# speechandlanguageprocessing/ICASSP2022-Depression

Measured on AMD Instinct MI355X. Metric: utterances/sec (train step) for GRU-256 on (B,T,F)=(512,300,256), higher is better.
Workload: dtype f32; 1 GPU; audio_gru_whole.AudioBiLSTM train step, B=512/GPU T=300 F=256 H=256 L=2 dropout=0.5 AdamW, CE-on-softmax; global_batch=512, parallelism=dp1, ranks=1, backend=none

## Files before the change

### icassp2022-depression_amd/_lib.py

```python
import ctypes as C
import os

import torch

HERE = os.path.dirname(os.path.abspath(__file__))
LIB_PATH = os.environ.get('DEP_LIB_PATH') or os.path.join(HERE, 'libdep_rnn.so')

CELL_GRU, CELL_LSTM = 0, 1
POOL_NONE, POOL_MEAN, POOL_SUM = 0, 1, 2
RUN_EVAL, RUN_TRAIN, RUN_DROPOUT_ONLY = 0, 1, 2
LOSS_CE_ON_SOFTMAX, LOSS_L1_RELU, LOSS_SMOOTHL1_RELU, LOSS_CE_LOGITS, LOSS_SMOOTHL1 = 0, 1, 2, 3, 4
LOSS_LABELS_I64 = 0x100
REG_L1, REG_SMOOTHL1, REG_HUBER, REG_MSE = 0, 1, 2, 3
SITE_FC0, SITE_FC1, SITE_FC2, SITE_FC3 = 1, 2, 3, 4


class DepError(RuntimeError):
    pass


class RnnDesc(C.Structure):
    _fields_ = [('cell', C.c_int32), ('B', C.c_int32), ('T', C.c_int32), ('F', C.c_int32), ('H', C.c_int32),
                ('L', C.c_int32), ('dirs', C.c_int32), ('training', C.c_int32), ('dropout_p', C.c_float),
                ('seed', C.c_uint64), ('pool', C.c_int32), ('impl', C.c_int32)]


_P = C.c_void_p


class GradSync(C.Structure):
    _fields_ = [('comm', _P), ('comm_stream', _P), ('range_ptr', _P * 8), ('range_count', C.c_long * 8)]


_BWD_ARGS = [C.POINTER(RnnDesc), _P, C.POINTER(_P), _P, _P, _P, C.POINTER(_P), _P, _P, C.c_size_t, _P, C.c_size_t, _P]
_BWD_VARLEN_ARGS = _BWD_ARGS[:2] + [_P] + _BWD_ARGS[2:]
_SIGS = {
    'dep_last_error': (C.c_char_p, []),
    'dep_version': (C.c_int, []),
    'dep_arch': (C.c_char_p, []),
    'dep_rnn_reserve_bytes': (C.c_size_t, [C.POINTER(RnnDesc)]),
    'dep_rnn_workspace_bytes': (C.c_size_t, [C.POINTER(RnnDesc)]),
    'dep_rnn_reserve_y_offset': (C.c_size_t, [C.POINTER(RnnDesc), C.c_int]),
    'dep_rnn_reserve_ydrop_offset': (C.c_size_t, [C.POINTER(RnnDesc), C.c_int]),
    'dep_rnn_status': (C.c_int, [C.POINTER(RnnDesc), _P, _P]),
    'dep_rnn_set_exclusive': (C.c_int, [C.c_int]),
    'dep_rnn_get_exclusive': (C.c_int, []),
    'dep_rnn_workspace_xbuf_offset': (C.c_size_t, [C.POINTER(RnnDesc)]),
    'dep_rnn_forward': (C.c_int, [C.POINTER(RnnDesc), _P, C.POINTER(_P), _P, _P, _P, _P, C.c_size_t, _P, C.c_size_t, _P]),
    'dep_rnn_backward': (C.c_int, _BWD_ARGS),
    'dep_rnn_backward_overlapped': (C.c_int, _BWD_ARGS + [C.POINTER(GradSync)]),
    'dep_rnn_forward_varlen': (C.c_int, [C.POINTER(RnnDesc), _P, _P, C.POINTER(_P), _P, _P, _P, _P, C.c_size_t, _P, C.c_size_t, _P]),
    'dep_rnn_backward_varlen': (C.c_int, _BWD_VARLEN_ARGS),
    'dep_rnn_backward_overlapped_varlen': (C.c_int, _BWD_VARLEN_ARGS + [C.POINTER(GradSync)]),
    'dep_comm_available': (C.c_int, []),
    'dep_comm_unique_id': (C.c_int, [_P, C.c_size_t]),
    'dep_comm_init': (C.c_int, [C.POINTER(_P), C.c_int, C.c_int, _P, C.c_size_t, C.c_int]),
    'dep_comm_world': (C.c_int, [_P]),
    'dep_comm_rank': (C.c_int, [_P]),
    'dep_comm_allreduce': (C.c_int, [_P, _P, C.c_long, _P]),
    'dep_comm_allreduce_ranges': (C.c_int, [_P, C.POINTER(_P), C.POINTER(C.c_long), C.c_int, _P]),
    'dep_comm_destroy': (C.c_int, [_P]),
    'dep_gemm_workspace_bytes': (C.c_size_t, [C.c_int] * 5),
    'dep_gemm_f32': (C.c_int, [C.c_int] * 5 + [_P, C.c_int, _P, C.c_int, _P, C.c_int, _P, C.c_float, C.c_int, C.c_int,
                               _P, C.c_size_t, _P]),
    'dep_gemm_bf16x3': (C.c_int, [C.c_int] * 5 + [_P, C.c_int, _P, C.c_int, _P, C.c_int, _P, C.c_float, C.c_int, C.c_int,
                                  _P, C.c_size_t, _P]),
    'dep_gemm': (C.c_int, [C.c_int] * 5 + [_P, C.c_int, _P, C.c_int, _P, C.c_int, _P, C.c_float, C.c_int, C.c_int,
                           _P, C.c_size_t, _P]),
    'dep_set_gemm_mode': (C.c_int, [C.c_int, C.c_long]),
    'dep_get_gemm_mode': (C.c_int, []),
    'dep_layernorm_fwd': (C.c_int, [_P, _P, _P, _P, _P, C.c_int, C.c_int, C.c_float, _P]),
    'dep_ln_fold_fwd': (C.c_int, [_P, _P, _P, _P, _P, _P, C.c_int, C.c_int, _P]),
    'dep_ln_fold_bwd': (C.c_int, [_P, _P, _P, _P, _P, _P, _P, _P, _P, C.c_int, C.c_int, _P]),
    'dep_layernorm_bwd_workspace_bytes': (C.c_size_t, [C.c_int, C.c_int]),
    'dep_layernorm_bwd': (C.c_int, [_P, _P, _P, _P, _P, _P, _P, C.c_int, C.c_int, _P, C.c_size_t, _P]),
    'dep_attn_fwd': (C.c_int, [_P, _P, C.c_int, _P, _P, _P, _P, _P, _P, C.c_int, C.c_int, C.c_int, _P]),
    'dep_attn_bwd_workspace_bytes': (C.c_size_t, [C.c_int, C.c_int, C.c_int]),
    'dep_attn_bwd': (C.c_int, [_P, _P, _P, _P, _P, _P, C.c_int, _P, _P, _P, _P, C.c_int, C.c_int, C.c_int, _P,
                               C.c_size_t, _P]),
    'dep_attn_fwd_varlen': (C.c_int, [_P, _P, _P, C.c_int, _P, _P, _P, _P, _P, _P, C.c_int, C.c_int, C.c_int, _P]),
    'dep_attn_bwd_varlen': (C.c_int, [_P, _P, _P, _P, _P, _P, _P, C.c_int, _P, _P, _P, _P, C.c_int, C.c_int, C.c_int, _P,
                                      C.c_size_t, _P]),
    'dep_dropout': (C.c_int, [_P, _P, C.c_long, C.c_float, C.c_uint64, C.c_uint32, _P]),
    'dep_dropout_mask': (C.c_int, [_P, C.c_long, C.c_float, C.c_uint64, C.c_uint32, _P]),
    'dep_relu_dropout_fwd': (C.c_int, [_P, _P, C.c_long, C.c_float, C.c_uint64, C.c_uint32, _P]),
    'dep_relu_dropout_bwd': (C.c_int, [_P, _P, _P, C.c_long, C.c_float, C.c_uint64, C.c_uint32, _P]),
    'dep_colsum': (C.c_int, [_P, C.c_int, C.c_int, C.c_int, _P, _P]),
    'dep_head_loss': (C.c_int, [C.c_int, _P, _P, _P, _P, _P, C.c_int, C.c_int, C.c_float, _P]),
    'dep_reduce_loss': (C.c_int, [_P, C.c_int, C.c_float, _P, C.c_int, _P]),
    'dep_head_loss_ce': (C.c_int, [C.c_int, _P, _P, _P, C.c_float, C.c_longlong, _P, _P, _P, C.c_int, C.c_int, C.c_float, _P, _P]),
    'dep_ce_weight_sum': (C.c_int, [_P, C.c_int, _P, C.c_longlong, C.c_int, C.c_int, _P, _P]),
    'dep_reduce_loss_by': (C.c_int, [_P, C.c_int, _P, _P, C.c_int, _P]),
    'dep_head_loss_reg': (C.c_int, [C.c_int, C.c_int, C.c_float, _P, _P, _P, _P, _P, _P, C.c_int, C.c_int, C.c_float, _P, _P]),
    'dep_row_weight_sum': (C.c_int, [_P, C.c_int, C.c_float, _P, _P]),
    'dep_gemm_set_xcds': (C.c_int, [C.c_int, C.c_int]),
    'dep_head_mlp_supported': (C.c_int, [C.c_int, C.c_int, C.c_int]),
    'dep_head_mlp_fwd': (C.c_int, [_P] * 9 + [C.c_int] * 4 + [C.c_float, C.c_uint64, C.c_uint32, C.c_uint32, C.c_int, _P]),
    'dep_head_mlp_bwd': (C.c_int, [_P] * 12 + [C.c_int] * 4 + [C.c_float, C.c_uint64, C.c_uint32, C.c_uint32, C.c_int, _P]),
    'dep_adam_step': (C.c_int, [_P, _P, _P, _P, C.c_long, C.c_float, C.c_float, C.c_float, C.c_float, C.c_float,
                                C.c_int, C.c_int, _P]),
    'dep_grad_norm_slots': (C.c_int, []),
    'dep_grad_norm_chunk': (C.c_int, []),
    'dep_grad_sqnorm': (C.c_int, [C.POINTER(_P), C.POINTER(C.c_long), C.c_int, _P, _P]),
    'dep_adam_step_clipped': (C.c_int, [_P, _P, _P, _P, C.c_long, C.c_float, C.c_float, C.c_float, C.c_float, C.c_float,
                                        C.c_int, C.c_int, _P, C.c_float, C.c_int, _P, _P, _P]),
    'dep_grad_clip_scale': (C.c_int, [C.POINTER(_P), C.POINTER(C.c_long), C.c_int, _P, C.c_float, _P, _P]),
    'dep_grad_accumulate': (C.c_int, [C.POINTER(_P), C.POINTER(_P), C.POINTER(C.c_long), C.c_int, C.c_float, C.c_int, _P, _P]),
    'dep_adam_step_ext': (C.c_int, [_P, _P, _P, _P, C.c_long, C.c_float, C.c_float, C.c_float, C.c_float, C.c_float,
                                    C.c_int, C.c_int, _P, _P, C.c_float, C.c_int, _P, _P, _P]),
    'dep_swap': (C.c_int, [_P, _P, C.c_long, _P]),
    'dep_frame_window': (C.c_int, [_P, C.c_long, C.c_int, C.c_int, C.c_int, _P, _P]),
    'dep_power_spectrum': (C.c_int, [_P, C.c_int, C.c_int, C.c_int, _P, _P]),
    'dep_log_floor': (C.c_int, [_P, _P, C.c_long, C.c_float, _P]),
    'dep_row_softmax': (C.c_int, [_P, _P, C.c_int, C.c_int, _P]),
    'dep_vlad_normalize': (C.c_int, [_P, _P, _P, _P, C.c_int, C.c_int, _P]),
    'dep_profile_enable': (C.c_int, [C.c_int]),
    'dep_profile_read': (C.c_int, [C.POINTER(C.c_double), C.POINTER(C.c_int), C.c_int]),
    'dep_instance_log_enable': (C.c_int, [C.c_int]),
    'dep_instance_log_read': (C.c_long, [C.c_char_p, C.c_long, C.c_int]),
    'dep_order_log_enable': (C.c_int, [C.c_int]),
    'dep_order_log_note': (C.c_int, [C.c_char_p]),
    'dep_order_log_read': (C.c_long, [C.c_char_p, C.c_long, C.c_int]),
    'dep_fill': (C.c_int, [_P, C.c_long, C.c_float, _P]),
    'dep_axpby': (C.c_int, [_P, _P, C.c_long, C.c_float, C.c_float, _P]),
    'dep_sigmoid_gate': (C.c_int, [_P, _P, _P, C.c_long, _P]),
    'dep_loss_accumulate': (C.c_int, [_P, _P, _P, _P, _P]),
    'dep_gather_rows': (C.c_int, [_P, _P, _P, C.c_long, C.c_long, _P]),
    'dep_copy2d': (C.c_int, [_P, C.c_long, _P, C.c_long, C.c_long, C.c_long, _P]),
    'dep_argmax_count': (C.c_int, [_P, _P, C.c_int, C.c_int, C.c_int, _P, _P, _P]),
}
EXPORTS = tuple(_SIGS)

_lib = None

# ... 362 lines not shown
    lib = load()
    dev = out.device
    dout = torch.empty_like(out)
    dh_n = torch.empty(K, B, H, dtype=torch.float32, device=dev)
    ws = torch.empty(lib.dep_attn_bwd_workspace_bytes(B, T, H) // 4 + 64, dtype=torch.float32, device=dev)
    if lengths is not None:
        check(lib.dep_attn_bwd_varlen(_ptr(dctx), _ptr(out), _ptr(check_lengths(lengths, B, dev)), _ptr(Wa), _ptr(alpha), _ptr(pre),
                                      _ptr(hsum), K, _ptr(dout), _ptr(dh_n), _ptr(dWa), _ptr(dba), B, T, H, _ptr(ws),
                                      ws.numel() * 4, stream()), 'dep_attn_bwd_varlen')
        return dout, dh_n
    check(lib.dep_attn_bwd(_ptr(dctx), _ptr(out), _ptr(Wa), _ptr(alpha), _ptr(pre), _ptr(hsum), K, _ptr(dout),
                           _ptr(dh_n), _ptr(dWa), _ptr(dba), B, T, H, _ptr(ws), ws.numel() * 4, stream()),
          'dep_attn_bwd')
    return dout, dh_n


_fallback_noted = [False]


def note_fallback():
    load().dep_rnn_set_exclusive(0)
    if not _fallback_noted[0]:
        _fallback_noted[0] = True
        import warnings
        warnings.warn('icassp2022_depression_amd: the GPU is shared with other kernels -- the fused GRU forward fell back to the '
                      'co-schedule-tolerant sweeps (results unaffected); using those directly from now on '
                      '(dep_rnn_set_exclusive(0); set DEP_EXCLUSIVE=0 to start that way)', RuntimeWarning, stacklevel=3)


class Rnn:

    def __init__(self, cell, B, T, F, H, L, dirs, training, dropout_p, pool, device, impl=0):
        self.lib = load()
        self.desc = RnnDesc(cell, B, T, F, H, L, dirs, int(training), float(dropout_p), 0, pool, impl)
        self.device = device
        rb = self.lib.dep_rnn_reserve_bytes(C.byref(self.desc))
        wb = self.lib.dep_rnn_workspace_bytes(C.byref(self.desc))
        if rb == 0 or wb == 0:
            why = self.lib.dep_last_error().decode() if cell == CELL_GRU and dirs == 2 else ''
            raise DepError(f'bad rnn descriptor: {cell=} {B=} {T=} {F=} {H=} {L=} {dirs=} {impl=}' + (f': {why}' if 'bidirectional GRU' in why else ''))
        self.reserve = torch.empty(rb // 4, dtype=torch.float32, device=device)
        self.workspace = torch.empty(wb // 4, dtype=torch.float32, device=device)
        self.n_w = 4 * L * dirs
        self._warr = (_P * self.n_w)()
        self._garr = (_P * self.n_w)()

    def check(self):
        check(self.lib.dep_rnn_status(C.byref(self.desc), _ptr(self.workspace), stream()), 'dep_rnn_status')
        w = self.fallback_word()
        if w is not None and self.lib.dep_rnn_get_exclusive() and int(w.item()) != 0:
            note_fallback()

    def fallback_word(self):
        off = self.lib.dep_rnn_workspace_xbuf_offset(C.byref(self.desc))
        if off == C.c_size_t(-1).value:
            return None
        return self.workspace.view(torch.int32)[off // 4 + 1]

    def status_word(self):
        off = self.lib.dep_rnn_workspace_xbuf_offset(C.byref(self.desc))
        if off == C.c_size_t(-1).value:
            return None
        return self.workspace.view(torch.int32)[off // 4]

    def layer_output(self, layer=None):
        d = self.desc
        layer = d.L - 1 if layer is None else layer
        off = self.lib.dep_rnn_reserve_y_offset(C.byref(d), layer)
        if off == C.c_size_t(-1).value:
            raise DepError(f'layer {layer} output is not kept in the reserve (run mode {d.training}; pass y= to forward)')
        off //= 4
        n = d.B * d.T * d.H * d.dirs
        return self.reserve[off:off + n].view(d.B, d.T, d.H * d.dirs)

    def layer_output_dropped(self, layer):
        d = self.desc
        off = self.lib.dep_rnn_reserve_ydrop_offset(C.byref(d), layer)
        if off == C.c_size_t(-1).value:
            return None
        off //= 4
        n = d.B * d.T * d.H * d.dirs
        return self.reserve[off:off + n].view(d.B, d.T, d.H * d.dirs)

    def forward(self, x, weights, seed=0, pooled=None, h_n=None, y=None, lengths=None):
        for i, w in enumerate(weights):
            self._warr[i] = w.data_ptr()
        self.desc.seed = seed
        if lengths is not None:
            check(self.lib.dep_rnn_forward_varlen(C.byref(self.desc), _ptr(x), _ptr(check_lengths(lengths, self.desc.B, self.device)),
                                                  self._warr, _ptr(y), _ptr(pooled), _ptr(h_n), _ptr(self.reserve),
                                                  self.reserve.numel() * 4, _ptr(self.workspace), self.workspace.numel() * 4,
                                                  stream()), 'dep_rnn_forward_varlen')
            return
        check(self.lib.dep_rnn_forward(C.byref(self.desc), _ptr(x), self._warr, _ptr(y), _ptr(pooled), _ptr(h_n),
                                       _ptr(self.reserve), self.reserve.numel() * 4, _ptr(self.workspace),
                                       self.workspace.numel() * 4, stream()), 'dep_rnn_forward')

    def backward(self, x, weights, dweights, dy=None, dpooled=None, dh_n=None, dx=None, grad_sync=None, lengths=None):
        for i, (w, g) in enumerate(zip(weights, dweights)):
            self._warr[i] = w.data_ptr()
            self._garr[i] = g.data_ptr()
        args = (C.byref(self.desc), _ptr(x), self._warr, _ptr(dy), _ptr(dpooled), _ptr(dh_n), self._garr, _ptr(dx),
                _ptr(self.reserve), self.reserve.numel() * 4, _ptr(self.workspace), self.workspace.numel() * 4, stream())
        if lengths is not None:
            args = args[:2] + (_ptr(check_lengths(lengths, self.desc.B, self.device)),) + args[2:]
            if grad_sync is None:
                check(self.lib.dep_rnn_backward_varlen(*args), 'dep_rnn_backward_varlen')
            else:
                check(self.lib.dep_rnn_backward_overlapped_varlen(*args, C.byref(grad_sync)), 'dep_rnn_backward_overlapped_varlen')
        elif grad_sync is None:
            check(self.lib.dep_rnn_backward(*args), 'dep_rnn_backward')
        else:
            check(self.lib.dep_rnn_backward_overlapped(*args, C.byref(grad_sync)), 'dep_rnn_backward_overlapped')


PROF_CATS = ('gru_fwd_sweep', 'gru_bwd_sweep', 'lstm_fwd_sweep', 'lstm_bwd_sweep', 'gemm_nt', 'gemm_nn', 'gemm_tn')


def instance_log_enable(on=True):
    load().dep_instance_log_enable(int(on))


def instance_log_read(reset=False):
    lib = load()
    n = lib.dep_instance_log_read(None, 0, 0)
    buf = C.create_string_buffer(n + 1)
    lib.dep_instance_log_read(buf, n + 1, int(reset))
    return set(l for l in buf.value.decode().split('\n') if l)


def profile_enable(on=True):
    load().dep_profile_enable(int(on))


def profile_read():
    n = len(PROF_CATS)
    ms = (C.c_double * n)(); cnt = (C.c_int * n)()
    load().dep_profile_read(ms, cnt, n)
    return {PROF_CATS[i]: (ms[i], cnt[i]) for i in range(n)}


_order_on = [False]


def order_log_enable(on=True):
    load().dep_order_log_enable(int(on)); _order_on[0] = bool(on)


def order_note(text):
    if _order_on[0]:
        load().dep_order_log_note(text.encode())


def order_log_read(reset=False):
    lib = load()
    n = lib.dep_order_log_read(None, 0, 0)
    buf = C.create_string_buffer(n + 1)
    lib.dep_order_log_read(buf, n + 1, int(reset))
    return [l for l in buf.value.decode().split('\n') if l]
```

### icassp2022-depression_amd/csrc/api.hip

```cpp
#include <stdarg.h>
#include <stdlib.h>
#include <string.h>
#include <atomic>
#include <mutex>
#include <set>
#include <string>
#include <utility>
#include <vector>
#include "dep_common.h"

static thread_local char g_err[512] = "";

void dep_set_error(const char* fmt, ...) {
    va_list ap;
    va_start(ap, fmt);
    vsnprintf(g_err, sizeof(g_err), fmt, ap);
    va_end(ap);
}

extern "C" const char* dep_last_error(void) { return g_err; }
extern "C" int dep_version(void) { return 100; }
extern "C" const char* dep_arch(void) { return "gfx950"; }

namespace {
// ... 197 lines not shown
    }
    {
        const size_t b3 = (size_t)D * G * H * maxin * sizeof(float);
        if (b3 > gb) gb = b3;
    }
    lo.gemm = w; lo.gemm_bytes = gb; w += al(gb / sizeof(float) + 64);
    const bool cok = d->cell == DEP_CELL_GRU ? d->dirs == 1 && dep_cluster_ok(d->cell, d->H, d->B, d->dirs) : dep_cluster_lstm_ok(d->H, d->B, d->dirs);
    if (d->impl == 3 && !cok) return false;
    lo.cluster = cok && (d->impl == 0 || d->impl == 3);
    lo.xbuf = w; lo.xbuf_bytes = !lo.cluster ? 0 : (d->cell == DEP_CELL_GRU ? dep_cluster_xbuf_bytes(d->cell, d->H, d->B, d->dirs)
                                                                : dep_cluster_lstm_xbuf_bytes(d->H, d->B, d->dirs));
    if (lo.cluster) lo.nwg = dep_cdiv(d->B, 16);
    lo.fused2 = lo.cluster && dep_fused2_ok(d->cell, d->H, d->L, d->dirs);
    if (lo.fused2) {
        size_t fb = dep_fused2_xbuf_bytes(d->B); if (fb > lo.xbuf_bytes) lo.xbuf_bytes = fb;
        if (lo.keep) { fb = dep_fused2_bwd_xbuf_bytes(d->B); if (fb > lo.xbuf_bytes) lo.xbuf_bytes = fb; }
    }
    w += al(lo.xbuf_bytes / sizeof(float) + 64);
    lo.wih_img = w; if (lo.fused2) w += al(G * H * H);
    lo.gi2 = lo.dghn2 = lo.dbpart2 = 0;
    if (lo.fused2 && lo.keep) {
        lo.gi2 = w; w += al(lo.BT * (G + 1) * H);
        lo.dghn2 = w; w += al(lo.BT * H);
        lo.dbpart2 = w; w += al((size_t)lo.nwg * 4 * H);
    }
    lo.ws_floats = w;
    return true;
}

}

extern "C" size_t dep_rnn_reserve_bytes(const dep_rnn_desc* d) {
    Layout lo;
    if (!make_layout(d, lo)) { (void)bigru_refusal(d, "dep_rnn_reserve_bytes"); return 0; }
    return lo.reserve_floats * sizeof(float);
}
extern "C" size_t dep_rnn_workspace_bytes(const dep_rnn_desc* d) {
    Layout lo;
    if (!make_layout(d, lo)) return 0;
    return lo.ws_floats * sizeof(float);
}
extern "C" size_t dep_rnn_reserve_y_offset(const dep_rnn_desc* d, int layer) {
    Layout lo;
    if (!make_layout(d, lo) || layer < 0 || layer >= d->L || lo.y[layer] == NOT_KEPT) return (size_t)-1;
    return lo.y[layer] * sizeof(float);
}
extern "C" size_t dep_rnn_reserve_ydrop_offset(const dep_rnn_desc* d, int layer) {
    Layout lo;
    if (!make_layout(d, lo) || layer < 0 || layer >= d->L - 1 || !lo.drop) return (size_t)-1;
    return lo.ydrop[layer] * sizeof(float);
}

extern "C" size_t dep_rnn_workspace_xbuf_offset(const dep_rnn_desc* d) {
    Layout lo;
    if (!make_layout(d, lo) || !lo.cluster) return (size_t)-1;
    return lo.xbuf * sizeof(float);
}

extern "C" int dep_rnn_status(const dep_rnn_desc* d, void* workspace, void* stream) {
    Layout lo;
    DEP_CHECK_ARG(make_layout(d, lo) && workspace);
    if (!lo.cluster) return DEP_OK;
    unsigned st = 0;
    if (hipMemcpyAsync(&st, (float*)workspace + lo.xbuf, sizeof(st), hipMemcpyDeviceToHost, (hipStream_t)stream) != hipSuccess ||
        hipStreamSynchronize((hipStream_t)stream) != hipSuccess) {
        dep_set_error("dep_rnn_status: HIP copy failed"); return DEP_ERR_HIP;
    }
    if (st != 0) { dep_set_error("cluster sweep gave up waiting for a member (status %u)", st); return DEP_ERR_HIP; }
    return DEP_OK;
}

const RnnSwitches& dep_rnn_switches() {
    static const RnnSwitches sw = [] {
        RnnSwitches w;
        const char* e = getenv("DEP_SV16"); w.sv16 = !(e && e[0] == '0');
        e = getenv("DEP_LSTM_SV16"); w.lstm_sv16 = e && e[0] == '1';
        e = getenv("DEP_FUSED2"); w.fused2 = !(e && e[0] == '0');
        e = getenv("DEP_FUSED2_BWD"); w.fused2_bwd = e ? e[0] == '1' : DEP_FUSED2_BWD_DEFAULT != 0;
        e = getenv("DEP_CLUSTER16"); w.cluster16 = !(e && e[0] == '0');
        e = getenv("DEP_CLUSTER_LSTM"); w.cluster_lstm = !(e && e[0] == '0');
        e = getenv("DEP_DGI_PK"); w.dgi_pk = !(e && e[0] == '0');
        e = getenv("DEP_COMM_OVERLAP"); w.comm_beside_sweeps = e && e[0] == 's';
        e = getenv("DEP_EXCLUSIVE"); w.exclusive = !(e && e[0] == '0');
        return w;
    }();
    return sw;
}

static std::atomic<int> g_exclusive{-1};
static bool dep_exclusive_on() { const int v = g_exclusive.load(std::memory_order_relaxed); return v >= 0 ? v == 1 : dep_rnn_switches().exclusive; }
extern "C" int dep_rnn_set_exclusive(int on) { g_exclusive.store(on ? 1 : 0); return DEP_OK; }
extern "C" int dep_rnn_get_exclusive(void) { return dep_exclusive_on() ? 1 : 0; }

namespace {

enum FwdKernel { FWD_FUSED2,
                 FWD_CLUSTER16,
                 FWD_CLUSTER_GRU,
                 FWD_CLUSTER_LSTM,
                 FWD_TILE };
enum BwdKernel { BWD_FUSED2, BWD_CLUSTER_GRU, BWD_CLUSTER_LSTM, BWD_TILE };
enum WhhImage { WHH_NONE, WHH_SPLIT16, WHH_SPLIT32, WHH_LSTM_PAIR , WHH_BWD_SPLIT, WHH_BWD_F32  };
enum ReserveTag { TAG_SPLIT = 1, TAG_SV16 = 4, TAG_BF16ST = 8, TAG_DONLY = 16 };

struct RnnPlan {
    bool excl;
    bool split;
    FwdKernel fwd; BwdKernel bwd;
    bool whh_f32;
    WhhImage whh_fwd, whh_bwd;
    bool sv16;
    bool sv16_fwd;
    bool dg4;
    bool bf16st;
    bool pk;
    int pk_fmt;
    bool dw_pair;
    int tag;
};

RnnPlan make_plan(const dep_rnn_desc* d, const Layout& lo, int mode, bool excl, bool ragged) {
    const RnnSwitches& sw = dep_rnn_switches();
    const bool gru = d->cell == DEP_CELL_GRU;
    RnnPlan p{};
    p.excl = excl; p.split = mode >= 1;
    const bool csplit = lo.cluster && p.split;
    const bool cluster16 = lo.cluster && dep_cluster16_ok(d->cell, d->H, d->B);
    p.fwd = (lo.fused2 && p.split && excl && !ragged) ? FWD_FUSED2 : (cluster16 && excl && !ragged) ? FWD_CLUSTER16
          : !lo.cluster ? FWD_TILE : gru ? FWD_CLUSTER_GRU : FWD_CLUSTER_LSTM;
    p.bwd = (lo.fused2 && sw.fused2_bwd && p.split && dep_fused2_bwd_fits(d->B, d->T) && !ragged) ? BWD_FUSED2
          : !lo.cluster ? BWD_TILE : gru ? BWD_CLUSTER_GRU : BWD_CLUSTER_LSTM;
    p.whh_f32 = lo.cluster ? !p.split : dep_sweep_use_mfma(d->H, d->impl);
    p.whh_fwd = !csplit ? WHH_NONE : !gru ? WHH_LSTM_PAIR : p.fwd == FWD_CLUSTER16 ? WHH_SPLIT16 : WHH_SPLIT32;
    p.whh_bwd = (!lo.cluster || !lo.keep || p.whh_fwd == WHH_LSTM_PAIR) ? WHH_NONE : p.split ? WHH_BWD_SPLIT : WHH_BWD_F32;
    p.sv16 = p.split && sw.sv16 && d->training != DEP_RUN_EVAL && lo.cluster && (gru ? (lo.fused2 || !cluster16) : dep_cluster_lstm_sv16_ok());
    p.sv16_fwd = p.sv16 && p.fwd != FWD_CLUSTER16;
    p.dg4 = lo.cluster && gru && d->dirs == 1;
    p.bf16st = mode == 3 && lo.keep && p.sv16 && lo.fused2 && p.dg4 && d->T % 2 == 0 && dep_cluster_bwd_pk_ok(d->H, d->T);
    p.pk = sw.dgi_pk && csplit && lo.BT % 2 == 0 &&
           (gru ? p.dg4 && d->T % 2 == 0 && (p.bwd == BWD_FUSED2 || dep_cluster_bwd_pk_ok(d->H, d->T)) : d->dirs == 2 && dep_cluster_lstm_bwd_pk_ok(d->T));
    p.pk_fmt = (p.bf16st || mode >= 2) ? FMT_PKH : FMT_PK;
    p.dw_pair = p.dg4 && mode == 1;
    p.tag = (p.split ? TAG_SPLIT : 0) | (p.sv16 ? TAG_SV16 : 0) | (p.bf16st ? TAG_BF16ST : 0) | (lo.donly ? TAG_DONLY : 0);
    return p;
}

struct LayerIn { const float* p; int K; };
LayerIn layer_input(const dep_rnn_desc* d, const Layout& lo, const float* x, const float* R, int l) {
    if (l == 0) return {x, d->F};
    return {R + (lo.drop ? lo.ydrop[l - 1] : lo.y[l - 1]), d->dirs * d->H};
}

struct TagRec { const void* p; int tag; };
TagRec g_tags[256];
int g_tag_next = 0;
std::mutex g_tag_mu;
void record_reserve_tag(const void* reserve, int tag) {
    std::lock_guard<std::mutex> lk(g_tag_mu);
    for (auto& r : g_tags) if (r.p == reserve) { r.tag = tag; return; }
    g_tags[g_tag_next] = {reserve, tag};
    g_tag_next = (g_tag_next + 1) % 256;
}
int reserve_tag_refusal(const void* reserve, int want, int bits) {
    int have = -1;
    {
        std::lock_guard<std::mutex> lk(g_tag_mu);
        for (auto& r : g_tags) if (r.p == reserve) { have = r.tag; break; }
    }
    if (have < 0) return DEP_OK;
    const int diff = (have ^ want) & bits;
    if (diff & TAG_DONLY)
        dep_set_error("dep_rnn_backward: the reserve was last written by a DEP_RUN_DROPOUT_ONLY forward, which keeps no saved gates; "
                      "run the forward with DEP_RUN_TRAIN before a backward");
    else if (diff & TAG_SPLIT)
        dep_set_error("dep_rnn_backward: the reserve was produced by a forward in %s mode, the current mode is %s "
                      "(dep_set_gemm_mode must not change between a forward and its backward)",
                      (have & TAG_SPLIT) ? "bf16x3" : "f32", (have & TAG_SPLIT) ? "f32" : "bf16x3");
    else if (diff & TAG_BF16ST)
        dep_set_error("dep_rnn_backward: the reserve was %swritten in bf16-storage mode (dep_set_gemm_mode(3)), this call runs in the other", (have & TAG_BF16ST) ? "" : "not ");
    else if (diff & TAG_SV16)
        dep_set_error("dep_rnn_backward: the reserve holds %s saved gates, this call expects the other format (DEP_SV16 / DEP_EXCLUSIVE changed?)",
                      (have & TAG_SV16) ? "16-bit" : "fp32");
    return diff ? DEP_ERR_ARG : DEP_OK;
}

int ragged_mode_refusal(const char* who, const int32_t* lengths, int mode) {
    if (!lengths || mode <= 1) return DEP_OK;
    dep_set_error("%s: a ragged call (lengths given) runs in GEMM modes 0 and 1 only; the current mode is %d (dep_set_gemm_mode)", who, mode);
    return DEP_ERR_ARG;
}

}

static int rnn_forward_impl(const dep_rnn_desc* d, const float* x, const int32_t* lengths, const float* const* weights, float* y,
                            float* pooled, float* h_n, void* reserve, size_t reserve_bytes, void* workspace,
                            size_t workspace_bytes, void* stream) {
    Layout lo;
    if (const int rf = bigru_refusal(d, "dep_rnn_forward")) return rf;
    DEP_CHECK_ARG(make_layout(d, lo));
    const int mode = dep_get_gemm_mode();
    if (const int rf = ragged_mode_refusal("dep_rnn_forward_varlen", lengths, mode)) return rf;
    const RnnPlan p = make_plan(d, lo, mode, dep_exclusive_on(), lengths != nullptr);
    DEP_CHECK_ARG(x && weights && reserve && workspace);
    DEP_CHECK_ARG(!(pooled && (d->cell != DEP_CELL_GRU || d->pool == DEP_POOL_NONE)));
    if (reserve_bytes < lo.reserve_floats * sizeof(float) || workspace_bytes < lo.ws_floats * sizeof(float)) {
        dep_set_error("dep_rnn_forward: reserve/workspace too small (%zu/%zu given, %zu/%zu needed)", reserve_bytes,
                      workspace_bytes, lo.reserve_floats * sizeof(float), lo.ws_floats * sizeof(float));
        return DEP_ERR_WORKSPACE;
    }
    hipStream_t s = (hipStream_t)stream;
    float* R = (float*)reserve; float* W = (float*)workspace;
    const int B = d->B, T = d->T, H = d->H, D = d->dirs, G = lo.G, L = d->L;
    const int BTr = (int)lo.BT;
    DepGemmOpts proj; proj.scratch = W + lo.gemm; proj.scratch_bytes = lo.gemm_bytes;
    float* const gi = W + lo.gi;
    int rc;
    if (lo.cluster) { rc = dep_cluster_reset_status(W + lo.xbuf, s); if (rc) return rc; }
    if (p.bf16st && (!p.excl || y)) {
        dep_set_error("dep_rnn_forward: bf16-storage mode (dep_set_gemm_mode(3)) runs the exclusive fused forward only (dep_rnn_set_exclusive(1)) "
                      "and has no fp32 copy of the output sequence (y must be NULL)");
        return DEP_ERR_ARG;
    }
    record_reserve_tag(reserve, p.tag);
    auto yout = [&](int l, bool null_ok) -> float* {
        if (lo.y[l] != NOT_KEPT) return R + lo.y[l];
        if (l == L - 1 && y) return y;
        return null_ok ? nullptr : W + lo.dx[0];
    };
    const bool ytop_kept = lo.y[L - 1] != NOT_KEPT;
    const float pool_scale = d->pool == DEP_POOL_MEAN ? 1.0f / (float)T : 1.0f;
    auto sweep_args = [&](int l, const unsigned* only_if) {
        dep_sweep_args a{};
        a.B = B; a.T = T; a.H = H; a.cell = d->cell; a.dirs = D; a.training = d->training; a.impl = d->impl;
        a.split = (lo.cluster && p.split) ? 1 : 0;
        for (int dd = 0; dd < D; ++dd) {
            const float* const* wl = weights + (size_t)(l * D + dd) * 4;
            a.w_hh[dd] = wl[1]; a.b_hh[dd] = wl[3]; a.wp[dd] = R + lo.wp[l][dd];
        }
        const bool dropl = lo.drop && l < L - 1;
        a.gi = gi; a.y = yout(l, p.fwd == FWD_CLUSTER_LSTM && dropl); a.ldy = D * H;
        a.ydrop = dropl ? R + lo.ydrop[l] : nullptr;
        a.drop_p = dropl ? d->dropout_p : 0.f; a.seed = d->seed; a.site = DEP_SITE_RNN0 + l;
        a.pooled = l == L - 1 ? pooled : nullptr;
        a.pool_scale = pool_scale;
        a.h_n = h_n ? h_n + (size_t)l * D * B * H : nullptr;
        if (lo.keep) { a.sv0 = R + lo.sv[l][0]; a.sv1 = R + lo.sv[l][1]; a.sv2 = R + lo.sv[l][2]; a.sv3 = R + lo.sv[l][3]; }
        a.only_if = only_if; a.stream = s; a.sv16 = p.sv16_fwd ? 1 : 0;
        a.lengths = lengths; a.pool_mean = d->pool == DEP_POOL_MEAN ? 1 : 0;
        a.hdr_slot = only_if ? 1 + l : (l < DEP_HDR_SLOTS ? l : 0); a.hdr_clean = only_if || l < DEP_HDR_SLOTS;
        return a;
    };
    if (p.fwd == FWD_FUSED2) {
        const float* const* w0 = weights; const float* const* w1 = weights + 4;
        for (int k = 0; k < 4; ++k) DEP_CHECK_ARG(w0[k] && w1[k]);
        {
            const float* srcs[5] = {w0[1], w1[1], w1[0], w0[1], w1[1]};
            float* dsts[5] = {R + lo.wp[0][0], R + lo.wp[1][0], W + lo.wih_img, R + lo.wpT[0][0], R + lo.wpT[1][0]};
            const int kinds[5] = {0, 0, 0, 1, 1};
            rc = dep_pack_cluster_split_multi(p.whh_bwd == WHH_BWD_SPLIT ? 5 : 3, srcs, dsts, kinds, H, s); if (rc) return rc;
        }
        rc = dep_gemm_internal(0, 1, BTr, G * H, d->F, x, d->F, w0[0], d->F, gi, G * H, w0[2], 0.f, 0, 0, nullptr, 0, proj, s);
        if (rc) return rc;
        dep_fused2_args f{};
        f.B = B; f.T = T; f.training = d->training;
        f.wp0 = R + lo.wp[0][0]; f.wp1 = R + lo.wp[1][0]; f.wpi = W + lo.wih_img;
        f.b_hh0 = w0[3]; f.b_ih1 = w1[2]; f.b_hh1 = w1[3];
        f.ostride = (lo.BT * H + 63) / 64 * 64;
        f.gi = gi; f.y0 = lo.donly ? nullptr : R + lo.y[0]; f.y0d = (lo.drop && !lo.donly) ? R + lo.ydrop[0] : nullptr; f.y1 = yout(1, true);
        f.drop_p = lo.drop ? d->dropout_p : 0.f; f.seed = d->seed; f.site = DEP_SITE_RNN0;
        f.pooled = pooled; f.pool_scale = pool_scale;
        f.hn0 = h_n; f.hn1 = h_n ? h_n + (size_t)B * H : nullptr;
        for (int l = 0; l < 2; ++l) for (int k = 0; k < 4; ++k) f.sv[l][k] = lo.keep ? R + lo.sv[l][k] : nullptr;
        f.stream = s;
        f.soft_fallback = p.bf16st ? 0 : 1;
        f.sv16 = p.sv16 ? 1 : 0; f.bf16st = p.bf16st ? 1 : 0;
        f.hdr_clean = 1;
        rc = dep_launch_fused2_fwd(f, W + lo.xbuf, lo.xbuf_bytes); if (rc) return rc;
        const unsigned* soft = reinterpret_cast<const unsigned*>(W + lo.xbuf) + 1;
        for (int l = 0; l < 2 && !p.bf16st; ++l) {
            if (l == 1) {
                const LayerIn in = layer_input(d, lo, x, R, 1);
                DepGemmOpts fallback = proj; fallback.only_if = soft;
                rc = dep_gemm_internal(0, 1, BTr, G * H, in.K, in.p, in.K, w1[0], in.K, gi, G * H, w1[2], 0.f, 0, 0, nullptr, 0, fallback, s);
                if (rc) return rc;
            }
            rc = dep_launch_cluster_fwd(sweep_args(l, soft), W + lo.xbuf, lo.xbuf_bytes); if (rc) return rc;
        }
        if (y && ytop_kept) { rc = dep_axpby(R + lo.y[1], y, (long)lo.BT * H, 1.f, 0.f, s); if (rc) return rc; }
        return DEP_OK;
    }
    if (D == 2) {
        const float* src[16]; const float* add[16]; float* dst[16]; long cnt[16]; int nj = 0;
        for (int l = 0; l < L; ++l) {
            const int Kl = layer_input(d, lo, x, R, l).K;
            for (int dd = 0; dd < D; ++dd) {
                const float* const* wl = weights + (size_t)(l * D + dd) * 4;
                DEP_CHECK_ARG(wl[0] && wl[1] && wl[2] && wl[3]);
                src[nj] = wl[0]; add[nj] = nullptr; dst[nj] = R + lo.wstack[l] + (size_t)dd * G * H * Kl; cnt[nj++] = (long)G * H * Kl;
                src[nj] = wl[2]; add[nj] = d->cell == DEP_CELL_LSTM ? wl[3] : nullptr; dst[nj] = R + lo.bstack[l] + (size_t)dd * G * H; cnt[nj++] = (long)G * H;
                if (nj == 16) { rc = dep_multi_copy(nj, src, add, dst, cnt, s); if (rc) return rc; nj = 0; }
            }
        }
        if (nj) { rc = dep_multi_copy(nj, src, add, dst, cnt, s); if (rc) return rc; }
    }
    for (int l = 0; l < L; ++l) {
        const LayerIn in = layer_input(d, lo, x, R, l);
        const int Kl = in.K;
        const bool stacked = D == 2;
        for (int dd = 0; dd < D; ++dd) {
            const float* const* wl = weights + (size_t)(l * D + dd) * 4;
            DEP_CHECK_ARG(wl[0] && wl[1] && wl[2] && wl[3]);
            float* const wp = R + lo.wp[l][dd]; float* const wpT = lo.wpT[l][dd] == NOT_KEPT ? nullptr : R + lo.wpT[l][dd];
            if (p.whh_f32) { rc = dep_pack_whh(wl[1], wp, wpT, G, H, s); if (rc) return rc; }
            rc = p.whh_fwd == WHH_LSTM_PAIR ? dep_pack_cluster_lstm_split(wl[1], wp, lo.keep ? wpT : nullptr, H, s)
               : p.whh_fwd == WHH_SPLIT16 ? dep_pack_cluster16_fwd_split(wl[1], wp, H, s)
               : p.whh_fwd == WHH_SPLIT32 ? dep_pack_cluster_fwd_split(wl[1], wp, H, s) : DEP_OK;
            if (rc) return rc;
            rc = p.whh_bwd == WHH_BWD_SPLIT ? dep_pack_cluster_bwd_split(wl[1], wpT, H, s)
               : p.whh_bwd == WHH_BWD_F32 ? dep_pack_cluster_bwd(wl[1], wpT, G, H, s) : DEP_OK;
            if (rc) return rc;
            const float* bias = wl[2];
            if (stacked) continue;
            if (d->cell == DEP_CELL_LSTM) {
                float* tb = W + lo.biastmp;
                rc = dep_axpby(wl[2], tb, (long)G * H, 1.f, 0.f, s); if (rc) return rc;
                rc = dep_axpby(wl[3], tb, (long)G * H, 1.f, 1.f, s); if (rc) return rc;
                bias = tb;
            }
            rc = dep_gemm_internal(0, 1, BTr, G * H, Kl, in.p, Kl, wl[0], Kl, gi + (size_t)dd * G * H, D * G * H, bias,
                                   0.f, 0, 0, nullptr, 0, proj, s);
            if (rc) return rc;
        }
        if (stacked) {
            rc = dep_gemm_internal(0, 1, BTr, D * G * H, Kl, in.p, Kl, R + lo.wstack[l], Kl, gi, D * G * H, R + lo.bstack[l],
                                   0.f, 0, 0, nullptr, 0, proj, s);
            if (rc) return rc;
        }
        const dep_sweep_args a = sweep_args(l, nullptr);
        rc = p.fwd == FWD_CLUSTER16 ? dep_launch_cluster16_fwd(a, W + lo.xbuf, lo.xbuf_bytes)
           : p.fwd == FWD_CLUSTER_LSTM ? dep_launch_cluster_lstm_fwd(a, W + lo.xbuf, lo.xbuf_bytes)
           : p.fwd == FWD_CLUSTER_GRU ? dep_launch_cluster_fwd(a, W + lo.xbuf, lo.xbuf_bytes) : dep_launch_sweep_fwd(a);
        if (rc) return rc;
    }
    if (y && ytop_kept) {
        rc = dep_axpby(R + lo.y[L - 1], y, (long)lo.BT * D * H, 1.f, 0.f, s);
        if (rc) return rc;
    }
    return DEP_OK;
}

extern "C" int dep_rnn_forward(const dep_rnn_desc* d, const float* x, const float* const* weights, float* y,
                               float* pooled, float* h_n, void* reserve, size_t reserve_bytes, void* workspace,
                               size_t workspace_bytes, void* stream) {
    return rnn_forward_impl(d, x, nullptr, weights, y, pooled, h_n, reserve, reserve_bytes, workspace, workspace_bytes, stream);
}

extern "C" int dep_rnn_forward_varlen(const dep_rnn_desc* d, const float* x, const int32_t* lengths, const float* const* weights,
                                      float* y, float* pooled, float* h_n, void* reserve, size_t reserve_bytes, void* workspace,
                                      size_t workspace_bytes, void* stream) {
    DEP_CHECK_ARG(lengths);
    return rnn_forward_impl(d, x, lengths, weights, y, pooled, h_n, reserve, reserve_bytes, workspace, workspace_bytes, stream);
}

static int rnn_backward_impl(const dep_rnn_desc* d, const float* x, const int32_t* lengths, const float* const* weights, const float* dy,
                             const float* dpooled, const float* dh_n, float* const* dweights, float* dx,
                             void* reserve, size_t reserve_bytes, void* workspace, size_t workspace_bytes,
                             void* stream, const dep_grad_sync* gs) {
    Layout lo;
    if (const int rf = bigru_refusal(d, "dep_rnn_backward")) return rf;
    DEP_CHECK_ARG(make_layout(d, lo));
    const int mode = dep_get_gemm_mode();
    if (const int rf = ragged_mode_refusal("dep_rnn_backward_varlen", lengths, mode)) return rf;
    const RnnPlan p = make_plan(d, lo, mode, dep_exclusive_on(), lengths != nullptr);
    if (d->training != DEP_RUN_TRAIN) {
        dep_set_error("dep_rnn_backward: the descriptor's run mode is %d; a backward needs a DEP_RUN_TRAIN (1) forward's reserve%s", d->training,
                      d->training == DEP_RUN_DROPOUT_ONLY ? " (DEP_RUN_DROPOUT_ONLY keeps no saved gates)" : "");
        return DEP_ERR_ARG;
    }
    int rc = reserve_tag_refusal(reserve, p.tag, TAG_DONLY); if (rc) return rc;
    DEP_CHECK_ARG(x && weights && dweights && reserve && workspace);
    DEP_CHECK_ARG(dy || dpooled || dh_n);
    DEP_CHECK_ARG(!(dpooled && (d->cell != DEP_CELL_GRU || d->pool == DEP_POOL_NONE)));
    if (reserve_bytes < lo.reserve_floats * sizeof(float) || workspace_bytes < lo.ws_floats * sizeof(float)) {
        dep_set_error("dep_rnn_backward: reserve/workspace too small");
        return DEP_ERR_WORKSPACE;
    }
    if (lo.cluster) { rc = reserve_tag_refusal(reserve, p.tag, TAG_SPLIT | TAG_BF16ST | TAG_SV16); if (rc) return rc; }
    hipStream_t s = (hipStream_t)stream;
    float* R = (float*)reserve; float* W = (float*)workspace;
    const int B = d->B, T = d->T, H = d->H, D = d->dirs, G = lo.G, L = d->L;
    const int BTr = (int)lo.BT;
    const bool gru = d->cell == DEP_CELL_GRU;
    void* gws = W + lo.gemm; const size_t gwsb = lo.gemm_bytes;
    const float pool_scale = d->pool == DEP_POOL_MEAN ? 1.0f / (float)T : 1.0f;
    const int ldg = p.dg4 ? 4 * H : D * G * H;
    const char* const no_pk = "dep_rnn_backward: bf16-storage mode needs the pre-split gate-gradient path (aligned operands, DEP_DGI_PK not 0, contractions above the split threshold)";
    const bool fused = p.bwd == BWD_FUSED2;
    auto al16 = [](const void* q) { return (reinterpret_cast<uintptr_t>(q) & 15) == 0; };
    auto pk_ok = [&](int l, const float* dxl) {
        const LayerIn in = layer_input(d, lo, x, R, l);
        const int M = D * G * H;
        bool ok = p.pk && (in.K % 4 == 0) && al16(in.p) &&
                  (gru ? al16(weights[(size_t)l * 4]) && al16(dweights[(size_t)l * 4]) : lo.wstack[l] != 0 && al16(W + lo.dwstack)) &&
                  dep_gemm_uses_bf16x3(M, in.K, BTr, 0) && dep_gemm_uses_bf16x3(G * H, H, BTr, T) &&
                  (!dxl || (dep_gemm_uses_bf16x3(BTr, in.K, M, 0) && al16(dxl)));
        for (int dd = 0; dd < D && ok; ++dd) ok = al16(dweights[(size_t)(l * D + dd) * 4 + 1]);
        return ok;
    };
    bool fused_pk = false;
    if (fused) {
        const float* const* w0 = weights; const float* const* w1 = weights + 4;
        float* const* g0 = dweights; float* const* g1 = dweights + 4;
        for (int k = 0; k < 4; ++k) DEP_CHECK_ARG(w0[k] && w1[k] && g0[k] && g1[k]);
        fused_pk = p.sv16 && pk_ok(1, nullptr) && pk_ok(0, dx);
        rc = dep_pack_cluster_bwd_split(w1[0], W + lo.wih_img, H, s); if (rc) return rc;
        dep_fused2_bwd_args f{};
        f.B = B; f.T = T;
        f.wh1 = R + lo.wpT[1][0]; f.wi1 = W + lo.wih_img; f.wh0 = R + lo.wpT[0][0];
        f.y1 = R + lo.y[1]; f.y0 = R + lo.y[0]; f.sv1 = R + lo.sv[1][0]; f.sv0 = R + lo.sv[0][0];
        f.svstride = (lo.BT * H + 63) / 64 * 64;
        f.dy = dy; f.dpooled = dpooled; f.pool_scale = pool_scale;
        f.dhn1 = dh_n ? dh_n + (size_t)B * H : nullptr; f.dhn0 = dh_n;
        f.drop_p = lo.drop ? d->dropout_p : 0.f; f.seed = d->seed; f.site = DEP_SITE_RNN0;
        f.dgi1 = W + lo.gi; f.dgi0 = W + lo.gi2;
        f.dghn1 = p.dg4 ? f.dgi1 + 3 * H : W + lo.dghn; f.dghn0 = p.dg4 ? f.dgi0 + 3 * H : W + lo.dghn2;
        f.lddg = ldg; f.lddghn = p.dg4 ? ldg : H;
        f.dbpart1 = W + lo.dbpart; f.dbpart0 = W + lo.dbpart2; f.dbpart_rows = lo.nwg; f.stream = s;
        if (p.bf16st && !fused_pk) { dep_set_error(no_pk); return DEP_ERR_ARG; }
        f.sv16 = p.sv16 ? 1 : 0; f.dg_pk = fused_pk ? 1 : 0; f.bf16st = p.bf16st ? 1 : 0;
        rc = dep_launch_fused2_bwd(f, W + lo.xbuf, lo.xbuf_bytes); if (rc) return rc;
    }
    auto sweep_args = [&](int l, bool pk) {
        const bool top = l == L - 1;
        const bool second = fused && l == 0;
        dep_sweep_bwd_args a{};
        a.B = B; a.T = T; a.H = H; a.cell = d->cell; a.dirs = D; a.impl = d->impl;
        a.split = (lo.cluster && p.split) ? 1 : 0;
        for (int dd = 0; dd < D; ++dd) {
            const float* const* wl = weights + (size_t)(l * D + dd) * 4;
            a.w_hh[dd] = wl[1]; a.wpT[dd] = R + lo.wpT[l][dd];
        }
        a.y = R + lo.y[l]; a.ldy = D * H;
        if (top) { a.dy = dy; a.drop_p = 0.f; }
        else { a.dy = W + lo.dx[(l + 1) & 1]; a.drop_p = lo.drop ? d->dropout_p : 0.f; }
        a.lddy = D * H; a.seed = d->seed; a.site = DEP_SITE_RNN0 + l;
        a.dpooled = top ? dpooled : nullptr;
        a.pool_scale = pool_scale;
        a.dh_n = dh_n ? dh_n + (size_t)l * D * B * H : nullptr;
        a.sv0 = R + lo.sv[l][0]; a.sv1 = R + lo.sv[l][1]; a.sv2 = R + lo.sv[l][2]; a.sv3 = R + lo.sv[l][3];
        a.dgi = W + (second ? lo.gi2 : lo.gi);
        a.dghn = p.dg4 ? a.dgi + 3 * H : W + (second ? lo.dghn2 : lo.dghn);
        a.lddg = p.dg4 ? ldg : 0; a.lddghn = p.dg4 ? ldg : 0;
        a.dbpart = W + (second ? lo.dbpart2 : lo.dbpart); a.dbpart_rows = D * lo.nwg; a.stream = s;
        a.hdr_slot = l < DEP_HDR_SLOTS ? l : 0; a.hdr_clean = l < DEP_HDR_SLOTS;
        a.dg_pk = pk ? 1 : 0; a.bf16st = p.bf16st ? 1 : 0; a.sv16 = p.sv16 ? 1 : 0;
        a.lengths = lengths; a.pool_mean = d->pool == DEP_POOL_MEAN ? 1 : 0;
        return a;
    };
    float* pending_ptr = nullptr; long pending_n = 0;
    if (lo.cluster && !fused) { rc = dep_cluster_reset_flags(W + lo.xbuf, s); if (rc) return rc; }
    for (int l = L - 1; l >= 0; --l) {
        const LayerIn lin = layer_input(d, lo, x, R, l);
        const float* const in = lin.p; const int Kl = lin.K;
        float* dxl = l == 0 ? dx : (fused ? nullptr : W + lo.dx[l & 1]);
        const bool pk = fused ? fused_pk : pk_ok(l, dxl);
        if (p.bf16st && !pk) { dep_set_error(no_pk); return DEP_ERR_ARG; }
        const dep_sweep_bwd_args a = sweep_args(l, pk);
        float* const dgi = a.dgi; float* const dghn = a.dghn;
        if (!fused) {
            rc = p.bwd == BWD_CLUSTER_LSTM ? dep_launch_cluster_lstm_bwd(a, W + lo.xbuf, lo.xbuf_bytes)
               : p.bwd == BWD_CLUSTER_GRU ? dep_launch_cluster_bwd(a, W + lo.xbuf, lo.xbuf_bytes) : dep_launch_sweep_bwd(a);
            if (rc) return rc;
        }
        if (pending_ptr) {
            rc = dep_comm_enqueue_after((dep_comm*)gs->comm, pending_ptr, pending_n, s, (hipStream_t)gs->comm_stream);
            if (rc) return rc;
            pending_ptr = nullptr;
        }
        float* dbi[2]; float* dbh[2];
        for (int dd = 0; dd < D; ++dd) {
            float* const* gl = dweights + (size_t)(l * D + dd) * 4;
            DEP_CHECK_ARG(gl[0] && gl[1] && gl[2] && gl[3]);
            dbi[dd] = gl[2]; dbh[dd] = gl[3];
        }
        rc = dep_finish_db(a, dbi, dbh);
        if (rc) return rc;
        DepGemmOpts go; go.scratch = gws; go.scratch_bytes = gwsb;
        if (pk) go.fmt_a = p.pk_fmt;
        const bool stacked = D == 2 && lo.wstack[l] != 0;
        if (dxl && stacked) {
            rc = dep_gemm_internal(0, 0, BTr, Kl, D * G * H, dgi, ldg, R + lo.wstack[l], Kl, dxl, Kl, nullptr, 0.f, 0, 0, nullptr, 0, go, s);
            if (rc) return rc;
        } else if (dxl) {
            for (int dd = 0; dd < D; ++dd) {
                const float* const* wl = weights + (size_t)(l * D + dd) * 4;
                rc = dep_gemm_internal(0, 0, BTr, Kl, G * H, dgi + (size_t)dd * G * H, ldg, wl[0], Kl, dxl, Kl, nullptr,
                                       dd == 0 ? 0.f : 1.f, 0, 0, nullptr, 0, go, s);
                if (rc) return rc;
            }
        }
        if (stacked) {
            float* dws = W + lo.dwstack;
            rc = dep_gemm_internal(1, 0, D * G * H, Kl, BTr, dgi, ldg, in, Kl, dws, Kl, nullptr, 0.f, 0, 0, gws, gwsb, go, s);
            if (rc) return rc;
            const float* src[2]; float* dst[2]; long cnt[2];
            for (int dd = 0; dd < D; ++dd) {
                src[dd] = dws + (size_t)dd * G * H * Kl; dst[dd] = (dweights + (size_t)(l * D + dd) * 4)[0]; cnt[dd] = (long)G * H * Kl;
            }
            rc = dep_multi_copy(D, src, nullptr, dst, cnt, s); if (rc) return rc;
        }
        bool paired = false;
        const bool pair_layer = p.dw_pair && Kl == H;
        const bool pair_shape = pair_layer && pk && !p.bf16st;
        DepGemmOpts dwo = go; dwo.split_target = pair_layer ? 512 : 0;
        if (pair_shape) {
            float* const* gl = dweights + (size_t)l * 4;
            DepGemmOpts po = dwo; po.skip_at = 2 * H; po.skip_by = H;
            const int pr = dep_gemm_tn_pair(G * H, H, BTr, dgi, dgi, ldg, in, Kl, 0, 0, R + lo.y[l], H, T, -1, gl[0], Kl, gl[1], H, po, gws, gwsb, s);
            if (pr < 0) return pr;
            paired = pr == 1;
        }
        bool paired_hh = false;
        if (pk && !gru) {
            float* const* gf = dweights + (size_t)(l * D) * 4; float* const* gb = dweights + (size_t)(l * D + 1) * 4;
            const int pr = dep_gemm_tn_pair(G * H, H, BTr, dgi, dgi + (size_t)G * H, ldg, R + lo.y[l], D * H, T, -1, R + lo.y[l] + H, D * H, T, 1,
                                            gf[1], H, gb[1], H, dwo, gws, gwsb, s);
            if (pr < 0) return pr;
            paired_hh = pr == 1;
        }
        for (int dd = 0; dd < D && !paired && !paired_hh; ++dd) {
            float* const* gl = dweights + (size_t)(l * D + dd) * 4;
            const float* dg = dgi + (size_t)dd * G * H;
            if (!stacked) {
                DepGemmOpts io = dwo; io.fmt_b = (p.bf16st && l > 0) ? FMT_BF16 : FMT_F32;
                rc = dep_gemm_internal(1, 0, G * H, Kl, BTr, dg, ldg, in, Kl, gl[0], Kl, nullptr, 0.f, 0, 0, gws, gwsb, io, s);
                if (rc) return rc;
            }
            DepGemmOpts ho = dwo; ho.fmt_b = p.bf16st ? FMT_BF16 : FMT_F32;
            const float* yl = R + lo.y[l] + (size_t)dd * H;
            const int shift = dd == 0 ? -1 : 1;
            if (p.dg4 && dep_gemm_uses_bf16x3(3 * H, H, BTr, T)) {
                DepGemmOpts so = ho; so.skip_at = 2 * H; so.skip_by = H;
                rc = dep_gemm_internal(1, 0, 3 * H, H, BTr, dg, ldg, yl, D * H, gl[1], H, nullptr, 0.f, T, shift, gws, gwsb, so, s);
                if (rc) return rc;
            } else if (gru) {
                rc = dep_gemm_internal(1, 0, 2 * H, H, BTr, dg, ldg, yl, D * H, gl[1], H, nullptr, 0.f, T, shift, gws, gwsb, ho, s);
                if (rc) return rc;
                rc = dep_gemm_internal(1, 0, H, H, BTr, dghn + (size_t)dd * H, p.dg4 ? ldg : D * H, yl, D * H, gl[1] + (size_t)2 * H * H, H, nullptr,
                                       0.f, T, shift, gws, gwsb, ho, s);
                if (rc) return rc;
            } else {
                rc = dep_gemm_internal(1, 0, 4 * H, H, BTr, dg, ldg, yl, D * H, gl[1], H, nullptr, 0.f, T, shift, gws, gwsb, ho, s);
                if (rc) return rc;
            }
        }
        if (gs && gs->comm && gs->range_ptr[l] && gs->range_count[l] > 0) {
            if (l > 0 && !dep_rnn_switches().comm_beside_sweeps && !fused) { pending_ptr = gs->range_ptr[l]; pending_n = gs->range_count[l]; }
            else {
                rc = dep_comm_enqueue_after((dep_comm*)gs->comm, gs->range_ptr[l], gs->range_count[l], s, (hipStream_t)gs->comm_stream);
                if (rc) return rc;
            }
        }
    }
    return DEP_OK;
}

extern "C" int dep_rnn_backward(const dep_rnn_desc* d, const float* x, const float* const* weights, const float* dy,
                                const float* dpooled, const float* dh_n, float* const* dweights, float* dx,
                                void* reserve, size_t reserve_bytes, void* workspace, size_t workspace_bytes,
// ... 32 lines not shown
```

### icassp2022-depression_amd/csrc/dep_common.h

```cpp
#pragma once
#include <hip/hip_runtime.h>
#include <stdint.h>
#include <stdio.h>
#include "../../include/dep_rnn.h"

typedef float f32x4 __attribute__((ext_vector_type(4)));
typedef float f32x16 __attribute__((ext_vector_type(16)));

void dep_set_error(const char* fmt, ...);

#define DEP_CHECK_ARG(cond)                                                          \
    do {                                                                             \
        if (!(cond)) {                                                               \
            dep_set_error("%s:%d: bad argument: %s", __FILE__, __LINE__, #cond);     \
            return DEP_ERR_ARG;                                                      \
        }                                                                            \
    } while (0)

#define DEP_CHECK_LAUNCH()                                                           \
    do {                                                                             \
        hipError_t e__ = hipGetLastError();                                          \
        if (e__ != hipSuccess) {                                                     \
            dep_set_error("%s:%d: HIP: %s", __FILE__, __LINE__, hipGetErrorString(e__)); \
            return DEP_ERR_HIP;                                                      \
        }                                                                            \
    } while (0)

static inline size_t dep_align(size_t x, size_t a = 256) { return (x + a - 1) / a * a; }
static inline int dep_cdiv(long a, long b) { return (int)((a + b - 1) / b); }

__device__ __forceinline__ float dep_sigmoid(float x) { return 1.0f / (1.0f + expf(-x)); }

__device__ __forceinline__ void dep_philox4(uint64_t seed, uint32_t site, uint64_t g4, uint32_t (&r)[4]) {
    uint32_t k0 = (uint32_t)seed, k1 = (uint32_t)(seed >> 32);
    uint32_t c0 = (uint32_t)g4, c1 = (uint32_t)(g4 >> 32), c2 = site, c3 = 0x2545F491u;
#pragma unroll
    for (int i = 0; i < 10; ++i) {
        const uint32_t hi0 = __umulhi(0xD2511F53u, c0), lo0 = 0xD2511F53u * c0;
        const uint32_t hi1 = __umulhi(0xCD9E8D57u, c2), lo1 = 0xCD9E8D57u * c2;
        const uint32_t n0 = hi1 ^ c1 ^ k0, n1 = lo1, n2 = hi0 ^ c3 ^ k1, n3 = lo0;
        c0 = n0; c1 = n1; c2 = n2; c3 = n3;
        k0 += 0x9E3779B9u; k1 += 0xBB67AE85u;
    }
    r[0] = c0; r[1] = c1; r[2] = c2; r[3] = c3;
}
__device__ __forceinline__ f32x4 dep_dropmask4(uint64_t seed, uint32_t site, uint64_t g4, float p, float scale) {
    uint32_t r[4];
    dep_philox4(seed, site, g4, r);
    f32x4 m;
#pragma unroll
    for (int i = 0; i < 4; ++i) {
        const float u = (float)(r[i] >> 8) * (1.0f / 16777216.0f);
        m[i] = (u >= p) ? scale : 0.0f;
    }
    return m;
}
__device__ __forceinline__ float dep_dropmask1(uint64_t seed, uint32_t site, uint64_t idx, float p, float scale) {
    const f32x4 m = dep_dropmask4(seed, site, idx >> 2, p, scale);
    return m[idx & 3];
}

__device__ __forceinline__ int dep_row_len(const int* lengths, int b, int T) { const int n = lengths[b]; return n < 0 ? 0 : (n > T ? T : n); }
__device__ __forceinline__ float dep_ragged_pool_scale(int pool_mean, int len, int T, float dense_scale) {
    return !pool_mean ? 1.0f : len == T ? dense_scale : len > 0 ? 1.0f / (float)len : 0.f;
}
__device__ __forceinline__ float2 dep_sel2(bool c, float2 a, float2 b) { return make_float2(c ? a.x : b.x, c ? a.y : b.y); }
__device__ __forceinline__ f32x4 dep_sel4(bool c, f32x4 a, f32x4 b) { f32x4 r = {c ? a[0] : b[0], c ? a[1] : b[1], c ? a[2] : b[2], c ? a[3] : b[3]}; return r; }


enum { DEP_SITE_RNN0 = 16 , DEP_SITE_USER = 0 };

__device__ __forceinline__ void dep_xcd_tile(int gx, int gy, int gz, int& bx, int& by, int& bz) {
    const int n = gx * gy * gz, orig = blockIdx.x;
    const int q = n / 8, r = n % 8, xcd = orig % 8;
    const int id = (xcd < r ? xcd * (q + 1) : r * (q + 1) + (xcd - r) * q) + orig / 8;
    bx = id % gx; by = (id / gx) % gy; bz = id / (gx * gy);
}

bool dep_ilog_on();
void dep_ilog_note(const char* kern, const char* where);
void dep_olog_add(char kind, const char* text, long n);
#define DEP_LAUNCH(kern, grid, blk, lds, stream, ...)                                          \
    do {                                                                                       \
        if (dep_ilog_on()) dep_ilog_note(#kern, __PRETTY_FUNCTION__);                          \
        hipLaunchKernelGGL(kern, grid, blk, lds, stream, __VA_ARGS__);                         \
    } while (0)

enum { DEP_PROF_GRU_FWD = 0, DEP_PROF_GRU_BWD = 1, DEP_PROF_LSTM_FWD = 2, DEP_PROF_LSTM_BWD = 3,
       DEP_PROF_GEMM_NT = 4, DEP_PROF_GEMM_NN = 5, DEP_PROF_GEMM_TN = 6, DEP_PROF_NCAT = 7 };
enum { FMT_F32 = 0, FMT_PK = 1, FMT_PKH = 2, FMT_BF16 = 3 };
enum { DEP_PREC_MODE = 0, DEP_PREC_EXACT = 1, DEP_PREC_X3 = 2 };
struct DepGemmOpts {
    int prec = DEP_PREC_MODE;
    int fmt_a = FMT_F32, fmt_b = FMT_F32;
    int skip_at = 0, skip_by = 0;
    long split_target = 0;
    const unsigned* only_if = nullptr;
    void* scratch = nullptr; size_t scratch_bytes = 0;
};
struct DepGemmSwitches {
    int mode;
    bool naive, pair, tn_dma, nt_dma, bm256, nt256;
    long split_target;
    int ablate, persist;
};
const DepGemmSwitches& dep_gemm_switches();
bool dep_gemm_bf16x3_pair_ok();
bool dep_gemm_uses_bf16x3(int M, int N, int K, int seq_T);
int dep_gemm_tn_pair(int M, int N, int K, const float* A0, const float* A1, int lda,
                     const float* B0, int ldb0, int seq_T0, int shift0, const float* B1, int ldb1, int seq_T1, int shift1,
                     float* C0, int ldc0, float* C1, int ldc1, const DepGemmOpts& o, void* ws, size_t ws_bytes, hipStream_t s);
int dep_gemm_bf16x3_tn_pair_launch(int M, int N, int K, const float* A0, const float* A1, int lda,
                                   const float* B0, int ldb0, int seq_T0, int shift0, const float* B1, int ldb1, int seq_T1, int shift1,
                                   float* C0, int ldc0, float* C1, int ldc1, const DepGemmOpts& o, int splits, int kchunk, float* part0, float* part1,
                                   hipStream_t s);
struct RnnSwitches {
    bool sv16, lstm_sv16;
    bool fused2, fused2_bwd;
    bool cluster16, cluster_lstm;
    bool dgi_pk;
    bool comm_beside_sweeps;
    bool exclusive;
};
const RnnSwitches& dep_rnn_switches();
bool dep_prof_on();
void dep_prof_begin(int cat, hipStream_t s);
void dep_prof_end(hipStream_t s);
struct DepProfScope {
    hipStream_t s; bool on;
    DepProfScope(int cat, hipStream_t st, bool enable = true) : s(st), on(enable && dep_prof_on()) { if (on) dep_prof_begin(cat, s); }
    ~DepProfScope() { if (on) dep_prof_end(s); }
};

struct dep_sweep_args {
    int B, T, H;
    int cell, dirs;
    int training;
    int impl;
    const float* w_hh[2];
    const float* b_hh[2];
    const float* wp[2];
    int split;
    const float* gi;
    float* y;  int ldy;
    float* ydrop;
    float drop_p; uint64_t seed; uint32_t site;
    float* pooled; float pool_scale;
    float* h_n;
    float* sv0; float* sv1; float* sv2; float* sv3;
    const unsigned* only_if;
    int sv16;
    int hdr_slot, hdr_clean;
    const int* lengths;
    int pool_mean;
    hipStream_t stream;
};
int dep_launch_sweep_fwd(const dep_sweep_args& a);

struct dep_sweep_bwd_args {
    int B, T, H;
    int cell, dirs;
    int impl;
    const float* w_hh[2];
    const float* wpT[2];
    int split;
    const float* y; int ldy;
    const float* dy; int lddy;
    float drop_p; uint64_t seed; uint32_t site;
    const float* dpooled; float pool_scale;
    const float* dh_n;
    const float* sv0; const float* sv1; const float* sv2; const float* sv3;
    float* dgi;
    float* dghn;
    int lddg, lddghn;
    float* dbpart;
    int dbpart_rows;
    int hdr_slot, hdr_clean;
    int sv16;
    int dg_pk;
    int bf16st;
    const int* lengths;
    int pool_mean;
    hipStream_t stream;
};
bool dep_cluster_bwd_pk_ok(int H, int T);
#define DEP_FUSED2_BWD_DEFAULT 1
bool dep_cluster_lstm_bwd_pk_ok(int T);
bool dep_cluster_lstm_sv16_ok();
int dep_launch_sweep_bwd(const dep_sweep_bwd_args& a);
int dep_sweep_num_wg(int B, int H, int impl);
bool dep_sweep_use_mfma(int H, int impl);

size_t dep_pack_floats(int G, int H);
int dep_pack_whh(const float* w_hh, float* wp, float* wpT, int G, int H, hipStream_t s);
int dep_finish_db(const dep_sweep_bwd_args& a, float* const* db_ih, float* const* db_hh);

bool dep_cluster_ok(int cell, int H, int B, int dirs);
size_t dep_cluster_xbuf_bytes(int cell, int H, int B, int dirs);
int dep_pack_cluster_bwd(const float* w_hh, float* out, int G, int H, hipStream_t s);
int dep_launch_cluster_fwd(const dep_sweep_args& a, void* xbuf, size_t xbuf_bytes);
int dep_launch_cluster_bwd(const dep_sweep_bwd_args& a, void* xbuf, size_t xbuf_bytes);
bool dep_cluster16_ok(int cell, int H, int B);
bool dep_cluster_lstm_ok(int H, int B, int dirs);
size_t dep_cluster_lstm_xbuf_bytes(int H, int B, int dirs);
int dep_launch_cluster_lstm_fwd(const dep_sweep_args& a, void* xbuf, size_t xbuf_bytes);
int dep_launch_cluster_lstm_bwd(const dep_sweep_bwd_args& a, void* xbuf, size_t xbuf_bytes);
int dep_cluster_chunk(int members, int per_cu, int max_wgs);
struct dep_fused2_args {
    int B, T, training;
    const float* wp0; const float* wp1; const float* wpi;
    const float* b_hh0; const float* b_ih1; const float* b_hh1;
    const float* gi;
    float* y0; float* y0d; float* y1;
    size_t ostride;
    float drop_p; uint64_t seed; uint32_t site;
    float* pooled; float pool_scale; float* hn0; float* hn1;
    float* sv[2][4];
    int sv16;
    int bf16st;
    int soft_fallback;
    int hdr_clean;
    hipStream_t stream;
};
bool dep_fused2_ok(int cell, int H, int L, int dirs);
size_t dep_fused2_xbuf_bytes(int B);
int dep_launch_fused2_fwd(const dep_fused2_args& a, void* xbuf, size_t xbuf_bytes);
struct dep_fused2_bwd_args {
    int B, T;
    const float* wh1; const float* wi1; const float* wh0;
    const float* y1; const float* y0; const float* sv1; const float* sv0; size_t svstride;
    const float* dy; const float* dpooled; float pool_scale; const float* dhn1; const float* dhn0;
    float drop_p; uint64_t seed; uint32_t site;
    float* dgi1; float* dghn1; float* dgi0; float* dghn0; float* dbpart1; float* dbpart0; int dbpart_rows;
    int lddg, lddghn;
    int sv16;
    int bf16st;
    int dg_pk;
    hipStream_t stream;
};
size_t dep_fused2_bwd_xbuf_bytes(int B);
bool dep_fused2_bwd_fits(int B, int T);
int dep_launch_fused2_bwd(const dep_fused2_bwd_args& a, void* xbuf, size_t xbuf_bytes);
int dep_comm_enqueue_after(dep_comm* c, float* buf, long n, hipStream_t compute, hipStream_t comm_stream);
constexpr int DEP_HDR_SLOTS = 4;
int dep_cluster_reset_status(void* xbuf, hipStream_t s);
int dep_cluster_reset_flags(void* xbuf, hipStream_t s);
int dep_pack_cluster16_fwd_split(const float* w_hh, float* out, int H, hipStream_t s);
int dep_pack_cluster_bwd_split(const float* w_hh, float* out, int H, hipStream_t s);
int dep_pack_cluster_split_multi(int n, const float* const* src, float* const* dst, const int* bwd, int H, hipStream_t s);
int dep_multi_copy(int count, const float* const* src, const float* const* add, float* const* dst, const long* n, hipStream_t s);
int dep_attn2_fwd(const float* out, const float* pre, float* ctx, float* alpha, int B, int T, int H, const int* lengths, hipStream_t s);
int dep_attn2_bwd(const float* dctx, const float* out, const float* alpha, const float* pre, float* dout, float* dpre, int B,
                  int T, int H, const int* lengths, hipStream_t s);
int dep_pack_cluster_fwd_split(const float* w_hh, float* out, int H, hipStream_t s);
int dep_pack_cluster_lstm_split(const float* w_hh, float* wp, float* wpT, int H, hipStream_t s);
int dep_launch_cluster16_fwd(const dep_sweep_args& a, void* xbuf, size_t xbuf_bytes);

int dep_gemm_internal(int transA, int transB, int M, int N, int K, const float* A, int lda,
                      const float* B, int ldb, float* C, int ldc, const float* bias, float beta,
                      int seq_T, int shiftB, void* ws, size_t ws_bytes, const DepGemmOpts& o, hipStream_t s);
```

### icassp2022-depression_amd/csrc/elementwise.hip

```cpp
#include "dep_common.h"

namespace {

__device__ __forceinline__ float wave_sum(float v) {
#pragma unroll
    for (int m = 32; m >= 1; m >>= 1) v += __shfl_xor(v, m, 64);
    return v;
}
__device__ __forceinline__ float wave_max(float v) {
#pragma unroll
    for (int m = 32; m >= 1; m >>= 1) v = fmaxf(v, __shfl_xor(v, m, 64));
    return v;
}
__device__ __forceinline__ float block_sum(float v, float* red) {
    const int lane = threadIdx.x & 63, w = threadIdx.x >> 6, nw = blockDim.x >> 6;
    v = wave_sum(v);
    __syncthreads();
    if (lane == 0) red[w] = v;
    __syncthreads();
    float s = 0.f;
    for (int i = 0; i < nw; ++i) s += red[i];
    return s;
}
__device__ __forceinline__ float block_max(float v, float* red) {
    const int lane = threadIdx.x & 63, w = threadIdx.x >> 6, nw = blockDim.x >> 6;
    v = wave_max(v);
    __syncthreads();
    if (lane == 0) red[w] = v;
    __syncthreads();
    float s = red[0];
    for (int i = 1; i < nw; ++i) s = fmaxf(s, red[i]);
    return s;
}

__global__ __launch_bounds__(256) void ln_fwd_kernel(const float* __restrict__ x, const float* __restrict__ gamma,
                                                     const float* __restrict__ beta, float* __restrict__ y,
                                                     float* __restrict__ mr, int rows, int F, float eps) {
    const int lane = threadIdx.x & 63;
    const long row = (long)blockIdx.x * 4 + (threadIdx.x >> 6);
    if (row >= rows) return;
    const float* xr = x + row * F;
    float s = 0.f;
    for (int i = lane; i < F; i += 64) s += xr[i];
    const float mean = wave_sum(s) / (float)F;
    float v = 0.f;
    for (int i = lane; i < F; i += 64) { const float d = xr[i] - mean; v = fmaf(d, d, v); }
    const float rstd = 1.0f / sqrtf(wave_sum(v) / (float)F + eps);
    float* yr = y + row * F;
    if (gamma) { for (int i = lane; i < F; i += 64) yr[i] = (xr[i] - mean) * rstd * gamma[i] + beta[i]; }
    else       { for (int i = lane; i < F; i += 64) yr[i] = (xr[i] - mean) * rstd; }
    if (mr && lane == 0) { mr[row * 2] = mean; mr[row * 2 + 1] = rstd; }
}

template <int NV>
__global__ __launch_bounds__(256) void ln_fwd_vec_kernel(const float* __restrict__ x, const float* __restrict__ gamma,
                                                         const float* __restrict__ beta, float* __restrict__ y,
                                                         float* __restrict__ mr, int rows, float eps) {
    constexpr int F = 256 * NV;
    const int lane = threadIdx.x & 63;
    const long row = (long)blockIdx.x * 4 + (threadIdx.x >> 6);
    if (row >= rows) return;
    const f32x4* xr = reinterpret_cast<const f32x4*>(x + row * F);
    f32x4 v[NV];
    float s = 0.f;
#pragma unroll
    for (int i = 0; i < NV; ++i) { v[i] = xr[i * 64 + lane]; s += (v[i][0] + v[i][1]) + (v[i][2] + v[i][3]); }
    const float mean = wave_sum(s) / (float)F;
    float q = 0.f;
#pragma unroll
    for (int i = 0; i < NV; ++i)
#pragma unroll
        for (int e = 0; e < 4; ++e) { const float d = v[i][e] - mean; q = fmaf(d, d, q); }
    const float rstd = 1.0f / sqrtf(wave_sum(q) / (float)F + eps);
    f32x4* yr = reinterpret_cast<f32x4*>(y + row * F);
#pragma unroll
    for (int i = 0; i < NV; ++i) {
        f32x4 o = (v[i] - mean) * rstd;
        if (gamma) {
            o = o * reinterpret_cast<const f32x4*>(gamma)[i * 64 + lane] + reinterpret_cast<const f32x4*>(beta)[i * 64 + lane];
        }
        yr[i * 64 + lane] = o;
    }
    if (mr && lane == 0) { mr[row * 2] = mean; mr[row * 2 + 1] = rstd; }
}

__global__ __launch_bounds__(256) void ln_fold_fwd_kernel(const float* __restrict__ W, const float* __restrict__ b,
                                                          const float* __restrict__ gamma, const float* __restrict__ beta,
                                                          float* __restrict__ Wf, float* __restrict__ bf, int J, int F) {
    const int lane = threadIdx.x & 63;
    const int j = blockIdx.x * 4 + (threadIdx.x >> 6);
    if (j >= J) return;
    float s = 0.f;
    for (int f = lane; f < F; f += 64) {
        const float w = W[(size_t)j * F + f];
        Wf[(size_t)j * F + f] = w * gamma[f];
        s = fmaf(w, beta[f], s);
    }
    s = wave_sum(s);
    if (lane == 0) bf[j] = b[j] + s;
}
constexpr int LFC = 16, LFR = 64;
__global__ __launch_bounds__(1024) void ln_fold_bwd_kernel(const float* __restrict__ W, const float* __restrict__ P,
                                                           const float* __restrict__ q, const float* __restrict__ gamma,
                                                           const float* __restrict__ beta, float* __restrict__ dW,
                                                           float* __restrict__ db, float* __restrict__ dgamma,
                                                           float* __restrict__ dbeta, int J, int F) {
    __shared__ float red[2][LFR][LFC];
    const int c = threadIdx.x % LFC, rg = threadIdx.x / LFC;
    const int f = blockIdx.x * LFC + c;
    float dg = 0.f, dbt = 0.f;
    if (f < F) {
        const float g = gamma[f], bt = beta[f];
#pragma unroll 4
        for (int j = rg; j < J; j += LFR) {
            const float w = W[(size_t)j * F + f], pj = P[(size_t)j * F + f], qj = q[j];
            dW[(size_t)j * F + f] = fmaf(pj, g, qj * bt);
            dg = fmaf(pj, w, dg);
            dbt = fmaf(w, qj, dbt);
        }
    }
    red[0][rg][c] = dg; red[1][rg][c] = dbt;
    __syncthreads();
    if (rg < 2 && f < F) {
        float a = 0.f;
#pragma unroll 8
        for (int r = 0; r < LFR; ++r) a += red[rg][r][c];
        (rg == 0 ? dgamma : dbeta)[f] = a;
    }
    if (blockIdx.x == 0) for (int j = threadIdx.x; j < J; j += 1024) db[j] = q[j];
}

__global__ __launch_bounds__(256) void ln_bwd_param_kernel(const float* __restrict__ dy, const float* __restrict__ x,
                                                           const float* __restrict__ mr, float* __restrict__ partial,
                                                           int rows, int F, int rows_per_blk) {
    const long r0 = (long)blockIdx.x * rows_per_blk;
    const long r1 = min((long)rows, r0 + rows_per_blk);
    for (int c = threadIdx.x; c < F; c += blockDim.x) {
        float dg = 0.f, db = 0.f;
        for (long r = r0; r < r1; ++r) {
            const float mean = mr[r * 2], rstd = mr[r * 2 + 1];
            const float g = dy[r * F + c];
            dg = fmaf(g, (x[r * F + c] - mean) * rstd, dg);
            db += g;
        }
        partial[((size_t)blockIdx.x * 2) * F + c] = dg;
        partial[((size_t)blockIdx.x * 2 + 1) * F + c] = db;
    }
}
__global__ __launch_bounds__(256) void ln_bwd_dx_kernel(const float* __restrict__ dy, const float* __restrict__ x,
                                                        const float* __restrict__ gamma, const float* __restrict__ mr,
                                                        float* __restrict__ dx, int rows, int F) {
    const int lane = threadIdx.x & 63;
    const long row = (long)blockIdx.x * 4 + (threadIdx.x >> 6);
    if (row >= rows) return;
    const float mean = mr[row * 2], rstd = mr[row * 2 + 1];
    const float* xr = x + row * F; const float* gr = dy + row * F;
    float s1 = 0.f, s2 = 0.f;
    for (int i = lane; i < F; i += 64) {
        const float g = gr[i] * gamma[i];
        s1 += g; s2 = fmaf(g, (xr[i] - mean) * rstd, s2);
    }
    s1 = wave_sum(s1) / (float)F; s2 = wave_sum(s2) / (float)F;
    for (int i = lane; i < F; i += 64) {
        const float g = gr[i] * gamma[i], xh = (xr[i] - mean) * rstd;
        dx[row * F + i] = rstd * (g - s1 - xh * s2);
    }
}

__global__ void dropout_kernel(const float* x, float* y, long n, float p, float scale, uint64_t seed, uint32_t site) {
    const long i = (long)blockIdx.x * blockDim.x + threadIdx.x;
    if (i >= n) return;
    y[i] = x[i] * dep_dropmask1(seed, site, (uint64_t)i, p, scale);
}
__global__ void dropout_mask_kernel(float* m, long n, float p, float scale, uint64_t seed, uint32_t site) {
    const long i = (long)blockIdx.x * blockDim.x + threadIdx.x;
    if (i >= n) return;
    m[i] = dep_dropmask1(seed, site, (uint64_t)i, p, scale);
}
__global__ void relu_dropout_fwd_kernel(const float* z, float* a, long n, float p, float scale, uint64_t seed, uint32_t site) {
    const long i = (long)blockIdx.x * blockDim.x + threadIdx.x;
    if (i >= n) return;
    float v = fmaxf(z[i], 0.f);
// ... 734 lines not shown
```

### icassp2022-depression_amd/csrc/head.hip

```cpp
#include "dep_common.h"

namespace {

constexpr int HR = 4;
constexpr int HT = 512;
constexpr int HMAX = 256;
constexpr int HC = 16;
constexpr int JR = 4;
constexpr int BCH = 1024;

struct HeadF {
    const float *x, *W1, *b1, *W2, *b2;
    float *a0, *z1, *a1, *z2;
    int B, Hin, H1, C;
    float p, scale;
    uint64_t seed;
    uint32_t site0, site1;
    int first;
};

__device__ __forceinline__ float wsum(float v) {
#pragma unroll
    for (int m = 32; m >= 1; m >>= 1) v += __shfl_xor(v, m, 64);
    return v;
// ... 9 lines not shown
    const int j = tid & (HMAX - 1), half = tid >> 8;
    const bool mine = j < q.H1;
    f32x4 w[NV];
    {
        const float* wr = q.W1 + (size_t)(mine ? j : 0) * Hin + half * KH;
#pragma unroll
        for (int m = 0; m < NV; ++m) w[m] = *reinterpret_cast<const f32x4*>(wr + 4 * m);
    }
    const bool drop0 = q.first && q.p > 0.f;
    constexpr int NX = (HR * Hin + HT - 1) / HT;
    float xv[NX];
#pragma unroll
    for (int k = 0; k < NX; ++k) {
        const int e = tid + k * HT, r = e / Hin, row = row0 + r;
        const bool ok = e < HR * Hin && row < q.B;
        xv[k] = q.x[ok ? (size_t)row * Hin + (e - r * Hin) : 0];
    }
#pragma unroll
    for (int k = 0; k < NX; ++k) {
        const int e = tid + k * HT, r = e / Hin, i = e - r * Hin, row = row0 + r;
        if (e >= HR * Hin) continue;
        float v = 0.f;
        if (row < q.B) {
            const size_t at = (size_t)row * Hin + i;
            v = xv[k];
            if (drop0) { v *= dep_dropmask1(q.seed, q.site0, (uint64_t)at, q.p, q.scale); q.a0[at] = v; }
        }
        xs[r][i] = v;
    }
    __syncthreads();
    float acc[HR] = {0.f, 0.f, 0.f, 0.f};
#pragma unroll
    for (int m = 0; m < NV; ++m) {
#pragma unroll
        for (int r = 0; r < HR; ++r) {
            const f32x4 xv = *reinterpret_cast<const f32x4*>(&xs[r][half * KH + 4 * m]);
            acc[r] = fmaf(xv[0], w[m][0], acc[r]); acc[r] = fmaf(xv[1], w[m][1], acc[r]);
            acc[r] = fmaf(xv[2], w[m][2], acc[r]); acc[r] = fmaf(xv[3], w[m][3], acc[r]);
        }
    }
    if (half == 1) {
#pragma unroll
        for (int r = 0; r < HR; ++r) part[r][j] = acc[r];
    }
    __syncthreads();
    if (half == 0 && mine) {
        const float bj = q.b1[j];
#pragma unroll
        for (int r = 0; r < HR; ++r) {
            const int row = row0 + r;
            float a = 0.f;
            if (row < q.B) {
                const size_t at = (size_t)row * q.H1 + j;
                const float z = (acc[r] + part[r][j]) + bj;
                a = fmaxf(z, 0.f);
                if (q.p > 0.f) a *= dep_dropmask1(q.seed, q.site1, (uint64_t)at, q.p, q.scale);
                q.z1[at] = z; q.a1[at] = a;
            }
            as1[r][j] = a;
        }
    }
    if (q.C <= 0) return;
    __syncthreads();
    const int wv = tid >> 6, lane = tid & 63, row = row0 + wv;
    if (wv >= HR || row >= q.B) return;
    for (int c = 0; c < q.C; ++c) {
        float s = 0.f;
        for (int k = lane; k < q.H1; k += 64) s = fmaf(as1[wv][k], q.W2[(size_t)c * q.H1 + k], s);
        s = wsum(s);
        if (lane == 0) q.z2[(size_t)row * q.C + c] = s + q.b2[c];
    }
}

struct HeadB {
    const float *dz2, *a0, *z1, *a1, *W1, *W2;
    float *dW1, *db1, *dW2, *db2, *dx, *dz1;
    int B, Hin, H1, C;
    float p, scale;
    uint64_t seed;
    uint32_t site0, site1;
    int first;
};

template <int NJ>
__global__ __launch_bounds__(HT) void head_mlp_bwd_rows_kernel(HeadB q) {
    __shared__ __attribute__((aligned(16))) float dzs[HR][HMAX];
    __shared__ __attribute__((aligned(16))) float ps[HT / 64][HR][HMAX];
    constexpr int H1 = NJ * 8;
    const int tid = threadIdx.x, row0 = blockIdx.x * HR, wv = tid >> 6, lane = tid & 63, i4 = lane * 4;
    const bool want_dx = q.dx != nullptr, col = i4 < q.Hin;
    f32x4 w[NJ];
    if (want_dx) {
        const float* wr = q.W1 + (size_t)(wv * NJ) * q.Hin + (col ? i4 : 0);
#pragma unroll
        for (int m = 0; m < NJ; ++m) w[m] = *reinterpret_cast<const f32x4*>(wr + (size_t)m * q.Hin);
    }
    constexpr int NX = (HR * H1 + HT - 1) / HT;
    float zv[NX];
#pragma unroll
    for (int k = 0; k < NX; ++k) {
        const int e = tid + k * HT, r = e / H1, row = row0 + r;
        const bool ok = e < HR * H1 && row < q.B;
        zv[k] = q.z1[ok ? (size_t)row * H1 + (e - r * H1) : 0];
    }
#pragma unroll
    for (int k = 0; k < NX; ++k) {
        const int e = tid + k * HT, r = e / H1, j = e - r * H1, row = row0 + r;
        if (e >= HR * H1) continue;
        float v = 0.f;
        if (row < q.B) {
            const size_t at = (size_t)row * H1 + j;
            float da = 0.f;
            for (int c = 0; c < q.C; ++c) da = fmaf(q.dz2[(size_t)row * q.C + c], q.W2[(size_t)c * H1 + j], da);
            v = zv[k] > 0.f ? da : 0.f;
            if (q.p > 0.f) v *= dep_dropmask1(q.seed, q.site1, (uint64_t)at, q.p, q.scale);
            q.dz1[at] = v;
        }
        dzs[r][j] = v;
    }
    if (!want_dx) return;
    __syncthreads();
    f32x4 acc[HR];
#pragma unroll
    for (int r = 0; r < HR; ++r) acc[r] = f32x4{0.f, 0.f, 0.f, 0.f};
#pragma unroll
    for (int m = 0; m < NJ; ++m) {
#pragma unroll
        for (int r = 0; r < HR; ++r) {
            const float d = dzs[r][wv * NJ + m];
#pragma unroll
            for (int e = 0; e < 4; ++e) acc[r][e] = fmaf(d, w[m][e], acc[r][e]);
        }
    }
#pragma unroll
    for (int r = 0; r < HR; ++r) *reinterpret_cast<f32x4*>(&ps[wv][r][i4]) = acc[r];
    __syncthreads();
    const bool drop0 = q.first && q.p > 0.f;
    for (int e = tid; e < HR * q.Hin; e += HT) {
        const int r = e / q.Hin, i = e - r * q.Hin, row = row0 + r;
        if (row >= q.B) continue;
        float v = 0.f;
#pragma unroll
        for (int u = 0; u < HT / 64; ++u) v += ps[u][r][i];
        const size_t at = (size_t)row * q.Hin + i;
        if (drop0) v *= dep_dropmask1(q.seed, q.site0, (uint64_t)at, q.p, q.scale);
        q.dx[at] = v;
    }
}

__device__ __forceinline__ void weight_rows(const float* __restrict__ D, int ldD, int nrows, int row0, const float* __restrict__ A,
                                            int ldA, int ncols, int B, float* out, float* bias) {
    __shared__ __attribute__((aligned(16))) float ds[BCH][JR];
    __shared__ __attribute__((aligned(16))) float ps[HT / 64][JR][HMAX];
    __shared__ float pb[HT / 64][JR];
    static_assert(JR == 4, "one 16-byte broadcast per batch row");
    const int tid = threadIdx.x, wv = tid >> 6, lane = tid & 63, i4 = lane * 4;
    const bool col = i4 < ncols;
    const float* Ac = A + (col ? i4 : 0);
    f32x4 acc[JR];
    float sb[JR];
#pragma unroll
    for (int u = 0; u < JR; ++u) { acc[u] = f32x4{0.f, 0.f, 0.f, 0.f}; sb[u] = 0.f; }
    for (int b0 = 0; b0 < B; b0 += BCH) {
        const int nb = (B - b0 < BCH) ? B - b0 : BCH;
        __syncthreads();
        for (int e0 = 0; e0 < nb * JR; e0 += HT * 4) {
            float dv[4];
#pragma unroll
            for (int k = 0; k < 4; ++k) {
                int e = e0 + tid + k * HT; e = e < nb * JR ? e : nb * JR - 1;
                const int bb = e / JR, u = e - bb * JR;
                dv[k] = D[(size_t)(b0 + bb) * ldD + (row0 + u < nrows ? row0 + u : nrows - 1)];
            }
#pragma unroll
            for (int k = 0; k < 4; ++k) {
                const int e = e0 + tid + k * HT;
                if (e < nb * JR) { const int bb = e / JR, u = e - bb * JR; ds[bb][u] = (row0 + u < nrows) ? dv[k] : 0.f; }
            }
        }
        __syncthreads();
        const int per = (nb + HT / 64 - 1) / (HT / 64);
        const int lo = wv * per, hi = (lo + per < nb) ? lo + per : nb;
        constexpr int NB = 16;
        for (int bb = lo; bb < hi; bb += NB) {
            f32x4 av[NB];
#pragma unroll
            for (int k = 0; k < NB; ++k) {
                const int b = bb + k < hi ? bb + k : hi - 1;
                av[k] = *reinterpret_cast<const f32x4*>(Ac + (size_t)(b0 + b) * ldA);
            }
#pragma unroll
            for (int k = 0; k < NB; ++k) {
                f32x4 d = *reinterpret_cast<const f32x4*>(&ds[bb + k < hi ? bb + k : hi - 1][0]);
                if (bb + k >= hi) d = f32x4{0.f, 0.f, 0.f, 0.f};
#pragma unroll
                for (int u = 0; u < JR; ++u) {
#pragma unroll
                    for (int e = 0; e < 4; ++e) acc[u][e] = fmaf(d[u], av[k][e], acc[u][e]);
                    sb[u] += d[u];
                }
            }
        }
    }
#pragma unroll
    for (int u = 0; u < JR; ++u) {
        *reinterpret_cast<f32x4*>(&ps[wv][u][i4]) = acc[u];
        if (lane == 0) pb[wv][u] = sb[u];
    }
    __syncthreads();
    for (int e = tid; e < JR * HMAX; e += HT) {
        const int u = e / HMAX, i = e - u * HMAX;
        if (i >= ncols || row0 + u >= nrows) continue;
        float v = 0.f;
#pragma unroll
        for (int k = 0; k < HT / 64; ++k) v += ps[k][u][i];
        out[(size_t)(row0 + u) * ncols + i] = v;
    }
    if (tid < JR && row0 + tid < nrows) {
        float v = 0.f;
#pragma unroll
        for (int k = 0; k < HT / 64; ++k) v += pb[k][tid];
        bias[row0 + tid] = v;
    }
}

__global__ __launch_bounds__(HT) void head_mlp_bwd_w_kernel(HeadB q) {
    const int n1 = (q.H1 + JR - 1) / JR;
    if ((int)blockIdx.x < n1) weight_rows(q.dz1, q.H1, q.H1, blockIdx.x * JR, q.a0, q.Hin, q.Hin, q.B, q.dW1, q.db1);
    else weight_rows(q.dz2, q.C, q.C, ((int)blockIdx.x - n1) * JR, q.a1, q.H1, q.H1, q.B, q.dW2, q.db2);
}

bool al16(const void* p) { return ((uintptr_t)p & 15) == 0; }
bool width_ok(int h) { return h >= 8 && h <= HMAX && (h & (h - 1)) == 0; }

}

#define S_ ((hipStream_t)stream)

extern "C" int dep_head_mlp_supported(int Hin, int H1, int C) { return width_ok(Hin) && width_ok(H1) && C >= 0 && C <= HC; }

extern "C" int dep_head_mlp_fwd(const float* x, const float* W1, const float* b1, const float* W2, const float* b2, float* a0,
                                float* z1, float* a1, float* z2, int B, int Hin, int H1, int C, float p, uint64_t seed,
                                uint32_t site0, uint32_t site1, int first_dropout, void* stream) {
    DEP_CHECK_ARG(x && W1 && b1 && z1 && a1 && B > 0 && p >= 0.f && p < 1.f);
    DEP_CHECK_ARG(C == 0 || (W2 && b2 && z2));
    DEP_CHECK_ARG(!(first_dropout && p > 0.f) || a0);
    if (!dep_head_mlp_supported(Hin, H1, C) || !al16(W1)) { dep_set_error("dep_head_mlp_fwd: shape not covered (see dep_head_mlp_supported)"); return DEP_ERR_ARG; }
    HeadF q{x, W1, b1, W2, b2, a0, z1, a1, z2, B, Hin, H1, C, p, 1.0f / (1.0f - p), seed, site0, site1, first_dropout};
    const dim3 g(dep_cdiv(B, HR)), b(HT);
    switch (Hin / 8) {
        case 1: DEP_LAUNCH(head_mlp_fwd_kernel<1>, g, b, 0, S_, q); break;
        case 2: DEP_LAUNCH(head_mlp_fwd_kernel<2>, g, b, 0, S_, q); break;
        case 4: DEP_LAUNCH(head_mlp_fwd_kernel<4>, g, b, 0, S_, q); break;
        case 8: DEP_LAUNCH(head_mlp_fwd_kernel<8>, g, b, 0, S_, q); break;
        case 16: DEP_LAUNCH(head_mlp_fwd_kernel<16>, g, b, 0, S_, q); break;
        default: DEP_LAUNCH(head_mlp_fwd_kernel<32>, g, b, 0, S_, q); break;
    }
    DEP_CHECK_LAUNCH();
    return DEP_OK;
}

extern "C" int dep_head_mlp_bwd(const float* dz2, const float* a0, const float* z1, const float* a1, const float* W1,
                                const float* W2, float* dW1, float* db1, float* dW2, float* db2, float* dx, float* dz1, int B,
                                int Hin, int H1, int C, float p, uint64_t seed, uint32_t site0, uint32_t site1,
                                int first_dropout, void* stream) {
    DEP_CHECK_ARG(dz2 && a0 && z1 && a1 && W1 && W2 && dW1 && db1 && dW2 && db2 && dz1 && B > 0 && C > 0 && p >= 0.f && p < 1.f);
    if (!dep_head_mlp_supported(Hin, H1, C) || !al16(W1) || !al16(a0) || !al16(a1)) {
        dep_set_error("dep_head_mlp_bwd: shape not covered (see dep_head_mlp_supported)"); return DEP_ERR_ARG;
    }
    HeadB q{dz2, a0, z1, a1, W1, W2, dW1, db1, dW2, db2, dx, dz1, B, Hin, H1, C, p, 1.0f / (1.0f - p), seed, site0, site1, first_dropout};
    const dim3 g(dep_cdiv(B, HR)), b(HT);
    switch (H1 / 8) {
        case 1: DEP_LAUNCH(head_mlp_bwd_rows_kernel<1>, g, b, 0, S_, q); break;
        case 2: DEP_LAUNCH(head_mlp_bwd_rows_kernel<2>, g, b, 0, S_, q); break;
        case 4: DEP_LAUNCH(head_mlp_bwd_rows_kernel<4>, g, b, 0, S_, q); break;
        case 8: DEP_LAUNCH(head_mlp_bwd_rows_kernel<8>, g, b, 0, S_, q); break;
        case 16: DEP_LAUNCH(head_mlp_bwd_rows_kernel<16>, g, b, 0, S_, q); break;
        default: DEP_LAUNCH(head_mlp_bwd_rows_kernel<32>, g, b, 0, S_, q); break;
    }
    DEP_LAUNCH(head_mlp_bwd_w_kernel, dim3(dep_cdiv(H1, JR) + dep_cdiv(C, JR)), b, 0, S_, q);
    DEP_CHECK_LAUNCH();
    return DEP_OK;
}
```

### icassp2022-depression_amd/csrc/rnn_cluster.hip

```cpp
#include <algorithm>
#include "rnn_cluster_launch.h"

using namespace depc;

namespace {

__global__ void pack_cluster_bwd_kernel(const float* __restrict__ W, float* __restrict__ out, int G, int H) {
    const long n = (long)G * H * H;
    const long idx = (long)blockIdx.x * blockDim.x + threadIdx.x;
    if (idx >= n) return;
    const int e = idx & 3, l = (idx >> 2) & 63;
    const long blk = idx >> 8;
    const int KCB = G * 2;
    const int kc = blk % KCB; const long r = blk / KCB;
    const int jt = r % (H / 16); const int c = r / (H / 16);
    const int k = kc * 16 + (l >> 4) * 4 + e;
    const int g = k / 32, u = k % 32;
    out[idx] = W[(size_t)(g * H + 32 * c + u) * H + jt * 16 + (l & 15)];
}

}

const ClusterSwitches& depc::cluster_switches() {
    static const ClusterSwitches sw = [] {
        ClusterSwitches w;
        const char* e = getenv("DEP_CLUSTER_NOFAST"); w.nofast = (e && e[0] == '1') ? 1 : 0;
        e = getenv("DEP_TRACE"); w.trace = e && e[0] == '1';
        e = getenv("DEP_NUM_CUS");
        int dev = 0, v = 0;
        if (e && atoi(e) > 0) w.num_cus = atoi(e);
        else if (hipGetDevice(&dev) == hipSuccess && hipDeviceGetAttribute(&v, hipDeviceAttributeMultiprocessorCount, dev) == hipSuccess && v > 0) w.num_cus = v;
        else w.num_cus = 256;
        e = getenv("DEP_FORCE_SOFT_FALLBACK"); w.force_soft = (e && e[0] >= '1' && e[0] <= '3') ? e[0] - '0' : 0;
        return w;
    }();
    return sw;
}

int dep_cluster_chunk(int members, int per_cu, int max_wgs) {
    long wgs = (long)cluster_switches().num_cus * per_cu;
    if (wgs > max_wgs) wgs = max_wgs;
    long tiles = wgs / members;
    if (tiles >= 8) tiles = tiles / 8 * 8;
    if (tiles < 1) tiles = 1;
    return (int)tiles * BT;
}

bool dep_cluster_ok(int cell, int H, int, int) {
    return cell == DEP_CELL_GRU && (H == 64 || H == 128 || H == 256 || H == 512);
}

size_t dep_cluster_xbuf_bytes(int cell, int H, int B, int dirs) {
    if (!dep_cluster_ok(cell, H, B, dirs)) return 0;
    const ChunkGeometry g32 = gru32_geometry(H, B), g16 = gru16_geometry(H, B);
    const size_t fwd = std::max(gru_fwd_payload_bytes(g32, H), gru_fwd_payload_bytes(g16, H));
    return PAYLOAD_OFF + std::max(fwd, 8192 + 2 * gru_bwd_payload_bytes(g32, H));
}

int dep_cluster_reset_status(void* xbuf, hipStream_t s) {
    if (hipMemsetAsync(xbuf, 0, PAYLOAD_OFF, s) != hipSuccess) { dep_set_error("hipMemsetAsync failed"); return DEP_ERR_HIP; }
    return DEP_OK;
}
int dep_cluster_reset_flags(void* xbuf, hipStream_t s) {
    if (hipMemsetAsync((char*)xbuf + FLAG_OFF, 0, PAYLOAD_OFF - FLAG_OFF, s) != hipSuccess) { dep_set_error("hipMemsetAsync failed"); return DEP_ERR_HIP; }
    return DEP_OK;
}

int dep_pack_cluster_bwd(const float* w_hh, float* out, int G, int H, hipStream_t s) {
    const long n = (long)G * H * H;
    DEP_LAUNCH(pack_cluster_bwd_kernel, dim3(dep_cdiv(n, 256)), dim3(256), 0, s, w_hh, out, G, H);
    DEP_CHECK_LAUNCH();
    return DEP_OK;
}
```

### icassp2022-depression_amd/csrc/rnn_cluster_bwd.hip

```cpp
#include "rnn_cluster_launch.h"

namespace {
using namespace depc;

constexpr size_t EXCLUSIVE_LDS = 84 * 1024;
#define DEP_STAMP(slot) do { if (tr && t >= 100 && t < 104) tr[(t - 100) * 8 + (slot)] = (long long)__builtin_readcyclecounter(); } while (0)

struct P2 {
    int B, T, H, nbtp, b0;
    const f32x4* wp;
    const float* y; int ldy;
    const float* dy; int lddy;
    float drop_p, drop_scale; uint64_t seed; uint32_t site;
    const float* dpooled; float pool_scale;
    const float* dh_n;
    const float* sv0; const float* sv1; const float* sv2; const float* sv3;
    float* dgi; int lddg;
    float* dghn; int lddghn;
    float* dbpart;
    unsigned* status; unsigned* flags; unsigned* hello; float* payload; unsigned payload_bytes;
    int nofast;
    long long* trace;
    int trall_off;
    int dgpk;
// ... 678 lines not shown
        float2 hy = h;
        if constexpr (RAG) {
            const bool live = t < len;
            h = dep_sel2(live, h, hprev);
            hy = dep_sel2(live, h, f2(0.f, 0.f));
        }
        hprev = h; pool.x += hy.x; pool.y += hy.y;
        const unsigned epoch = (unsigned)t + 1u;
        const size_t pbase = (size_t)(t & 1) * pstride + tile_base;
        const bool more = t + 1 < T;
        DEP_STAMP(3);
        if (more) {
            const u64 bits = SPLIT ? ((u64)split_word(h.x) | ((u64)split_word(h.y) << 32))
                                   : ((u64)__float_as_uint(h.x) | ((u64)__float_as_uint(h.y) << 32));
            if (fast) __hip_atomic_store((gu64*)(p.payload + pbase + (size_t)j * H + col), bits, __ATOMIC_RELAXED, __HIP_MEMORY_SCOPE_WORKGROUP);
            else __hip_atomic_store((gu64*)(p.payload + pbase + (size_t)j * H + col), bits, __ATOMIC_RELAXED, __HIP_MEMORY_SCOPE_AGENT);
            asm volatile("s_waitcnt vmcnt(0)" ::: "memory");
            DEP_STAMP(4);
            __builtin_amdgcn_s_barrier();
            if (tid == 0) { if (fast) st_local(myflag, epoch); else st_agent(myflag, epoch); }
        }
        if (valid) {
            const size_t o = row * p.ldy + col;
            st2(p.y + o, hy);
            if (p.ydrop) {
                const f32x4 m = dep_dropmask4(p.seed, p.site, o >> 2, p.drop_p, p.drop_scale);
                st2(p.ydrop + o, f2(hy.x * (kh ? m[2] : m[0]), hy.y * (kh ? m[3] : m[1])));
            }
            if (p.sv0) {
                const size_t so = row * H + col;
                if (p.sv16) {
                    *reinterpret_cast<unsigned*>(reinterpret_cast<unsigned short*>(p.sv0) + so) = pack_unorm2(r.x, r.y);
                    *reinterpret_cast<unsigned*>(reinterpret_cast<unsigned short*>(p.sv1) + so) = pack_unorm2(z.x, z.y);
                    *reinterpret_cast<unsigned*>(reinterpret_cast<unsigned short*>(p.sv2) + so) = pack_snorm2(n.x, n.y);
                } else { st2(p.sv0 + so, r); st2(p.sv1 + so, z); st2(p.sv2 + so, n); }
                st2(p.sv3 + so, hn);
            }
        }
        if (more) {
            if (!wait_flags(tflags, NC, epoch, p.status, 4)) return;
            DEP_STAMP(5);
            DEP_STAMP(6);
            constexpr int PER = KCH / 2;
#pragma unroll
            for (int k = 0; k < PER; ++k) {
                const int i4 = (tid + CT * k) * 4;
                const u32x4 v = __builtin_amdgcn_raw_buffer_load_b128(rsrc, (unsigned)((pbase + i4) * 4), 0, 16 );
                if constexpr (SPLIT) {
                    const int o = (i4 >> hshift) * LDHB + (i4 & (H - 1));
                    uint2 hi2, lo2;
                    hi2.x = (v.x >> 16) | (v.y & 0xffff0000u); hi2.y = (v.z >> 16) | (v.w & 0xffff0000u);
                    lo2.x = (v.x & 0xffffu) | (v.y << 16);      lo2.y = (v.z & 0xffffu) | (v.w << 16);
                    *reinterpret_cast<uint2*>(hs_hi + o) = hi2; *reinterpret_cast<uint2*>(hs_lo + o) = lo2;
                } else {
                    f32x4 f;
                    f[0] = __uint_as_float(v.x); f[1] = __uint_as_float(v.y); f[2] = __uint_as_float(v.z); f[3] = __uint_as_float(v.w);
                    *reinterpret_cast<f32x4*>(hs + (i4 >> hshift) * LDH + (i4 & (H - 1))) = f;
                }
            }
            bar_lds();
            DEP_STAMP(7);
        }
    }
    if (valid) {
        const float ps = RAG ? dep_ragged_pool_scale(p.pool_mean, len, T, p.pool_scale) : p.pool_scale;
        if (p.pooled) st2(p.pooled + (size_t)b * H + col, f2(pool.x * ps, pool.y * ps));
        if (p.h_n) st2(p.h_n + (size_t)b * H + col, hprev);
    }
}

__global__ void pack_cluster_bwd_split_kernel(const float* __restrict__ W, u32x4* __restrict__ out, int H) {
    const long n = pack_bwd_split_pieces(3, H);
    const long idx = (long)blockIdx.x * blockDim.x + threadIdx.x;
    if (idx >= n) return;
    pack_bwd_split_piece<3>(W, out, H, idx);
}
__global__ void pack_cluster_fwd_split_kernel(const float* __restrict__ W, u32x4* __restrict__ out, int H) {
    const long n = pack_fwd_split_pieces(3, H);
    const long idx = (long)blockIdx.x * blockDim.x + threadIdx.x;
    if (idx >= n) return;
    pack_fwd_split_piece<3>(W, out, H, idx);
}

struct PackJobs { const float* src[8]; u32x4* dst[8]; int bwd[8]; int n; };
__global__ void pack_cluster_split_multi_kernel(PackJobs j, int H) {
    const int k = blockIdx.y;
    if (k >= j.n) return;
    const long idx = (long)blockIdx.x * blockDim.x + threadIdx.x;
    const float* W = j.src[k]; u32x4* out = j.dst[k];
    if (j.bwd[k]) {
        if (idx >= pack_bwd_split_pieces(3, H)) return;
        pack_bwd_split_piece<3>(W, out, H, idx);
    } else {
        if (idx >= pack_fwd_split_pieces(3, H)) return;
        pack_fwd_split_piece<3>(W, out, H, idx);
    }
}

Instance<F2>& fwd_instance(int H, bool split, bool rag) {
    static Instance<F2> rows[4][2] = {
        { DEP_INSTANCE((gru_fwd_cluster_r1<2, false>), EXCLUSIVE_LDS), DEP_INSTANCE((gru_fwd_cluster_r1<2, true>), EXCLUSIVE_LDS) },
        { DEP_INSTANCE((gru_fwd_cluster_r1<4, false>), EXCLUSIVE_LDS), DEP_INSTANCE((gru_fwd_cluster_r1<4, true>), EXCLUSIVE_LDS) },
        { DEP_INSTANCE((gru_fwd_cluster_r1<8, false>), EXCLUSIVE_LDS), DEP_INSTANCE((gru_fwd_cluster_r1<8, true>), EXCLUSIVE_LDS) },
        { DEP_INSTANCE((gru_fwd_cluster_r1<16, false>), EXCLUSIVE_LDS), DEP_INSTANCE((gru_fwd_cluster_r1<16, true>), EXCLUSIVE_LDS) } };
    static Instance<F2> ragged[4][2] = {
        { DEP_INSTANCE((gru_fwd_cluster_r1<2, false, true>), EXCLUSIVE_LDS), DEP_INSTANCE((gru_fwd_cluster_r1<2, true, true>), EXCLUSIVE_LDS) },
        { DEP_INSTANCE((gru_fwd_cluster_r1<4, false, true>), EXCLUSIVE_LDS), DEP_INSTANCE((gru_fwd_cluster_r1<4, true, true>), EXCLUSIVE_LDS) },
        { DEP_INSTANCE((gru_fwd_cluster_r1<8, false, true>), EXCLUSIVE_LDS), DEP_INSTANCE((gru_fwd_cluster_r1<8, true, true>), EXCLUSIVE_LDS) },
        { DEP_INSTANCE((gru_fwd_cluster_r1<16, false, true>), EXCLUSIVE_LDS), DEP_INSTANCE((gru_fwd_cluster_r1<16, true, true>), EXCLUSIVE_LDS) } };
    return (rag ? ragged : rows)[H == 64 ? 0 : H == 128 ? 1 : H == 256 ? 2 : 3][split];
}

constexpr int bwd_burst(int H) { return H >= 512 ? 0 : 4; }
Instance<P2>& bwd_instance(int H, bool split, bool sv16, bool bf16st, bool rag) {
    constexpr size_t R1 = EXCLUSIVE_LDS + 2048, AG = burst_lds_bytes_ag(4) + 2048;
    constexpr size_t BURST = (burst_lds_bytes(4) > EXCLUSIVE_LDS ? burst_lds_bytes(4) : EXCLUSIVE_LDS) + 2048;
    static Instance<P2> h64[3] = { DEP_INSTANCE((gru_bwd_cluster_r1<1, false, 4, false>), BURST), DEP_INSTANCE((gru_bwd_cluster_r1<1, true, 4, true>), BURST),
                                   DEP_INSTANCE((gru_bwd_cluster_r1<1, true, 4, false>), BURST) };
    static Instance<P2> h128[3] = { DEP_INSTANCE((gru_bwd_cluster_r1<2, false, 4, false>), BURST), DEP_INSTANCE((gru_bwd_cluster_r1<2, true, 4, true>), BURST),
                                    DEP_INSTANCE((gru_bwd_cluster_r1<2, true, 4, false>), BURST) };
    static Instance<P2> h256_exact DEP_INSTANCE((gru_bwd_cluster_r1<4, false, 4, false>), BURST);
    static Instance<P2> h512[3] = { DEP_INSTANCE((gru_bwd_cluster_r1<8, false, 0>), R1), DEP_INSTANCE((gru_bwd_cluster_r1<8, true, 0, true>), R1),
                                    DEP_INSTANCE((gru_bwd_cluster_r1<8, true, 0>), R1) };
    static Instance<P2> h256_ag[3] = { DEP_INSTANCE((gru_bwd_cluster_r1<4, true, 4, false, false, true>), AG), DEP_INSTANCE((gru_bwd_cluster_r1<4, true, 4, true, false, true>), AG),
                                       DEP_INSTANCE((gru_bwd_cluster_r1<4, true, 4, true, true, true>), AG) };
    const int form = !split ? 0 : sv16 ? 1 : 2;
    if (rag) {
        static Instance<P2> r64[3] = { DEP_INSTANCE((gru_bwd_cluster_r1<1, false, 4, false, false, false, true>), BURST), DEP_INSTANCE((gru_bwd_cluster_r1<1, true, 4, true, false, false, true>), BURST),
                                       DEP_INSTANCE((gru_bwd_cluster_r1<1, true, 4, false, false, false, true>), BURST) };
        static Instance<P2> r128[3] = { DEP_INSTANCE((gru_bwd_cluster_r1<2, false, 4, false, false, false, true>), BURST), DEP_INSTANCE((gru_bwd_cluster_r1<2, true, 4, true, false, false, true>), BURST),
                                        DEP_INSTANCE((gru_bwd_cluster_r1<2, true, 4, false, false, false, true>), BURST) };
        static Instance<P2> r256[3] = { DEP_INSTANCE((gru_bwd_cluster_r1<4, false, 4, false, false, false, true>), BURST), DEP_INSTANCE((gru_bwd_cluster_r1<4, true, 4, true, false, true, true>), AG),
                                        DEP_INSTANCE((gru_bwd_cluster_r1<4, true, 4, false, false, true, true>), AG) };
        static Instance<P2> r512[3] = { DEP_INSTANCE((gru_bwd_cluster_r1<8, false, 0, false, false, false, true>), R1), DEP_INSTANCE((gru_bwd_cluster_r1<8, true, 0, true, false, false, true>), R1),
                                        DEP_INSTANCE((gru_bwd_cluster_r1<8, true, 0, false, false, false, true>), R1) };
        return (H == 64 ? r64 : H == 128 ? r128 : H == 256 ? r256 : r512)[form];
    }
    switch (H) {
        case 64: return h64[form];
        case 128: return h128[form];
        case 256: return !split ? h256_exact : h256_ag[bf16st ? 2 : sv16 ? 1 : 0];
        default: return h512[form];
    }
}
}

int dep_pack_cluster_split_multi(int n, const float* const* src, float* const* dst, const int* bwd, int H, hipStream_t s) {
    DEP_CHECK_ARG(n > 0 && n <= 8 && src && dst && bwd);
    PackJobs j{};
    j.n = n;
    for (int k = 0; k < n; ++k) { DEP_CHECK_ARG(src[k] && dst[k]); j.src[k] = src[k]; j.dst[k] = (u32x4*)dst[k]; j.bwd[k] = bwd[k]; }
    const long nf = pack_fwd_split_pieces(3, H), nb = pack_bwd_split_pieces(3, H);
    DEP_LAUNCH(pack_cluster_split_multi_kernel, dim3(dep_cdiv(nf > nb ? nf : nb, 256), n), dim3(256), 0, s, j, H);
    DEP_CHECK_LAUNCH();
    return DEP_OK;
}

int dep_pack_cluster_fwd_split(const float* w_hh, float* out, int H, hipStream_t s) {
    DEP_LAUNCH(pack_cluster_fwd_split_kernel, dim3(dep_cdiv(pack_fwd_split_pieces(3, H), 256)), dim3(256), 0, s, w_hh, (u32x4*)out, H);
    DEP_CHECK_LAUNCH();
    return DEP_OK;
}

int dep_pack_cluster_bwd_split(const float* w_hh, float* out, int H, hipStream_t s) {
    DEP_LAUNCH(pack_cluster_bwd_split_kernel, dim3(dep_cdiv(pack_bwd_split_pieces(3, H), 256)), dim3(256), 0, s, w_hh, (u32x4*)out, H);
    DEP_CHECK_LAUNCH();
    return DEP_OK;
}

int dep_launch_cluster_fwd(const dep_sweep_args& a, void* xbuf, size_t xbuf_bytes) {
    DEP_CHECK_ARG(dep_cluster_ok(a.cell, a.H, a.B, a.dirs) && xbuf && xbuf_bytes >= dep_cluster_xbuf_bytes(a.cell, a.H, a.B, a.dirs));
    const ChunkGeometry g = gru32_geometry(a.H, a.B);
    F2 p{};
    p.B = a.B; p.T = a.T; p.H = a.H;
    p.wp = (const f32x4*)a.wp[0]; p.b_hh = a.b_hh[0];
    p.gi = a.gi; p.ldgi = 3 * a.H; p.y = a.y; p.ldy = a.ldy;
    p.ydrop = (a.drop_p > 0.f) ? a.ydrop : nullptr;
    p.drop_p = a.drop_p; p.drop_scale = a.drop_p > 0.f ? 1.0f / (1.0f - a.drop_p) : 1.0f; p.seed = a.seed; p.site = a.site;
    p.pooled = a.pooled; p.pool_scale = a.pool_scale; p.h_n = a.h_n;
    p.sv0 = a.training ? a.sv0 : nullptr; p.sv1 = a.sv1; p.sv2 = a.sv2; p.sv3 = a.sv3;
    const size_t pay = gru_fwd_payload_bytes(g, a.H);
    DEP_CHECK_ARG(PAYLOAD_OFF + pay <= xbuf_bytes && g.resident());
    p.flags = bind_exchange(p, xbuf, a.hdr_slot, pay);
    p.only_if = a.only_if; p.sv16 = a.training ? a.sv16 : 0;
    p.lengths = a.lengths; p.pool_mean = a.pool_mean;
    DepProfScope prof(DEP_PROF_GRU_FWD, a.stream, a.only_if == nullptr);
    return launch_chunks(fwd_instance(a.H, a.split, a.lengths != nullptr), g, dim3(CT), p, a.stream, __PRETTY_FUNCTION__,
                         [&](int b0) { return hdr_prepare(xbuf, a.hdr_slot, a.hdr_clean && b0 == 0, a.stream); });
}

bool dep_cluster_bwd_pk_ok(int H, int T) { return H <= 256 && T % 2 == 0; }

int dep_launch_cluster_bwd(const dep_sweep_bwd_args& a, void* xbuf, size_t xbuf_bytes) {
    DEP_CHECK_ARG(dep_cluster_ok(a.cell, a.H, a.B, a.dirs) && xbuf && xbuf_bytes >= dep_cluster_xbuf_bytes(a.cell, a.H, a.B, a.dirs));
    const ChunkGeometry g = gru32_geometry(a.H, a.B);
    const int nbt = dep_cdiv(a.B, BT);
    P2 p{};
    p.B = a.B; p.T = a.T; p.H = a.H;
    p.wp = (const f32x4*)a.wpT[0];
    p.y = a.y; p.ldy = a.ldy; p.dy = a.dy; p.lddy = a.lddy;
    p.drop_p = a.dy ? a.drop_p : 0.f; p.drop_scale = a.drop_p > 0.f ? 1.0f / (1.0f - a.drop_p) : 1.0f;
    p.seed = a.seed; p.site = a.site;
    p.dpooled = a.dpooled; p.pool_scale = a.pool_scale; p.dh_n = a.dh_n;
    p.sv0 = a.sv0; p.sv1 = a.sv1; p.sv2 = a.sv2; p.sv3 = a.sv3;
    p.dgi = a.dgi; p.lddg = a.lddg ? a.lddg : 3 * a.H; p.dghn = a.dghn; p.lddghn = a.lddghn ? a.lddghn : a.H; p.dbpart = a.dbpart;
    p.dgpk = a.dg_pk;
    p.lengths = a.lengths; p.pool_mean = a.pool_mean;
    DEP_CHECK_ARG(!(a.lengths && a.bf16st));
    DEP_CHECK_ARG(!a.sv16 || a.split);
    DEP_CHECK_ARG(!a.bf16st || (a.H == 256 && a.split && a.sv16 && a.dg_pk));
    DEP_CHECK_ARG(a.dbpart_rows >= nbt);
    const size_t pay = gru_bwd_payload_bytes(g, a.H);
    DEP_CHECK_ARG(PAYLOAD_OFF + pay <= xbuf_bytes && g.resident());
    p.flags = bind_exchange(p, xbuf, a.hdr_slot, pay);
    DepProfScope prof(DEP_PROF_GRU_BWD, a.stream);
    { const int mxl = p.lddg > p.lddy ? p.lddg : p.lddy; DEP_CHECK_ARG((size_t)(BT * a.T + 1) * (mxl > p.ldy ? mxl : p.ldy) * 4 < 0xffffffffull); }
    const int kb = bwd_burst(a.H);
    Instance<P2>& k = bwd_instance(a.H, a.split, a.sv16, a.bf16st, a.lengths != nullptr);
    p.trall_off = (int)((k.lds - 2048) / 4);
    if (p.dgpk) {
        DEP_CHECK_ARG(kb == 4 && a.split && a.T % 2 == 0 && a.lddg == 4 * a.H && a.lddghn == 4 * a.H && a.dghn == a.dgi + 3 * a.H);
    }
    return launch_chunks(k, g, dim3(kb ? CT + SVC_THREADS : CT), p, a.stream, __PRETTY_FUNCTION__,
                         [&](int b0) { return hdr_prepare(xbuf, a.hdr_slot, a.hdr_clean && b0 == 0, a.stream); });
}
```

### icassp2022-depression_amd/csrc/rnn_fused2_bwd.hip

```cpp
#include "rnn_cluster_launch.h"

namespace {
using namespace depc;

constexpr int BH = 256, BNC = 8, BTHREADS = 768;
constexpr int N_IBUF = 11, N_OBUF = 8;
constexpr unsigned L1_MEMBER = 8 * 1024, L0_MEMBER = 6 * 1024;
constexpr int N_RED = 3 * 4 * 2 * 256;
constexpr int IARR = BT * 32;
constexpr int gate_arr(bool sv16) { return sv16 ? IARR / 2 : IARR; }
constexpr int hid_arr(bool bf) { return bf ? IARR / 2 : IARR; }
constexpr int ipar_floats(bool sv16, bool hasdy, bool bf = false) { return 2 * (3 * gate_arr(sv16) + 2 * hid_arr(bf)) + (hasdy ? IARR : 0); }
constexpr int iarr_off(int a, bool sv16, bool hasdy, bool bf = false) {
    const int n1 = hasdy ? 6 : 5, l1sz = 3 * gate_arr(sv16) + 2 * hid_arr(bf) + (hasdy ? IARR : 0);
    const int k = a < n1 ? a : a - n1;
    return (a < n1 ? 0 : l1sz) + (k < 3 ? k * gate_arr(sv16) : 3 * gate_arr(sv16) + (k - 3 < 2 ? (k - 3) * hid_arr(bf) : 2 * hid_arr(bf)));
}
constexpr int pf_dist(bool sv16, bool hasdy) { return (sv16 && !hasdy) ? 2 : 1; }
constexpr size_t fb_lds_bytes(bool sv16, bool hasdy, bool pk, bool bf = false) {
    return (size_t)(2 * N_RED + (pf_dist(sv16, hasdy) + 1) * ipar_floats(sv16, hasdy, bf) + ((pk ? 3 : 2) * N_OBUF + 8 + 2) * IARR + 64 + 192) * sizeof(float);
}

struct FB {
    int B, T, nbtp, b0;
// ... 349 lines not shown
        else { flush(tid, T); flush(tid, T + 1); }
    }
    if (grp != 1) {
        float2 a[4];
        {
            const int lt0 = tid & 255, lp0 = (lt0 >> 1) & 63, j0 = lp0 & 15, ul0 = (lt0 >> 7) * 16 + (lp0 >> 4) * 4 + 2 * (lt0 & 1);
            const float* da = dbl + (grp == 0 ? 0 : 4) * IARR + j0 * 32 + (((ul0 >> 2) ^ (j0 & 7)) << 2) + (ul0 & 3);
            const bool rowok = b0t + j0 < p.B;
#pragma unroll
            for (int k = 0; k < 4; ++k) a[k] = rowok ? ld2(da + k * IARR) : f2(0.f, 0.f);
        }
#pragma unroll
        for (int k = 0; k < 4; ++k)
#pragma unroll
            for (int m = 2; m <= 16; m <<= 1) { a[k].x += __shfl_xor(a[k].x, m, 64); a[k].y += __shfl_xor(a[k].y, m, 64); }
        const int lt = tid & 255, lp = (lt >> 1) & 63, half = lt & 1;
        const int col = c * 32 + (lt >> 7) * 16 + (lp >> 4) * 4 + 2 * half;
        if ((lp & 15) == 0) {
            float* o = (grp == 0 ? p.dbpart1 : p.dbpart0) + (size_t)(p.b0 / BT + bt) * 4 * BH;
            st2(o + col, a[0]); st2(o + BH + col, a[1]); st2(o + 2 * BH + col, a[2]); st2(o + 3 * BH + col, a[3]);
        }
    }
}

#define FB_ROW(D, Y, S, P) DEP_INSTANCE((gru2_bwd_fused<D, Y, S, P>), fb_lds_bytes(S, Y, P))
#define FB_ROWS(S, P) { { FB_ROW(true, true, S, P), FB_ROW(true, false, S, P) }, { FB_ROW(false, true, S, P), FB_ROW(false, false, S, P) } }
#define FB_ROW_BF(D, Y) DEP_INSTANCE((gru2_bwd_fused<D, Y, true, true, false, true>), fb_lds_bytes(true, Y, true, true))
Instance<FB>& bwd_instance(bool drop, bool hasdy, bool sv16, bool pk, bool bf, bool trace) {
    static Instance<FB> rows[3][2][2] = { FB_ROWS(false, false), FB_ROWS(true, false), FB_ROWS(true, true) };
    static Instance<FB> bf16st[2][2] = { { FB_ROW_BF(true, true), FB_ROW_BF(true, false) }, { FB_ROW_BF(false, true), FB_ROW_BF(false, false) } };
    static Instance<FB> stamped[2] = { DEP_INSTANCE((gru2_bwd_fused<true, false, true, true, true>), fb_lds_bytes(true, false, true)),
                                       DEP_INSTANCE((gru2_bwd_fused<false, false, true, true, true>), fb_lds_bytes(true, false, true)) };
    if (bf) return bf16st[!drop][!hasdy];
    if (trace && pk && !hasdy) return stamped[!drop];
    return rows[pk ? 2 : sv16 ? 1 : 0][!drop][!hasdy];
}
#undef FB_ROW_BF
#undef FB_ROWS
#undef FB_ROW

ChunkGeometry fused2_bwd_geometry(int B) { return chunk_geometry(BNC, 1, 256, B); }
size_t fused2_bwd_payload_bytes(int nbtp) { return (size_t)nbtp * BNC * (3 * L1_MEMBER + 2 * L0_MEMBER); }

}

bool dep_fused2_bwd_fits(int B, int T) { return (size_t)B * T * BH * sizeof(float) * 8 < 0xfffffff0ull; }

size_t dep_fused2_bwd_xbuf_bytes(int B) { return PAYLOAD_OFF + fused2_bwd_payload_bytes(fused2_bwd_geometry(B).nbtp_max) + 4096; }

int dep_launch_fused2_bwd(const dep_fused2_bwd_args& a, void* xbuf, size_t xbuf_bytes) {
    const ChunkGeometry g = fused2_bwd_geometry(a.B);
    const int nbt = dep_cdiv(a.B, BT);
    FB p{};
    p.B = a.B; p.T = a.T;
    p.wh1 = (const u32x4*)a.wh1; p.wi1 = (const u32x4*)a.wi1; p.wh0 = (const u32x4*)a.wh0;
    p.y1 = a.y1; p.y0 = a.y0; p.sv1 = a.sv1; p.sv0 = a.sv0; p.svstride = (unsigned)a.svstride;
    p.dy = a.dy; p.dpooled = a.dpooled; p.pool_scale = a.pool_scale; p.dhn1 = a.dhn1; p.dhn0 = a.dhn0;
    const bool drop = a.drop_p > 0.f;
    p.drop_p = a.drop_p; p.drop_scale = drop ? 1.0f / (1.0f - a.drop_p) : 1.0f; p.seed = a.seed; p.site = a.site;
    p.dgi1 = a.dgi1; p.dghn1 = a.dghn1; p.dgi0 = a.dgi0; p.dghn0 = a.dghn0; p.dbpart1 = a.dbpart1; p.dbpart0 = a.dbpart0;
    p.lddg = a.lddg ? a.lddg : 3 * BH; p.lddghn = a.lddghn ? a.lddghn : BH;
    DEP_CHECK_ARG(!a.dg_pk || (p.lddg == 4 * BH && a.dghn1 == a.dgi1 + 3 * BH && a.dghn0 == a.dgi0 + 3 * BH));
    DEP_CHECK_ARG(a.dbpart_rows >= nbt && a.wh1 && a.wi1 && a.wh0 && a.dgi1 && a.dgi0 && a.dghn1 && a.dghn0);
    static_assert(DEP_HDR_SLOTS >= 2, "the fused backward keeps layer 0's flags in header slot 1");
    p.flags1 = bind_exchange(p, xbuf, 0, 0);
    p.flags0 = hdr_words(xbuf, 1, FLAG_OFF);
    {
        const size_t arr = (size_t)a.B * a.T * BH * sizeof(float);
        auto span = [&](const float* y, const float* sv, const char*& base, unsigned& bytes, unsigned& oy, unsigned& osv) {
            const char* cy = (const char*)y; const char* cs = (const char*)sv;
            base = cy < cs ? cy : cs;
            const char* e1 = cy + arr; const char* e2 = cs + (size_t)3 * a.svstride * sizeof(float) + arr;
            const size_t n = (size_t)((e1 > e2 ? e1 : e2) - base);
            oy = (unsigned)(cy - base); osv = (unsigned)(cs - base); bytes = (unsigned)n;
            return n < 0xfffffff0ull;
        };
        DEP_CHECK_ARG(span(a.y1, a.sv1, p.sb1, p.sbytes1, p.o_y1, p.o_sv1) && span(a.y0, a.sv0, p.sb0, p.sbytes0, p.o_y0, p.o_sv0));
        DEP_CHECK_ARG(arr < 0xfffffff0ull);
    }
    const bool sv16 = a.sv16 != 0, pk = a.dg_pk != 0, bf = a.bf16st != 0;
    DEP_CHECK_ARG(!bf || (sv16 && pk));
    DEP_CHECK_ARG(!pk || (sv16 && a.T % 2 == 0 && (size_t)a.B * a.T * 4 * BH * 4 < 0xfffffff0ull));
    DepProfScope prof(DEP_PROF_GRU_BWD, a.stream);
    return launch_chunks(bwd_instance(drop, a.dy != nullptr, sv16, pk, bf, p.trace != nullptr), g, dim3(BTHREADS), p, a.stream, __PRETTY_FUNCTION__, [&](int) -> int {
        const size_t pay = fused2_bwd_payload_bytes(p.nbtp);
        DEP_CHECK_ARG(xbuf && PAYLOAD_OFF + pay <= xbuf_bytes && g.resident() && pay < (1ull << 32));
        p.payload_bytes = (unsigned)pay; p.l0_off = (unsigned)((size_t)3 * p.nbtp * BNC * L1_MEMBER);
        if (const int rc = hdr_prepare(xbuf, 0, false, a.stream)) return rc;
        return hdr_prepare(xbuf, 1, false, a.stream);
    });
}
```

### icassp2022-depression_amd/csrc/rnn_sweep.hip

```cpp
#include "dep_common.h"

namespace {

constexpr int BT = 16;
constexpr int LPAD = 4;

struct DirP {
    const f32x4* wp;
    const float* w;
    const float* b_hh;
};

struct FwdP {
    int B, T, H, dirs;
    DirP d[2];
    const float* gi; int ldgi;
    float* y; int ldy;
    float* ydrop; float drop_p, drop_scale; uint64_t seed; uint32_t site;
    float* pooled; float pool_scale;
    float* h_n;
    float* sv0; float* sv1; float* sv2; float* sv3;
    const int* lengths; int pool_mean;
};

// ... 555 lines not shown
    if (p.h_n) for (int i = threadIdx.x; i < H; i += GEN_T) p.h_n[((size_t)dir * p.B + b) * H + i] = hs[i];
}

template <bool RAG = false>
__global__ __launch_bounds__(GEN_T) void lstm_bwd_generic(BwdP p) {
    extern __shared__ __attribute__((aligned(16))) float smem[];
    const int H = p.H, T = p.T, b = blockIdx.x, dir = blockIdx.y, G4 = 4 * H;
    const int len = RAG ? dep_row_len(p.lengths, b, T) : T;
    float* dg = smem; float* dh = smem + G4; float* dc = smem + G4 + H;
    const float* W = p.d[dir].w;
    const int ldsg = p.dirs * 4 * H, ldsc = p.dirs * H;
    float* dbp = p.dbpart + ((size_t)dir * p.nwg + b) * 4 * H;
    for (int i = threadIdx.x; i < H; i += GEN_T) {
        dh[i] = p.dh_n ? p.dh_n[((size_t)dir * p.B + b) * H + i] : 0.f;
        dc[i] = 0.f;
    }
    for (int i = threadIdx.x; i < 4 * H; i += GEN_T) dbp[i] = 0.f;
    __syncthreads();
    for (int s = T - 1; s >= 0; --s) {
        const int t = dir ? (T - 1 - s) : s;
        const size_t row = (size_t)b * T + t;
        for (int i = threadIdx.x; i < H; i += GEN_T) {
            const float* gs = p.sv0 + row * ldsg + dir * 4 * H;
            const float ig = gs[i], fg = gs[H + i], gg = gs[2 * H + i], og = gs[3 * H + i];
            const float ct = p.sv1[row * ldsc + dir * H + i];
            float cp = 0.f;
            if (s > 0) { const size_t rowp = dir ? row + 1 : row - 1; cp = p.sv1[rowp * ldsc + dir * H + i]; }
            float d = dh[i];
            if (p.dy) {
                const size_t o = row * p.lddy + dir * H + i;
                float dyv = p.dy[o];
                if (p.drop_p > 0.f) dyv *= dep_dropmask1(p.seed, p.site, o, p.drop_p, p.drop_scale);
                d += dyv;
            }
            const float tc = tanhf(ct);
            if constexpr (RAG) {
                if (t >= len) {
                    dg[i] = 0.f; dg[H + i] = 0.f; dg[2 * H + i] = 0.f; dg[3 * H + i] = 0.f;
                    float* g0 = p.dgi + row * p.lddg + dir * 4 * H;
                    g0[i] = 0.f; g0[H + i] = 0.f; g0[2 * H + i] = 0.f; g0[3 * H + i] = 0.f;
                    continue;
                }
            }
            const float dog = d * tc * og * (1.0f - og);
            const float dct = d * og * (1.0f - tc * tc) + dc[i];
            const float dig = dct * gg * ig * (1.0f - ig);
            const float dfg = dct * cp * fg * (1.0f - fg);
            const float dgg = dct * ig * (1.0f - gg * gg);
            dc[i] = dct * fg;
            dg[i] = dig; dg[H + i] = dfg; dg[2 * H + i] = dgg; dg[3 * H + i] = dog;
            float* g = p.dgi + row * p.lddg + dir * 4 * H;
            g[i] = dig; g[H + i] = dfg; g[2 * H + i] = dgg; g[3 * H + i] = dog;
            dbp[i] += dig; dbp[H + i] += dfg; dbp[2 * H + i] += dgg; dbp[3 * H + i] += dog;
        }
        __syncthreads();
        for (int i = threadIdx.x; i < H; i += GEN_T) {
            float sum = 0.f;
            for (int k = 0; k < G4; ++k) sum = fmaf(dg[k], W[(size_t)k * H + i], sum);
            if (!RAG || t < len) dh[i] = sum;
        }
        __syncthreads();
    }
}

__global__ void pack_whh_kernel(const float* __restrict__ W, float* __restrict__ wp, float* __restrict__ wpT, int G, int H) {
    const long n = (long)G * H * H;
    const long idx = (long)blockIdx.x * blockDim.x + threadIdx.x;
    if (idx >= n) return;
    const int e = idx & 3, l = (idx >> 2) & 63;
    const long blk = idx >> 8;
    {
        const int KC = H / 16;
        const int kc = blk % KC; const long tg = blk / KC;
        const int g = tg % G; const int jt = tg / G;
        wp[idx] = W[(size_t)(g * H + jt * 16 + (l & 15)) * H + kc * 16 + (l >> 4) * 4 + e];
    }
    if (wpT) {
        const int KC2 = G * H / 16;
        const int kc = blk % KC2; const int jt = blk / KC2;
        wpT[idx] = W[(size_t)(kc * 16 + (l >> 4) * 4 + e) * H + jt * 16 + (l & 15)];
    }
}

__global__ void finish_db_kernel(const float* __restrict__ part, int nrows, int H, int G, int cell,
                                 float* db_ih, float* db_hh) {
    const int i = blockIdx.x * blockDim.x + threadIdx.x;
    if (i >= 4 * H) return;
    float s = 0.f;
    int r = 0;
    for (; r + 8 <= nrows; r += 8) {
        float v[8];
#pragma unroll
        for (int k = 0; k < 8; ++k) v[k] = part[(size_t)(r + k) * 4 * H + i];
#pragma unroll
        for (int k = 0; k < 8; ++k) s += v[k];
    }
    for (; r < nrows; ++r) s += part[(size_t)r * 4 * H + i];
    const int g = i / H, c = i % H;
    if (cell == DEP_CELL_GRU) {
        if (g < 2) { db_ih[g * H + c] = s; db_hh[g * H + c] = s; }
        else if (g == 2) db_ih[2 * H + c] = s;
        else db_hh[2 * H + c] = s;
    } else {
        db_ih[i] = s; db_hh[i] = s;
    }
}

int pick_jpw(int H, int* nw) {
    if (H % 16) return 0;
    const int tiles = H / 16;
    for (int w = 8; w >= 1; w >>= 1) {
        if (tiles % w == 0 && tiles / w <= 4) { *nw = w; return tiles / w; }
    }
    return 0;
}

}

bool dep_sweep_use_mfma(int H, int impl) {
    if (impl == 1) return false;
    int nw; const int jpw = pick_jpw(H, &nw);
    if (!jpw) return false;
    return (size_t)2 * BT * (4 * H + LPAD) * sizeof(float) <= 160 * 1024;
}

int dep_sweep_num_wg(int B, int H, int impl) { return dep_sweep_use_mfma(H, impl) ? dep_cdiv(B, BT) : B; }

size_t dep_pack_floats(int G, int H) { return (size_t)G * H * H; }

int dep_pack_whh(const float* w_hh, float* wp, float* wpT, int G, int H, hipStream_t s) {
    const long n = (long)G * H * H;
    DEP_LAUNCH(pack_whh_kernel, dim3(dep_cdiv(n, 256)), dim3(256), 0, s, w_hh, wp, wpT, G, H);
    DEP_CHECK_LAUNCH();
    return DEP_OK;
}

#define LAUNCH_JPW(kern, grid, nthr, lds, s, P)                                                    \
    do {                                                                                           \
        if (P.lengths) {                                                                           \
            switch (jpw) {                                                                         \
                case 1: (void)hipFuncSetAttribute((const void*)kern<1, true>, hipFuncAttributeMaxDynamicSharedMemorySize, (int)(lds)); \
                        DEP_LAUNCH((kern<1, true>), grid, dim3(nthr), lds, s, P); break;           \
                case 2: (void)hipFuncSetAttribute((const void*)kern<2, true>, hipFuncAttributeMaxDynamicSharedMemorySize, (int)(lds)); \
                        DEP_LAUNCH((kern<2, true>), grid, dim3(nthr), lds, s, P); break;           \
                case 3: (void)hipFuncSetAttribute((const void*)kern<3, true>, hipFuncAttributeMaxDynamicSharedMemorySize, (int)(lds)); \
                        DEP_LAUNCH((kern<3, true>), grid, dim3(nthr), lds, s, P); break;           \
                default: (void)hipFuncSetAttribute((const void*)kern<4, true>, hipFuncAttributeMaxDynamicSharedMemorySize, (int)(lds)); \
                        DEP_LAUNCH((kern<4, true>), grid, dim3(nthr), lds, s, P); break;           \
            }                                                                                      \
        } else                                                                                     \
        switch (jpw) {                                                                             \
            case 1: (void)hipFuncSetAttribute((const void*)kern<1>, hipFuncAttributeMaxDynamicSharedMemorySize, (int)(lds)); \
                    DEP_LAUNCH(kern<1>, grid, dim3(nthr), lds, s, P); break;               \
            case 2: (void)hipFuncSetAttribute((const void*)kern<2>, hipFuncAttributeMaxDynamicSharedMemorySize, (int)(lds)); \
                    DEP_LAUNCH(kern<2>, grid, dim3(nthr), lds, s, P); break;               \
            case 3: (void)hipFuncSetAttribute((const void*)kern<3>, hipFuncAttributeMaxDynamicSharedMemorySize, (int)(lds)); \
                    DEP_LAUNCH(kern<3>, grid, dim3(nthr), lds, s, P); break;               \
            default: (void)hipFuncSetAttribute((const void*)kern<4>, hipFuncAttributeMaxDynamicSharedMemorySize, (int)(lds)); \
                    DEP_LAUNCH(kern<4>, grid, dim3(nthr), lds, s, P); break;               \
        }                                                                                          \
    } while (0)

#define LAUNCH_JPW_BI_CASE(kern, J, RAG, grid, nthr, lds, s, P)                                    \
    (void)hipFuncSetAttribute((const void*)kern<J, RAG, true>, hipFuncAttributeMaxDynamicSharedMemorySize, (int)(lds)); \
    DEP_LAUNCH((kern<J, RAG, true>), grid, dim3(nthr), lds, s, P); break
#define LAUNCH_JPW_BI(kern, grid, nthr, lds, s, P)                                                 \
    do {                                                                                           \
        if (P.lengths) {                                                                           \
            switch (jpw) {                                                                         \
                case 1: LAUNCH_JPW_BI_CASE(kern, 1, true, grid, nthr, lds, s, P);                  \
                case 2: LAUNCH_JPW_BI_CASE(kern, 2, true, grid, nthr, lds, s, P);                  \
                case 3: LAUNCH_JPW_BI_CASE(kern, 3, true, grid, nthr, lds, s, P);                  \
                default: LAUNCH_JPW_BI_CASE(kern, 4, true, grid, nthr, lds, s, P);                 \
            }                                                                                      \
        } else                                                                                     \
        switch (jpw) {                                                                             \
            case 1: LAUNCH_JPW_BI_CASE(kern, 1, false, grid, nthr, lds, s, P);                     \
            case 2: LAUNCH_JPW_BI_CASE(kern, 2, false, grid, nthr, lds, s, P);                     \
            case 3: LAUNCH_JPW_BI_CASE(kern, 3, false, grid, nthr, lds, s, P);                     \
            default: LAUNCH_JPW_BI_CASE(kern, 4, false, grid, nthr, lds, s, P);                    \
        }                                                                                          \
    } while (0)

int dep_launch_sweep_fwd(const dep_sweep_args& a) {
    const int G = a.cell == DEP_CELL_GRU ? 3 : 4;
    FwdP p{};
    p.B = a.B; p.T = a.T; p.H = a.H; p.dirs = a.dirs;
    for (int d = 0; d < a.dirs; ++d) { p.d[d].wp = (const f32x4*)a.wp[d]; p.d[d].w = a.w_hh[d]; p.d[d].b_hh = a.b_hh[d]; }
    p.gi = a.gi; p.ldgi = a.dirs * G * a.H; p.y = a.y; p.ldy = a.ldy;
    p.ydrop = (a.drop_p > 0.f) ? a.ydrop : nullptr;
    p.drop_p = a.drop_p; p.drop_scale = a.drop_p > 0.f ? 1.0f / (1.0f - a.drop_p) : 1.0f; p.seed = a.seed; p.site = a.site;
    p.pooled = a.pooled; p.pool_scale = a.pool_scale; p.h_n = a.h_n;
    p.sv0 = a.training ? a.sv0 : nullptr; p.sv1 = a.sv1; p.sv2 = a.sv2; p.sv3 = a.sv3;
    p.lengths = a.lengths; p.pool_mean = a.pool_mean;
    DEP_CHECK_ARG(a.y && a.gi);
    const bool bigru = a.cell == DEP_CELL_GRU && a.dirs == 2;
    DEP_CHECK_ARG(!bigru || dep_sweep_use_mfma(a.H, a.impl));
    DepProfScope prof(a.cell == DEP_CELL_GRU ? DEP_PROF_GRU_FWD : DEP_PROF_LSTM_FWD, a.stream);
    if (dep_sweep_use_mfma(a.H, a.impl)) {
        int nw = 0; const int jpw = pick_jpw(a.H, &nw);
        const size_t lds = (size_t)2 * BT * (a.H + LPAD) * sizeof(float);
        dim3 grid(dep_cdiv(a.B, BT), a.dirs);
        if (bigru) LAUNCH_JPW_BI(gru_fwd_mfma, grid, nw * 64, lds, a.stream, p);
        else if (a.cell == DEP_CELL_GRU) LAUNCH_JPW(gru_fwd_mfma, grid, nw * 64, lds, a.stream, p);
        else LAUNCH_JPW(lstm_fwd_mfma, grid, nw * 64, lds, a.stream, p);
    } else {
        dim3 grid(a.B, a.dirs);
        const size_t lds = (size_t)3 * a.H * sizeof(float);
        if (a.lengths) {
            if (a.cell == DEP_CELL_GRU) DEP_LAUNCH(gru_fwd_generic<true>, grid, dim3(GEN_T), lds, a.stream, p);
            else DEP_LAUNCH(lstm_fwd_generic<true>, grid, dim3(GEN_T), lds, a.stream, p);
        } else if (a.cell == DEP_CELL_GRU) DEP_LAUNCH(gru_fwd_generic<>, grid, dim3(GEN_T), lds, a.stream, p);
        else DEP_LAUNCH(lstm_fwd_generic<>, grid, dim3(GEN_T), lds, a.stream, p);
    }
    DEP_CHECK_LAUNCH();
    return DEP_OK;
}

int dep_launch_sweep_bwd(const dep_sweep_bwd_args& a) {
    const int G = a.cell == DEP_CELL_GRU ? 3 : 4;
    BwdP p{};
    p.B = a.B; p.T = a.T; p.H = a.H; p.dirs = a.dirs;
    for (int d = 0; d < a.dirs; ++d) { p.d[d].wp = (const f32x4*)a.wpT[d]; p.d[d].w = a.w_hh[d]; p.d[d].b_hh = nullptr; }
    p.y = a.y; p.ldy = a.ldy; p.dy = a.dy; p.lddy = a.lddy;
    p.drop_p = a.dy ? a.drop_p : 0.f; p.drop_scale = a.drop_p > 0.f ? 1.0f / (1.0f - a.drop_p) : 1.0f;
    p.seed = a.seed; p.site = a.site;
    p.dpooled = a.dpooled; p.pool_scale = a.pool_scale; p.dh_n = a.dh_n;
    p.sv0 = a.sv0; p.sv1 = a.sv1; p.sv2 = a.sv2; p.sv3 = a.sv3;
    p.dgi = a.dgi; p.lddg = a.dirs * G * a.H; p.dghn = a.dghn; p.dbpart = a.dbpart;
    p.nwg = dep_sweep_num_wg(a.B, a.H, a.impl);
    p.lengths = a.lengths; p.pool_mean = a.pool_mean;
    DEP_CHECK_ARG(a.dbpart_rows >= p.nwg * a.dirs);
    DEP_CHECK_ARG(a.sv0 && a.dgi && a.dbpart);
    const bool bigru = a.cell == DEP_CELL_GRU && a.dirs == 2;
    DEP_CHECK_ARG(!bigru || dep_sweep_use_mfma(a.H, a.impl));
    DepProfScope prof(a.cell == DEP_CELL_GRU ? DEP_PROF_GRU_BWD : DEP_PROF_LSTM_BWD, a.stream);
    if (dep_sweep_use_mfma(a.H, a.impl)) {
        int nw = 0; const int jpw = pick_jpw(a.H, &nw);
        const size_t lds = (size_t)2 * BT * (G * a.H + LPAD) * sizeof(float);
        dim3 grid(dep_cdiv(a.B, BT), a.dirs);
        if (bigru) LAUNCH_JPW_BI(gru_bwd_mfma, grid, nw * 64, lds, a.stream, p);
        else if (a.cell == DEP_CELL_GRU) LAUNCH_JPW(gru_bwd_mfma, grid, nw * 64, lds, a.stream, p);
        else LAUNCH_JPW(lstm_bwd_mfma, grid, nw * 64, lds, a.stream, p);
    } else {
        dim3 grid(a.B, a.dirs);
        const size_t lds = (size_t)(G * a.H + 2 * a.H) * sizeof(float);
        if (a.lengths) {
            if (a.cell == DEP_CELL_GRU) DEP_LAUNCH(gru_bwd_generic<true>, grid, dim3(GEN_T), lds, a.stream, p);
            else DEP_LAUNCH(lstm_bwd_generic<true>, grid, dim3(GEN_T), lds, a.stream, p);
        } else if (a.cell == DEP_CELL_GRU) DEP_LAUNCH(gru_bwd_generic<>, grid, dim3(GEN_T), lds, a.stream, p);
        else DEP_LAUNCH(lstm_bwd_generic<>, grid, dim3(GEN_T), lds, a.stream, p);
    }
    DEP_CHECK_LAUNCH();
    return DEP_OK;
}

int dep_finish_db(const dep_sweep_bwd_args& a, float* const* db_ih, float* const* db_hh) {
    const int G = a.cell == DEP_CELL_GRU ? 3 : 4;
    DEP_CHECK_ARG(a.dirs >= 1 && a.dbpart_rows >= a.dirs && a.dbpart_rows % a.dirs == 0);
    const int nwg = a.dbpart_rows / a.dirs;
    for (int d = 0; d < a.dirs; ++d) {
        DEP_LAUNCH(finish_db_kernel, dim3(dep_cdiv(4 * a.H, 128)), dim3(128), 0, a.stream,
                           a.dbpart + (size_t)d * nwg * 4 * a.H, nwg, a.H, G, a.cell, db_ih[d], db_hh[d]);
        DEP_CHECK_LAUNCH();
    }
    return DEP_OK;
}
```

### icassp2022-depression_amd/models.py

```python
from __future__ import annotations

import numpy as np
import torch

from . import _lib as L
from . import nn
from . import parallel


def _rnn_names(prefix, F, H, Lyr, dirs, G):
    out = []
    for l in range(Lyr):
        for d in range(dirs):
            s = f'l{l}' + ('_reverse' if d else '')
            inp = F if l == 0 else H * dirs
            out += [(f'{prefix}.weight_ih_{s}', (G * H, inp)), (f'{prefix}.weight_hh_{s}', (G * H, H)),
                    (f'{prefix}.bias_ih_{s}', (G * H,)), (f'{prefix}.bias_hh_{s}', (G * H,))]
    return out


class _RnnCache:

    def __init__(self, cell, F, H, Lyr, dirs, p, pool, device):
        self.args = (cell, F, H, Lyr, dirs, p, pool, device)
# ... 100 lines not shown
        L.gemm(1, 0, H, Hin, B, dz1, H, a0, Hin, W1._grad, Hin)
        L.colsum(dz1, P[self.n1 + '.bias']._grad)
        dx = torch.empty_like(a0)
        L.gemm(0, 0, B, Hin, H, dz1, H, W1.data, Hin, dx, Hin)
        if self.first and p > 0:
            L.dropout(dx, dx, p, seed, self.sites[0])
        return dx


class AudioGRU(nn.Module):
    def __init__(self, config, variant='clf', seed=None):
        super().__init__()
        self.variant = variant
        self.num_classes = config['num_classes']; self.learning_rate = config['learning_rate']
        self.dropout = float(config['dropout']); self.hidden_dims = H = config['hidden_dims']
        self.rnn_layers = Lyr = config['rnn_layers']; self.embedding_size = F = config['embedding_size']
        self.bidirectional = config.get('bidirectional', False)
        if self.bidirectional:
            raise L.DepError('AudioBiLSTM: the reference runs a unidirectional GRU (bidirectional=False)')
        gen = nn.make_generator(seed)
        init = {}
        self._add('attention_layer.0.weight', (H, H), live=False); self._add('attention_layer.0.bias', (H,), live=False)
        init.update(nn.default_linear_init('attention_layer.0.weight', 'attention_layer.0.bias', H, H, gen))
        rn = _rnn_names('lstm_net_audio', F, H, Lyr, 1, 3)
        for n, s in rn:
            self._add(n, s)
        init.update(nn.default_rnn_init(rn, H, gen))
        self._buffers = {}
        if variant == 'clf':
            self._add('ln.weight', (F,)); self._add('ln.bias', (F,))
            init['ln.weight'] = np.ones(F, np.float32); init['ln.bias'] = np.zeros(F, np.float32)
        else:
            self._add('bn.weight', (3,), live=False); self._add('bn.bias', (3,), live=False)
            init['bn.weight'] = np.ones(3, np.float32); init['bn.bias'] = np.zeros(3, np.float32)
            self._buffers = {'bn.running_mean': torch.zeros(3), 'bn.running_var': torch.ones(3),
                             'bn.num_batches_tracked': torch.zeros((), dtype=torch.long)}
        self._add('fc_audio.1.weight', (H, H)); self._add('fc_audio.1.bias', (H,))
        self._add('fc_audio.4.weight', (self.num_classes, H)); self._add('fc_audio.4.bias', (self.num_classes,))
        init.update(nn.default_linear_init('fc_audio.1.weight', 'fc_audio.1.bias', H, H, gen))
        init.update(nn.default_linear_init('fc_audio.4.weight', 'fc_audio.4.bias', self.num_classes, H, gen))
        self._finalize(init)
        self._rnn_w = [self._params[n].data for n, _ in rn]
        self._rnn_g = [self._params[n]._grad for n, _ in rn]
        if variant == 'clf':
            mk = lambda *shape: torch.empty(*shape, dtype=torch.float32, device=self.device)
            self._fold = (mk(3 * H, F), mk(3 * H), mk(3 * H, F), mk(3 * H))
            self._rnn_w_fold = [self._fold[0], self._rnn_w[1], self._fold[1]] + self._rnn_w[3:]
            self._rnn_g_fold = [self._fold[2], self._rnn_g[1], self._fold[3]] + self._rnn_g[3:]
        pool = L.POOL_MEAN if variant == 'clf' else L.POOL_SUM
        self._rnns = _RnnCache(L.CELL_GRU, F, H, Lyr, 1, self.dropout, pool, self.device)
        self._head = _MLPHead(self, 'fc_audio.1', 'fc_audio.4', self.dropout, True, (L.SITE_FC0, L.SITE_FC1))

    def state_dict(self):
        sd = super().state_dict()
        if self._buffers:
            out = type(sd)()
            for k, v in sd.items():
                out[k] = v
                if k == 'bn.bias':
                    out.update(self._buffers)
            return out
        return sd

    def load_state_dict(self, sd, strict=True):
        sd = {k: v for k, v in sd.items() if k not in self._buffers}
        return super().load_state_dict(sd, strict)

    def check_health(self):
        self._rnns.check()

    def status_words(self):
        w = self._rnns.status_word()
        return [] if w is None else [w]

    def fallback_words(self):
        w = self._rnns.fallback_word()
        return [] if w is None else [w]

    def encode(self, x, training, seed, lengths=None):
        B, T, F = x.shape
        P = self._params
        if self.variant == 'clf':
            xn, _ = L.layernorm_fwd(x.view(B * T, F), None, None, save=False)
            L.ln_fold_fwd(self._rnn_w[0], self._rnn_w[2], P['ln.weight'].data, P['ln.bias'].data, *self._fold[:2])
            weights = self._rnn_w_fold
        else:
            xn, weights = x.view(B * T, F), self._rnn_w
        rnn = self._rnns.get(B, T, training)
        pooled = torch.empty(B, self.hidden_dims, dtype=torch.float32, device=self.device)
        rnn.forward(xn, weights, seed=seed, pooled=pooled, lengths=lengths)
        return pooled, (x, xn, rnn, lengths)

    def forward(self, x, lengths=None):
        x = self._to_dev(x)
        lengths = _RnnCache.lengths_on(lengths, x.shape[0], self.device)
        training = self.training
        seed = nn.next_dropout_seed() if training else 0
        pooled, enc = self.encode(x, training, seed, lengths)
        z = self._head.forward(pooled, seed, training)
        out = torch.empty_like(z)
        kind = L.LOSS_CE_ON_SOFTMAX if self.variant == 'clf' else L.LOSS_L1_RELU
        L.head_loss(kind, z, None, out, None, None, 1.0)
        self._saved = enc
        return nn.Output(out, self, z)

    def sync_plan(self):
        Lyr, px = self.rnn_layers, 'lstm_net_audio'
        in_call, post = {}, []
        for l in range(Lyr):
            first, last = f'{px}.weight_ih_l{l}', ('fc_audio.4.bias' if l == Lyr - 1 else f'{px}.bias_hh_l{l}')
            if l == 0 and self.variant == 'clf':
                post.append(self._span('ln.weight', last))
            else:
                in_call[l] = self._span(first, last)
        return in_call, post

    def backward(self, dz):
        x, xn, rnn, lengths = self._saved
        dpool = self._head.backward(dz)
        P = self._params
        in_call, post = self.sync_plan()
        gs = parallel.make_grad_sync(self, in_call)
        if self.variant == 'clf':
            rnn.backward(xn, self._rnn_w_fold, self._rnn_g_fold, dpooled=dpool, dx=None, grad_sync=gs, lengths=lengths)
            L.ln_fold_bwd(self._rnn_w[0], self._fold[2], self._fold[3], P['ln.weight'].data, P['ln.bias'].data,
                          self._rnn_g[0], self._rnn_g[2], P['ln.weight']._grad, P['ln.bias']._grad)
        else:
            rnn.backward(xn, self._rnn_w, self._rnn_g, dpooled=dpool, dx=None, grad_sync=gs, lengths=lengths)
        self._grad_ready = True
        parallel.finish_grad_sync(self, in_call, post)


class TextBiLSTM(nn.Module):
    def __init__(self, config, variant='clf', seed=None, head_out=True, fc_idx=None):
        super().__init__()
        self.variant = variant
        self.num_classes = config['num_classes']; self.learning_rate = config['learning_rate']
        self.dropout = float(config['dropout']); self.hidden_dims = H = config['hidden_dims']
        self.rnn_layers = Lyr = config['rnn_layers']; self.embedding_size = F = config['embedding_size']
        self.bidirectional = config.get('bidirectional', True)
        if not self.bidirectional:
            raise L.DepError('TextBiLSTM: the reference runs a bidirectional LSTM (bidirectional=True)')
        i1, i2 = fc_idx if fc_idx else ((0, 3) if variant == 'clf' else (1, 4))
        self._fc = (f'fc_out.{i1}', f'fc_out.{i2}')
        gen = nn.make_generator(seed)
        shapes = [('attention_layer.0.weight', (H, H)), ('attention_layer.0.bias', (H,))]
        rn = _rnn_names('lstm_net', F, H, Lyr, 2, 4)
        shapes += rn
        shapes += [(self._fc[0] + '.weight', (H, H)), (self._fc[0] + '.bias', (H,)),
                   (self._fc[1] + '.weight', (self.num_classes, H)), (self._fc[1] + '.bias', (self.num_classes,))]
        init = {}
        for n, s in shapes:
            self._add(n, s)
            init[n] = nn.xavier_uniform(s, gen) if 'weight' in n else np.zeros(s, np.float32)
        if variant == 'clf':
            for n, s in (('ln1.weight', (F,)), ('ln1.bias', (F,)), ('ln2.weight', (H,)), ('ln2.bias', (H,))):
                self._add(n, s, live=False)
                init[n] = np.ones(s, np.float32) if 'weight' in n else np.zeros(s, np.float32)
        self._finalize(init)
        self._rnn_w = [self._params[n].data for n, _ in rn]
        self._rnn_g = [self._params[n]._grad for n, _ in rn]
        self._rnns = _RnnCache(L.CELL_LSTM, F, H, Lyr, 2, self.dropout, L.POOL_NONE, self.device)
        self._head = _MLPHead(self, self._fc[0], self._fc[1], self.dropout, variant == 'reg', (L.SITE_FC0, L.SITE_FC1))

    def check_health(self):
        self._rnns.check()

    def status_words(self):
        w = self._rnns.status_word()
        return [] if w is None else [w]

    def fallback_words(self):
        w = self._rnns.fallback_word()
# ... 221 lines not shown
```

### include/dep_rnn.h

```cpp
#ifndef DEP_RNN_H
#define DEP_RNN_H

#include <stddef.h>
#include <stdint.h>

#ifdef __cplusplus
extern "C" {
#endif

typedef enum {
    DEP_OK = 0,
    DEP_ERR_ARG = -1,
    DEP_ERR_WORKSPACE = -2,
    DEP_ERR_HIP = -3
} dep_status;

const char* dep_last_error(void);
int dep_version(void);
const char* dep_arch(void);

enum { DEP_POOL_NONE = 0, DEP_POOL_MEAN = 1, DEP_POOL_SUM = 2 };
enum { DEP_CELL_GRU = 0, DEP_CELL_LSTM = 1 };
enum { DEP_RUN_EVAL = 0, DEP_RUN_TRAIN = 1, DEP_RUN_DROPOUT_ONLY = 2 };

// ... 12 lines not shown
size_t dep_rnn_reserve_bytes(const dep_rnn_desc* d);
size_t dep_rnn_workspace_bytes(const dep_rnn_desc* d);
size_t dep_rnn_reserve_y_offset(const dep_rnn_desc* d, int layer);
size_t dep_rnn_reserve_ydrop_offset(const dep_rnn_desc* d, int layer);

int dep_rnn_status(const dep_rnn_desc* d, void* workspace, void* stream);
size_t dep_rnn_workspace_xbuf_offset(const dep_rnn_desc* d);
int dep_rnn_set_exclusive(int on);
int dep_rnn_get_exclusive(void);

int dep_rnn_forward(const dep_rnn_desc* d, const float* x, const float* const* weights,
                    float* y, float* pooled, float* h_n,
                    void* reserve, size_t reserve_bytes, void* workspace, size_t workspace_bytes,
                    void* stream);

int dep_rnn_backward(const dep_rnn_desc* d, const float* x, const float* const* weights,
                     const float* dy, const float* dpooled, const float* dh_n,
                     float* const* dweights, float* dx,
                     void* reserve, size_t reserve_bytes, void* workspace, size_t workspace_bytes,
                     void* stream);

int dep_rnn_forward_varlen(const dep_rnn_desc* d, const float* x, const int32_t* lengths, const float* const* weights,
                           float* y, float* pooled, float* h_n,
                           void* reserve, size_t reserve_bytes, void* workspace, size_t workspace_bytes,
                           void* stream);
int dep_rnn_backward_varlen(const dep_rnn_desc* d, const float* x, const int32_t* lengths, const float* const* weights,
                            const float* dy, const float* dpooled, const float* dh_n,
                            float* const* dweights, float* dx,
                            void* reserve, size_t reserve_bytes, void* workspace, size_t workspace_bytes,
                            void* stream);

typedef struct dep_comm dep_comm;
int dep_comm_available(void);
int dep_comm_unique_id(void* id_out, size_t bytes);
int dep_comm_init(dep_comm** comm, int world, int rank, const void* unique_id, size_t id_bytes, int device);
int dep_comm_world(const dep_comm* comm);
int dep_comm_rank(const dep_comm* comm);
int dep_comm_allreduce(dep_comm* comm, float* buf, long n, void* stream);
int dep_comm_allreduce_ranges(dep_comm* comm, float* const* bufs, const long* counts, int nranges, void* stream);
int dep_comm_destroy(dep_comm* comm);

typedef struct {
    dep_comm* comm;
    void* comm_stream;
    float* range_ptr[8];
    long range_count[8];
} dep_grad_sync;
int dep_rnn_backward_overlapped(const dep_rnn_desc* d, const float* x, const float* const* weights,
                                const float* dy, const float* dpooled, const float* dh_n,
                                float* const* dweights, float* dx,
                                void* reserve, size_t reserve_bytes, void* workspace, size_t workspace_bytes,
                                void* stream, const dep_grad_sync* gs);

int dep_rnn_backward_overlapped_varlen(const dep_rnn_desc* d, const float* x, const int32_t* lengths, const float* const* weights,
                                       const float* dy, const float* dpooled, const float* dh_n,
                                       float* const* dweights, float* dx,
                                       void* reserve, size_t reserve_bytes, void* workspace, size_t workspace_bytes,
                                       void* stream, const dep_grad_sync* gs);

size_t dep_gemm_workspace_bytes(int transA, int transB, int M, int N, int K);
int dep_gemm_f32(int transA, int transB, int M, int N, int K,
                 const float* A, int lda, const float* B, int ldb, float* C, int ldc,
                 const float* bias, float beta, int seq_T, int shiftB,
                 void* workspace, size_t workspace_bytes, void* stream);

int dep_gemm_bf16x3(int transA, int transB, int M, int N, int K,
                    const float* A, int lda, const float* B, int ldb, float* C, int ldc,
                    const float* bias, float beta, int seq_T, int shiftB,
                    void* workspace, size_t workspace_bytes, void* stream);
int dep_gemm(int transA, int transB, int M, int N, int K,
             const float* A, int lda, const float* B, int ldb, float* C, int ldc,
             const float* bias, float beta, int seq_T, int shiftB,
             void* workspace, size_t workspace_bytes, void* stream);
int dep_gemm_set_xcds(int lo, int n);
int dep_set_gemm_mode(int mode, long min_macs);
int dep_get_gemm_mode(void);

int dep_layernorm_fwd(const float* x, const float* gamma, const float* beta, float* y,
                      float* mean_rstd, int rows, int F, float eps, void* stream);
int dep_ln_fold_fwd(const float* W, const float* b, const float* gamma, const float* beta,
                    float* Wf, float* bf, int J, int F, void* stream);
int dep_ln_fold_bwd(const float* W, const float* dWf, const float* dbf, const float* gamma, const float* beta,
                    float* dW, float* db, float* dgamma, float* dbeta, int J, int F, void* stream);
size_t dep_layernorm_bwd_workspace_bytes(int rows, int F);
int dep_layernorm_bwd(const float* dy, const float* x, const float* gamma, const float* mean_rstd,
                      float* dx, float* dgamma, float* dbeta, int rows, int F,
                      void* workspace, size_t workspace_bytes, void* stream);

int dep_attn_fwd(const float* out, const float* h_n, int K, const float* Wa, const float* ba,
                 float* ctx, float* alpha, float* pre, float* hsum, int B, int T, int H,
                 void* stream);
size_t dep_attn_bwd_workspace_bytes(int B, int T, int H);
int dep_attn_bwd(const float* dctx, const float* out, const float* Wa, const float* alpha,
                 const float* pre, const float* hsum, int K,
                 float* dout, float* dh_n, float* dWa, float* dba, int B, int T, int H,
                 void* workspace, size_t workspace_bytes, void* stream);

int dep_attn_fwd_varlen(const float* out, const int32_t* lengths, const float* h_n, int K, const float* Wa, const float* ba,
                        float* ctx, float* alpha, float* pre, float* hsum, int B, int T, int H,
                        void* stream);
int dep_attn_bwd_varlen(const float* dctx, const float* out, const int32_t* lengths, const float* Wa, const float* alpha,
                        const float* pre, const float* hsum, int K,
                        float* dout, float* dh_n, float* dWa, float* dba, int B, int T, int H,
                        void* workspace, size_t workspace_bytes, void* stream);

int dep_dropout(const float* x, float* y, long n, float p, uint64_t seed, uint32_t site, void* stream);
int dep_dropout_mask(float* mask, long n, float p, uint64_t seed, uint32_t site, void* stream);
int dep_relu_dropout_fwd(const float* z, float* a, long n, float p, uint64_t seed, uint32_t site, void* stream);
int dep_relu_dropout_bwd(const float* da, const float* z, float* dz, long n, float p, uint64_t seed,
                         uint32_t site, void* stream);
int dep_colsum(const float* x, int M, int N, int ld, float* out, void* stream);

enum { DEP_LOSS_CE_ON_SOFTMAX = 0, DEP_LOSS_L1_RELU = 1, DEP_LOSS_SMOOTHL1_RELU = 2, DEP_LOSS_CE_LOGITS = 3,
       DEP_LOSS_SMOOTHL1 = 4,
       DEP_LOSS_LABELS_I64 = 0x100  };
int dep_head_loss(int kind, const float* z, const void* target, float* out, float* loss_rows,
                  float* dz, int B, int C, float norm, void* stream);
int dep_reduce_loss(const float* loss_rows, int B, float norm, float* loss_out, int accumulate, void* stream);
int dep_head_loss_ce(int kind, const float* z, const void* target, const float* class_weight, float label_smoothing,
                     long long ignore_index, float* out, float* loss_rows, float* dz, int B, int C, float norm,
                     const float* norm_dev, void* stream);
int dep_ce_weight_sum(const void* target, int labels_i64, const float* class_weight, long long ignore_index, int B, int C,
                      float* den_out, void* stream);
int dep_reduce_loss_by(const float* loss_rows, int B, const float* norm_dev, float* loss_out, int accumulate, void* stream);

enum { DEP_REG_L1 = 0, DEP_REG_SMOOTHL1 = 1, DEP_REG_HUBER = 2, DEP_REG_MSE = 3 };
int dep_head_loss_reg(int form, int relu, float param, const float* z, const float* target, const float* row_weight,
                      float* out, float* loss_rows, float* dz, int B, int C, float norm, const float* norm_dev, void* stream);
int dep_row_weight_sum(const float* row_weight, int B, float scale, float* den_out, void* stream);

int dep_head_mlp_supported(int Hin, int H1, int C);
int dep_head_mlp_fwd(const float* x, const float* W1, const float* b1, const float* W2, const float* b2, float* a0,
                     float* z1, float* a1, float* z2, int B, int Hin, int H1, int C, float p, uint64_t seed,
                     uint32_t site0, uint32_t site1, int first_dropout, void* stream);
int dep_head_mlp_bwd(const float* dz2, const float* a0, const float* z1, const float* a1, const float* W1,
                     const float* W2, float* dW1, float* db1, float* dW2, float* db2, float* dx, float* dz1, int B,
                     int Hin, int H1, int C, float p, uint64_t seed, uint32_t site0, uint32_t site1, int first_dropout,
                     void* stream);

int dep_adam_step(float* p, const float* g, float* m, float* v, long n, float lr, float beta1,
                  float beta2, float eps, float weight_decay, int decoupled, int step, void* stream);

int dep_grad_norm_slots(void);
int dep_grad_norm_chunk(void);
int dep_grad_sqnorm(const float* const* bufs, const long* counts, int nranges, double* partials, void* stream);
int dep_adam_step_clipped(float* p, const float* g, float* m, float* v, long n, float lr, float beta1, float beta2,
                          float eps, float weight_decay, int decoupled, int step, const double* partials, float max_norm,
                          int skip_nonfinite, float* clip_out, double* stats, void* stream);
int dep_grad_clip_scale(float* const* bufs, const long* counts, int nranges, const double* partials, float max_norm,
                        float* clip_out, void* stream);

int dep_grad_accumulate(float* const* acc, const float* const* g, const long* counts, int nranges, float scale, int first,
                        double* partials, void* stream);

typedef struct {
    float* vmax;
    float* ema;
    float  ema_decay;
    int    ema_first;
} dep_adam_ext;
int dep_adam_step_ext(float* p, const float* g, float* m, float* v, long n, float lr, float beta1, float beta2, float eps,
                      float weight_decay, int decoupled, int step, const dep_adam_ext* ext,
                      const double* partials, float max_norm, int skip_nonfinite, float* clip_out, double* stats, void* stream);
int dep_swap(float* a, float* b, long n, void* stream);

int dep_frame_window(const float* y, long n, int n_fft, int hop, int n_frames, float* out, void* stream);
// ... 29 lines not shown
```

Before: 165,500 utterances/s.

## Fuse per-step setup kernels (weight packing, header zeroing, LN fold) into one launch

Gathers the small per-step setup work into a single multi-job kernel launch: weight image packing, cluster header zeroing, and the layernorm-fold of the first-layer weights. In the forward pass this replaces a separate ln_fold launch, a reset-status launch and the packing launch. The backward pass merges packing with slot zeroing and computes both layers' bias-gradient reductions in one launch. The aim is to cut kernel launch overhead and serialized tiny kernels in the train step. The cost is extra plumbing and a new ordering dependency, since the sweep kernels must see cleared headers from the combined launch.

```diff
diff --git a/icassp2022-depression_amd/_lib.py b/icassp2022-depression_amd/_lib.py
--- a/icassp2022-depression_amd/_lib.py
+++ b/icassp2022-depression_amd/_lib.py
@@ -30,6 +30,14 @@
 
 class GradSync(C.Structure):
     _fields_ = [('comm', _P), ('comm_stream', _P), ('range_ptr', _P * 8), ('range_count', C.c_long * 8)]
+
+
+class LnFold(C.Structure):
+    _fields_ = [('W', _P), ('b', _P), ('gamma', _P), ('beta', _P), ('Wf', _P), ('bf', _P)]
+
+
+class StepJob(C.Structure):
+    _fields_ = [('kind', C.c_int), ('region', C.c_int), ('offset', C.c_size_t), ('bytes', C.c_size_t)]
 
 
 _BWD_ARGS = [C.POINTER(RnnDesc), _P, C.POINTER(_P), _P, _P, _P, C.POINTER(_P), _P, _P, C.c_size_t, _P, C.c_size_t, _P]
@@ -50,6 +58,8 @@
     'dep_rnn_backward': (C.c_int, _BWD_ARGS),
     'dep_rnn_backward_overlapped': (C.c_int, _BWD_ARGS + [C.POINTER(GradSync)]),
     'dep_rnn_forward_varlen': (C.c_int, [C.POINTER(RnnDesc), _P, _P, C.POINTER(_P), _P, _P, _P, _P, C.c_size_t, _P, C.c_size_t, _P]),
+    'dep_rnn_forward_fold': (C.c_int, [C.POINTER(RnnDesc), _P, _P, C.POINTER(_P), C.POINTER(LnFold), _P, _P, _P, _P, C.c_size_t, _P, C.c_size_t, _P]),
+    'dep_rnn_step_jobs': (C.c_int, [C.POINTER(RnnDesc), C.c_int, C.c_int, C.POINTER(StepJob), C.c_int]),
     'dep_rnn_backward_varlen': (C.c_int, _BWD_VARLEN_ARGS),
     'dep_rnn_backward_overlapped_varlen': (C.c_int, _BWD_VARLEN_ARGS + [C.POINTER(GradSync)]),
     'dep_comm_available': (C.c_int, []),
@@ -578,10 +588,17 @@
         n = d.B * d.T * d.H * d.dirs
         return self.reserve[off:off + n].view(d.B, d.T, d.H * d.dirs)
 
-    def forward(self, x, weights, seed=0, pooled=None, h_n=None, y=None, lengths=None):
+    def forward(self, x, weights, seed=0, pooled=None, h_n=None, y=None, lengths=None, fold=None):
         for i, w in enumerate(weights):
             self._warr[i] = w.data_ptr()
         self.desc.seed = seed
+        if fold is not None:
+            f = LnFold(*[_ptr(t) for t in fold])
+            ln = None if lengths is None else _ptr(check_lengths(lengths, self.desc.B, self.device))
+            check(self.lib.dep_rnn_forward_fold(C.byref(self.desc), _ptr(x), ln, self._warr, C.byref(f), _ptr(y), _ptr(pooled), _ptr(h_n),
+                                                _ptr(self.reserve), self.reserve.numel() * 4, _ptr(self.workspace),
+                                                self.workspace.numel() * 4, stream()), 'dep_rnn_forward_fold')
+            return
         if lengths is not None:
             check(self.lib.dep_rnn_forward_varlen(C.byref(self.desc), _ptr(x), _ptr(check_lengths(lengths, self.desc.B, self.device)),
                                                   self._warr, _ptr(y), _ptr(pooled), _ptr(h_n), _ptr(self.reserve),
diff --git a/icassp2022-depression_amd/csrc/api.hip b/icassp2022-depression_amd/csrc/api.hip
--- a/icassp2022-depression_amd/csrc/api.hip
+++ b/icassp2022-depression_amd/csrc/api.hip
@@ -303,6 +303,7 @@
         e = getenv("DEP_DGI_PK"); w.dgi_pk = !(e && e[0] == '0');
         e = getenv("DEP_COMM_OVERLAP"); w.comm_beside_sweeps = e && e[0] == 's';
         e = getenv("DEP_EXCLUSIVE"); w.exclusive = !(e && e[0] == '0');
+        e = getenv("DEP_STEP_FUSE"); w.step_fuse = !(e && e[0] == '0');
         return w;
     }();
     return sw;
@@ -411,10 +412,60 @@
     return DEP_ERR_ARG;
 }
 
-}
-
-static int rnn_forward_impl(const dep_rnn_desc* d, const float* x, const int32_t* lengths, const float* const* weights, float* y,
-                            float* pooled, float* h_n, void* reserve, size_t reserve_bytes, void* workspace,
+constexpr int MAX_STEP_JOBS = 8;
+struct StepJob { dep_step_job j; int weight; };
+int build_step_jobs(const dep_rnn_desc* d, const Layout& lo, const RnnPlan& p, int phase, bool fold, StepJob* out) {
+    if (!dep_rnn_switches().step_fuse) return 0;
+    const size_t F4 = sizeof(float), img = (size_t)lo.G * d->H * d->H * F4;
+    int n = 0;
+    auto add = [&](int kind, int region, size_t off, size_t bytes, int weight) { out[n++] = StepJob{{kind, region, off, bytes}, weight}; };
+    if (phase == 0 && p.fwd == FWD_FUSED2) {
+        add(DEP_JOB_IMAGE_FWD, DEP_REGION_RESERVE, lo.wp[0][0] * F4, img, 1);
+        add(DEP_JOB_IMAGE_FWD, DEP_REGION_RESERVE, lo.wp[1][0] * F4, img, 5);
+        add(DEP_JOB_IMAGE_FWD, DEP_REGION_WORKSPACE, lo.wih_img * F4, img, 4);
+        if (p.whh_bwd == WHH_BWD_SPLIT) {
+            add(DEP_JOB_IMAGE_BWD, DEP_REGION_RESERVE, lo.wpT[0][0] * F4, img, 1);
+            add(DEP_JOB_IMAGE_BWD, DEP_REGION_RESERVE, lo.wpT[1][0] * F4, img, 5);
+        }
+        add(DEP_JOB_ZERO, DEP_REGION_WORKSPACE, lo.xbuf * F4, dep_cluster_header_bytes(), -1);
+        if (fold) add(DEP_JOB_LN_FOLD, DEP_REGION_CALLER, 0, ((size_t)lo.G * d->H * d->F + (size_t)lo.G * d->H) * F4, -1);
+    } else if (phase == 1 && p.bwd == BWD_FUSED2) {
+        add(DEP_JOB_IMAGE_BWD, DEP_REGION_WORKSPACE, lo.wih_img * F4, img, 4);
+        for (int slot = 0; slot < 2; ++slot) {
+            size_t off, bytes; dep_cluster_slot_words(slot, &off, &bytes);
+            add(DEP_JOB_ZERO, DEP_REGION_WORKSPACE, lo.xbuf * F4 + off, bytes, -1);
+        }
+    }
+    return n;
+}
+int launch_step_jobs(const StepJob* jobs, int n, const dep_rnn_desc* d, const Layout& lo, const float* const* weights, const dep_ln_fold* fold,
+                     float* R, float* W, hipStream_t s) {
+    const float* src[MAX_STEP_JOBS]; float* dst[MAX_STEP_JOBS]; int bwd[MAX_STEP_JOBS]; void* zero[2]; size_t zbytes[2];
+    int ni = 0, nz = 0; bool has_fold = false;
+    for (int k = 0; k < n; ++k) {
+        const dep_step_job& j = jobs[k].j;
+        char* at = (char*)(j.region == DEP_REGION_RESERVE ? R : W) + j.offset;
+        if (j.kind == DEP_JOB_ZERO) { DEP_CHECK_ARG(nz < 2); zero[nz] = at; zbytes[nz++] = j.bytes; }
+        else if (j.kind == DEP_JOB_LN_FOLD) has_fold = true;
+        else { src[ni] = weights[jobs[k].weight]; dst[ni] = (float*)at; bwd[ni++] = j.kind == DEP_JOB_IMAGE_BWD; }
+    }
+    return dep_step_jobs_launch(ni, src, dst, bwd, nz, zero, zbytes, has_fold ? fold : nullptr, lo.G * d->H, d->F, d->H, s);
+}
+
+}
+
+extern "C" int dep_rnn_step_jobs(const dep_rnn_desc* d, int phase, int with_fold, dep_step_job* jobs, int cap) {
+    Layout lo;
+    DEP_CHECK_ARG(make_layout(d, lo) && (phase == 0 || phase == 1) && (jobs || cap <= 0));
+    const RnnPlan p = make_plan(d, lo, dep_get_gemm_mode(), dep_exclusive_on(), false);
+    StepJob sj[MAX_STEP_JOBS];
+    const int n = build_step_jobs(d, lo, p, phase, with_fold != 0, sj);
+    for (int k = 0; k < n && k < cap; ++k) jobs[k] = sj[k].j;
+    return n;
+}
+
+static int rnn_forward_impl(const dep_rnn_desc* d, const float* x, const int32_t* lengths, const float* const* weights, const dep_ln_fold* fold,
+                            float* y, float* pooled, float* h_n, void* reserve, size_t reserve_bytes, void* workspace,
                             size_t workspace_bytes, void* stream) {
     Layout lo;
     if (const int rf = bigru_refusal(d, "dep_rnn_forward")) return rf;
@@ -436,7 +487,11 @@
     DepGemmOpts proj; proj.scratch = W + lo.gemm; proj.scratch_bytes = lo.gemm_bytes;
     float* const gi = W + lo.gi;
     int rc;
-    if (lo.cluster) { rc = dep_cluster_reset_status(W + lo.xbuf, s); if (rc) return rc; }
+    if (fold) DEP_CHECK_ARG(D == 1 && weights[0] == fold->Wf && weights[2] == fold->bf);
+    StepJob jobs[MAX_STEP_JOBS];
+    const int njobs = build_step_jobs(d, lo, p, 0, fold != nullptr, jobs);
+    if (fold && !njobs) { rc = dep_ln_fold_fwd(fold->W, fold->b, fold->gamma, fold->beta, fold->Wf, fold->bf, G * H, d->F, stream); if (rc) return rc; }
+    if (lo.cluster && !njobs) { rc = dep_cluster_reset_status(W + lo.xbuf, s); if (rc) return rc; }
     if (p.bf16st && (!p.excl || y)) {
         dep_set_error("dep_rnn_forward: bf16-storage mode (dep_set_gemm_mode(3)) runs the exclusive fused forward only (dep_rnn_set_exclusive(1)) "
                       "and has no fp32 copy of the output sequence (y must be NULL)");
@@ -474,7 +529,8 @@
     if (p.fwd == FWD_FUSED2) {
         const float* const* w0 = weights; const float* const* w1 = weights + 4;
         for (int k = 0; k < 4; ++k) DEP_CHECK_ARG(w0[k] && w1[k]);
-        {
+        if (njobs) { rc = launch_step_jobs(jobs, njobs, d, lo, weights, fold, R, W, s); if (rc) return rc; }
+        else {
             const float* srcs[5] = {w0[1], w1[1], w1[0], w0[1], w1[1]};
             float* dsts[5] = {R + lo.wp[0][0], R + lo.wp[1][0], W + lo.wih_img, R + lo.wpT[0][0], R + lo.wpT[1][0]};
             const int kinds[5] = {0, 0, 0, 1, 1};
@@ -573,14 +629,21 @@
 extern "C" int dep_rnn_forward(const dep_rnn_desc* d, const float* x, const float* const* weights, float* y,
                                float* pooled, float* h_n, void* reserve, size_t reserve_bytes, void* workspace,
                                size_t workspace_bytes, void* stream) {
-    return rnn_forward_impl(d, x, nullptr, weights, y, pooled, h_n, reserve, reserve_bytes, workspace, workspace_bytes, stream);
+    return rnn_forward_impl(d, x, nullptr, weights, nullptr, y, pooled, h_n, reserve, reserve_bytes, workspace, workspace_bytes, stream);
 }
 
 extern "C" int dep_rnn_forward_varlen(const dep_rnn_desc* d, const float* x, const int32_t* lengths, const float* const* weights,
                                       float* y, float* pooled, float* h_n, void* reserve, size_t reserve_bytes, void* workspace,
                                       size_t workspace_bytes, void* stream) {
     DEP_CHECK_ARG(lengths);
-    return rnn_forward_impl(d, x, lengths, weights, y, pooled, h_n, reserve, reserve_bytes, workspace, workspace_bytes, stream);
+    return rnn_forward_impl(d, x, lengths, weights, nullptr, y, pooled, h_n, reserve, reserve_bytes, workspace, workspace_bytes, stream);
+}
+
+extern "C" int dep_rnn_forward_fold(const dep_rnn_desc* d, const float* x, const int32_t* lengths, const float* const* weights,
+                                    const dep_ln_fold* fold, float* y, float* pooled, float* h_n, void* reserve, size_t reserve_bytes,
+                                    void* workspace, size_t workspace_bytes, void* stream) {
+    if (fold) DEP_CHECK_ARG(fold->W && fold->b && fold->gamma && fold->beta && fold->Wf && fold->bf);
+    return rnn_forward_impl(d, x, lengths, weights, fold, y, pooled, h_n, reserve, reserve_bytes, workspace, workspace_bytes, stream);
 }
 
 static int rnn_backward_impl(const dep_rnn_desc* d, const float* x, const int32_t* lengths, const float* const* weights, const float* dy,
@@ -634,8 +697,12 @@
         float* const* g0 = dweights; float* const* g1 = dweights + 4;
         for (int k = 0; k < 4; ++k) DEP_CHECK_ARG(w0[k] && w1[k] && g0[k] && g1[k]);
         fused_pk = p.sv16 && pk_ok(1, nullptr) && pk_ok(0, dx);
-        rc = dep_pack_cluster_bwd_split(w1[0], W + lo.wih_img, H, s); if (rc) return rc;
+        StepJob jobs[MAX_STEP_JOBS];
+        const int njobs = build_step_jobs(d, lo, p, 1, false, jobs);
+        rc = njobs ? launch_step_jobs(jobs, njobs, d, lo, weights, nullptr, R, W, s) : dep_pack_cluster_bwd_split(w1[0], W + lo.wih_img, H, s);
+        if (rc) return rc;
         dep_fused2_bwd_args f{};
+        f.hdr_clean = njobs ? 1 : 0;
         f.B = B; f.T = T;
         f.wh1 = R + lo.wpT[1][0]; f.wi1 = W + lo.wih_img; f.wh0 = R + lo.wpT[0][0];
         f.y1 = R + lo.y[1]; f.y0 = R + lo.y[0]; f.sv1 = R + lo.sv[1][0]; f.sv0 = R + lo.sv[0][0];
@@ -678,6 +745,11 @@
         a.lengths = lengths; a.pool_mean = d->pool == DEP_POOL_MEAN ? 1 : 0;
         return a;
     };
+    const bool db_both = fused && dep_rnn_switches().step_fuse;
+    if (db_both) {
+        rc = dep_finish_db2(sweep_args(1, fused_pk), dweights[4 + 2], dweights[4 + 3], sweep_args(0, fused_pk), dweights[2], dweights[3]);
+        if (rc) return rc;
+    }
     float* pending_ptr = nullptr; long pending_n = 0;
     if (lo.cluster && !fused) { rc = dep_cluster_reset_flags(W + lo.xbuf, s); if (rc) return rc; }
     for (int l = L - 1; l >= 0; --l) {
@@ -704,8 +776,7 @@
             DEP_CHECK_ARG(gl[0] && gl[1] && gl[2] && gl[3]);
             dbi[dd] = gl[2]; dbh[dd] = gl[3];
         }
-        rc = dep_finish_db(a, dbi, dbh);
-        if (rc) return rc;
+        if (!db_both) { rc = dep_finish_db(a, dbi, dbh); if (rc) return rc; }
         DepGemmOpts go; go.scratch = gws; go.scratch_bytes = gwsb;
         if (pk) go.fmt_a = p.pk_fmt;
         const bool stacked = D == 2 && lo.wstack[l] != 0;
diff --git a/icassp2022-depression_amd/csrc/dep_common.h b/icassp2022-depression_amd/csrc/dep_common.h
--- a/icassp2022-depression_amd/csrc/dep_common.h
+++ b/icassp2022-depression_amd/csrc/dep_common.h
@@ -58,6 +58,20 @@
 __device__ __forceinline__ float dep_dropmask1(uint64_t seed, uint32_t site, uint64_t idx, float p, float scale) {
     const f32x4 m = dep_dropmask4(seed, site, idx >> 2, p, scale);
     return m[idx & 3];
+}
+
+__device__ __forceinline__ void dep_ln_fold_fwd_row(const float* __restrict__ W, const float* __restrict__ b,
+                                                    const float* __restrict__ gamma, const float* __restrict__ beta,
+                                                    float* __restrict__ Wf, float* __restrict__ bf, int j, int F, int lane) {
+    float s = 0.f;
+    for (int f = lane; f < F; f += 64) {
+        const float w = W[(size_t)j * F + f];
+        Wf[(size_t)j * F + f] = w * gamma[f];
+        s = fmaf(w, beta[f], s);
+    }
+#pragma unroll
+    for (int m = 32; m >= 1; m >>= 1) s += __shfl_xor(s, m, 64);
+    if (lane == 0) bf[j] = b[j] + s;
 }
 
 __device__ __forceinline__ int dep_row_len(const int* lengths, int b, int T) { const int n = lengths[b]; return n < 0 ? 0 : (n > T ? T : n); }
@@ -121,6 +135,7 @@
     bool dgi_pk;
     bool comm_beside_sweeps;
     bool exclusive;
+    bool step_fuse;
 };
 const RnnSwitches& dep_rnn_switches();
 bool dep_prof_on();
@@ -194,6 +209,7 @@
 size_t dep_pack_floats(int G, int H);
 int dep_pack_whh(const float* w_hh, float* wp, float* wpT, int G, int H, hipStream_t s);
 int dep_finish_db(const dep_sweep_bwd_args& a, float* const* db_ih, float* const* db_hh);
+int dep_finish_db2(const dep_sweep_bwd_args& a, float* dbi_a, float* dbh_a, const dep_sweep_bwd_args& b, float* dbi_b, float* dbh_b);
 
 bool dep_cluster_ok(int cell, int H, int B, int dirs);
 size_t dep_cluster_xbuf_bytes(int cell, int H, int B, int dirs);
@@ -236,6 +252,7 @@
     int sv16;
     int bf16st;
     int dg_pk;
+    int hdr_clean;
     hipStream_t stream;
 };
 size_t dep_fused2_bwd_xbuf_bytes(int B);
@@ -245,9 +262,13 @@
 constexpr int DEP_HDR_SLOTS = 4;
 int dep_cluster_reset_status(void* xbuf, hipStream_t s);
 int dep_cluster_reset_flags(void* xbuf, hipStream_t s);
+size_t dep_cluster_header_bytes();
+void dep_cluster_slot_words(int slot, size_t* off, size_t* bytes);
 int dep_pack_cluster16_fwd_split(const float* w_hh, float* out, int H, hipStream_t s);
 int dep_pack_cluster_bwd_split(const float* w_hh, float* out, int H, hipStream_t s);
 int dep_pack_cluster_split_multi(int n, const float* const* src, float* const* dst, const int* bwd, int H, hipStream_t s);
+int dep_step_jobs_launch(int n, const float* const* src, float* const* dst, const int* bwd, int nzero, void* const* zero,
+                         const size_t* zero_bytes, const dep_ln_fold* fold, int J, int F, int H, hipStream_t s);
 int dep_multi_copy(int count, const float* const* src, const float* const* add, float* const* dst, const long* n, hipStream_t s);
 int dep_attn2_fwd(const float* out, const float* pre, float* ctx, float* alpha, int B, int T, int H, const int* lengths, hipStream_t s);
 int dep_attn2_bwd(const float* dctx, const float* out, const float* alpha, const float* pre, float* dout, float* dpre, int B,
diff --git a/icassp2022-depression_amd/csrc/elementwise.hip b/icassp2022-depression_amd/csrc/elementwise.hip
--- a/icassp2022-depression_amd/csrc/elementwise.hip
+++ b/icassp2022-depression_amd/csrc/elementwise.hip
@@ -87,17 +87,9 @@
 __global__ __launch_bounds__(256) void ln_fold_fwd_kernel(const float* __restrict__ W, const float* __restrict__ b,
                                                           const float* __restrict__ gamma, const float* __restrict__ beta,
                                                           float* __restrict__ Wf, float* __restrict__ bf, int J, int F) {
-    const int lane = threadIdx.x & 63;
     const int j = blockIdx.x * 4 + (threadIdx.x >> 6);
     if (j >= J) return;
-    float s = 0.f;
-    for (int f = lane; f < F; f += 64) {
-        const float w = W[(size_t)j * F + f];
-        Wf[(size_t)j * F + f] = w * gamma[f];
-        s = fmaf(w, beta[f], s);
-    }
-    s = wave_sum(s);
-    if (lane == 0) bf[j] = b[j] + s;
+    dep_ln_fold_fwd_row(W, b, gamma, beta, Wf, bf, j, F, threadIdx.x & 63);
 }
 constexpr int LFC = 16, LFR = 64;
 __global__ __launch_bounds__(1024) void ln_fold_bwd_kernel(const float* __restrict__ W, const float* __restrict__ P,
diff --git a/icassp2022-depression_amd/csrc/head.hip b/icassp2022-depression_amd/csrc/head.hip
--- a/icassp2022-depression_amd/csrc/head.hip
+++ b/icassp2022-depression_amd/csrc/head.hip
@@ -115,77 +115,88 @@
     int first;
 };
 
+__device__ __forceinline__ float head_dz1(const HeadB& q, int H1, int row, int j, float z) {
+    const size_t at = (size_t)row * H1 + j;
+    float da = 0.f;
+    for (int c = 0; c < q.C; ++c) da = fmaf(q.dz2[(size_t)row * q.C + c], q.W2[(size_t)c * H1 + j], da);
+    float v = z > 0.f ? da : 0.f;
+    if (q.p > 0.f) v *= dep_dropmask1(q.seed, q.site1, (uint64_t)at, q.p, q.scale);
+    return v;
+}
+
+template <int NJ>
+__device__ __forceinline__ void bwd_rows(const HeadB& q, int blk, float (*dzs)[HMAX], float (*ps)[HR][HMAX]) {
+    constexpr int H1 = NJ * 8;
+    const int tid = threadIdx.x, row0 = blk * HR, wv = tid >> 6, lane = tid & 63, i4 = lane * 4;
+    const bool want_dx = q.dx != nullptr, col = i4 < q.Hin;
+    f32x4 w[NJ];
+    if (want_dx) {
+        const float* wr = q.W1 + (size_t)(wv * NJ) * q.Hin + (col ? i4 : 0);
+#pragma unroll
+        for (int m = 0; m < NJ; ++m) w[m] = *reinterpret_cast<const f32x4*>(wr + (size_t)m * q.Hin);
+    }
+    constexpr int NX = (HR * H1 + HT - 1) / HT;
+    float zv[NX];
+#pragma unroll
+    for (int k = 0; k < NX; ++k) {
+        const int e = tid + k * HT, r = e / H1, row = row0 + r;
+        const bool ok = e < HR * H1 && row < q.B;
+        zv[k] = q.z1[ok ? (size_t)row * H1 + (e - r * H1) : 0];
+    }
+#pragma unroll
+    for (int k = 0; k < NX; ++k) {
+        const int e = tid + k * HT, r = e / H1, j = e - r * H1, row = row0 + r;
+        if (e >= HR * H1) continue;
+        float v = 0.f;
+        if (row < q.B) {
+            v = head_dz1(q, H1, row, j, zv[k]);
+            q.dz1[(size_t)row * H1 + j] = v;
+        }
+        dzs[r][j] = v;
+    }
+    if (!want_dx) return;
+    __syncthreads();
+    f32x4 acc[HR];
+#pragma unroll
+    for (int r = 0; r < HR; ++r) acc[r] = f32x4{0.f, 0.f, 0.f, 0.f};
+#pragma unroll
+    for (int m = 0; m < NJ; ++m) {
+#pragma unroll
+        for (int r = 0; r < HR; ++r) {
+            const float d = dzs[r][wv * NJ + m];
+#pragma unroll
+            for (int e = 0; e < 4; ++e) acc[r][e] = fmaf(d, w[m][e], acc[r][e]);
+        }
+    }
+#pragma unroll
+    for (int r = 0; r < HR; ++r) *reinterpret_cast<f32x4*>(&ps[wv][r][i4]) = acc[r];
+    __syncthreads();
+    const bool drop0 = q.first && q.p > 0.f;
+    for (int e = tid; e < HR * q.Hin; e += HT) {
+        const int r = e / q.Hin, i = e - r * q.Hin, row = row0 + r;
+        if (row >= q.B) continue;
+        float v = 0.f;
+#pragma unroll
+        for (int u = 0; u < HT / 64; ++u) v += ps[u][r][i];
+        const size_t at = (size_t)row * q.Hin + i;
+        if (drop0) v *= dep_dropmask1(q.seed, q.site0, (uint64_t)at, q.p, q.scale);
+        q.dx[at] = v;
+    }
+}
 template <int NJ>
 __global__ __launch_bounds__(HT) void head_mlp_bwd_rows_kernel(HeadB q) {
     __shared__ __attribute__((aligned(16))) float dzs[HR][HMAX];
     __shared__ __attribute__((aligned(16))) float ps[HT / 64][HR][HMAX];
-    constexpr int H1 = NJ * 8;
-    const int tid = threadIdx.x, row0 = blockIdx.x * HR, wv = tid >> 6, lane = tid & 63, i4 = lane * 4;
-    const bool want_dx = q.dx != nullptr, col = i4 < q.Hin;
-    f32x4 w[NJ];
-    if (want_dx) {
-        const float* wr = q.W1 + (size_t)(wv * NJ) * q.Hin + (col ? i4 : 0);
-#pragma unroll
-        for (int m = 0; m < NJ; ++m) w[m] = *reinterpret_cast<const f32x4*>(wr + (size_t)m * q.Hin);
-    }
-    constexpr int NX = (HR * H1 + HT - 1) / HT;
-    float zv[NX];
-#pragma unroll
-    for (int k = 0; k < NX; ++k) {
-        const int e = tid + k * HT, r = e / H1, row = row0 + r;
-        const bool ok = e < HR * H1 && row < q.B;
-        zv[k] = q.z1[ok ? (size_t)row * H1 + (e - r * H1) : 0];
-    }
-#pragma unroll
-    for (int k = 0; k < NX; ++k) {
-        const int e = tid + k * HT, r = e / H1, j = e - r * H1, row = row0 + r;
-        if (e >= HR * H1) continue;
-        float v = 0.f;
-        if (row < q.B) {
-            const size_t at = (size_t)row * H1 + j;
-            float da = 0.f;
-            for (int c = 0; c < q.C; ++c) da = fmaf(q.dz2[(size_t)row * q.C + c], q.W2[(size_t)c * H1 + j], da);
-            v = zv[k] > 0.f ? da : 0.f;
-            if (q.p > 0.f) v *= dep_dropmask1(q.seed, q.site1, (uint64_t)at, q.p, q.scale);
-            q.dz1[at] = v;
-        }
-        dzs[r][j] = v;
-    }
-    if (!want_dx) return;
-    __syncthreads();
-    f32x4 acc[HR];
-#pragma unroll
-    for (int r = 0; r < HR; ++r) acc[r] = f32x4{0.f, 0.f, 0.f, 0.f};
-#pragma unroll
-    for (int m = 0; m < NJ; ++m) {
-#pragma unroll
-        for (int r = 0; r < HR; ++r) {
-            const float d = dzs[r][wv * NJ + m];
-#pragma unroll
-            for (int e = 0; e < 4; ++e) acc[r][e] = fmaf(d, w[m][e], acc[r][e]);
-        }
-    }
-#pragma unroll
-    for (int r = 0; r < HR; ++r) *reinterpret_cast<f32x4*>(&ps[wv][r][i4]) = acc[r];
-    __syncthreads();
-    const bool drop0 = q.first && q.p > 0.f;
-    for (int e = tid; e < HR * q.Hin; e += HT) {
-        const int r = e / q.Hin, i = e - r * q.Hin, row = row0 + r;
-        if (row >= q.B) continue;
-        float v = 0.f;
-#pragma unroll
-        for (int u = 0; u < HT / 64; ++u) v += ps[u][r][i];
-        const size_t at = (size_t)row * q.Hin + i;
-        if (drop0) v *= dep_dropmask1(q.seed, q.site0, (uint64_t)at, q.p, q.scale);
-        q.dx[at] = v;
-    }
-}
-
-__device__ __forceinline__ void weight_rows(const float* __restrict__ D, int ldD, int nrows, int row0, const float* __restrict__ A,
-                                            int ldA, int ncols, int B, float* out, float* bias) {
-    __shared__ __attribute__((aligned(16))) float ds[BCH][JR];
-    __shared__ __attribute__((aligned(16))) float ps[HT / 64][JR][HMAX];
-    __shared__ float pb[HT / 64][JR];
+    bwd_rows<NJ>(q, blockIdx.x, dzs, ps);
+}
+
+constexpr int W_DS = BCH * JR, W_PS = (HT / 64) * JR * HMAX, W_PB = (HT / 64) * JR;
+template <class DV>
+__device__ __forceinline__ void weight_rows(DV dval, int nrows, int row0, const float* __restrict__ A,
+                                            int ldA, int ncols, int B, float* out, float* bias, float* lds) {
+    float (*ds)[JR] = reinterpret_cast<float (*)[JR]>(lds);
+    float (*ps)[JR][HMAX] = reinterpret_cast<float (*)[JR][HMAX]>(lds + W_DS);
+    float (*pb)[JR] = reinterpret_cast<float (*)[JR]>(lds + W_DS + W_PS);
     static_assert(JR == 4, "one 16-byte broadcast per batch row");
     const int tid = threadIdx.x, wv = tid >> 6, lane = tid & 63, i4 = lane * 4;
     const bool col = i4 < ncols;
@@ -203,7 +214,7 @@
             for (int k = 0; k < 4; ++k) {
                 int e = e0 + tid + k * HT; e = e < nb * JR ? e : nb * JR - 1;
                 const int bb = e / JR, u = e - bb * JR;
-                dv[k] = D[(size_t)(b0 + bb) * ldD + (row0 + u < nrows ? row0 + u : nrows - 1)];
+                dv[k] = dval(b0 + bb, row0 + u < nrows ? row0 + u : nrows - 1);
             }
 #pragma unroll
             for (int k = 0; k < 4; ++k) {
@@ -257,10 +268,28 @@
     }
 }
 
+template <bool FROM_Z1>
+__device__ __forceinline__ void bwd_w(const HeadB& q, int blk, float* lds) {
+    const int n1 = (q.H1 + JR - 1) / JR;
+    if (blk < n1) {
+        if (FROM_Z1) weight_rows([&](int b, int r) { return head_dz1(q, q.H1, b, r, q.z1[(size_t)b * q.H1 + r]); }, q.H1, blk * JR, q.a0, q.Hin, q.Hin, q.B, q.dW1, q.db1, lds);
+        else weight_rows([&](int b, int r) { return q.dz1[(size_t)b * q.H1 + r]; }, q.H1, blk * JR, q.a0, q.Hin, q.Hin, q.B, q.dW1, q.db1, lds);
+    } else {
+        weight_rows([&](int b, int r) { return q.dz2[(size_t)b * q.C + r]; }, q.C, (blk - n1) * JR, q.a1, q.H1, q.H1, q.B, q.dW2, q.db2, lds);
+    }
+}
 __global__ __launch_bounds__(HT) void head_mlp_bwd_w_kernel(HeadB q) {
-    const int n1 = (q.H1 + JR - 1) / JR;
-    if ((int)blockIdx.x < n1) weight_rows(q.dz1, q.H1, q.H1, blockIdx.x * JR, q.a0, q.Hin, q.Hin, q.B, q.dW1, q.db1);
-    else weight_rows(q.dz2, q.C, q.C, ((int)blockIdx.x - n1) * JR, q.a1, q.H1, q.H1, q.B, q.dW2, q.db2);
+    __shared__ __attribute__((aligned(16))) float lds[W_DS + W_PS + W_PB];
+    bwd_w<false>(q, blockIdx.x, lds);
+}
+
+template <int NJ>
+__global__ __launch_bounds__(HT) void head_mlp_bwd_kernel(HeadB q) {
+    __shared__ __attribute__((aligned(16))) float lds[W_DS + W_PS + W_PB];
+    static_assert(HR == JR && W_DS >= HR * HMAX, "the rows pass's dzs | ps fit the weight pass's ds | ps");
+    const int nrow = (q.B + HR - 1) / HR;
+    if ((int)blockIdx.x < nrow) bwd_rows<NJ>(q, blockIdx.x, reinterpret_cast<float (*)[HMAX]>(lds), reinterpret_cast<float (*)[HR][HMAX]>(lds + W_DS));
+    else bwd_w<true>(q, (int)blockIdx.x - nrow, lds);
 }
 
 bool al16(const void* p) { return ((uintptr_t)p & 15) == 0; }
@@ -303,6 +332,19 @@
     }
     HeadB q{dz2, a0, z1, a1, W1, W2, dW1, db1, dW2, db2, dx, dz1, B, Hin, H1, C, p, 1.0f / (1.0f - p), seed, site0, site1, first_dropout};
     const dim3 g(dep_cdiv(B, HR)), b(HT);
+    if (dep_rnn_switches().step_fuse) {
+        const dim3 ga(dep_cdiv(B, HR) + dep_cdiv(H1, JR) + dep_cdiv(C, JR));
+        switch (H1 / 8) {
+            case 1: DEP_LAUNCH(head_mlp_bwd_kernel<1>, ga, b, 0, S_, q); break;
+            case 2: DEP_LAUNCH(head_mlp_bwd_kernel<2>, ga, b, 0, S_, q); break;
+            case 4: DEP_LAUNCH(head_mlp_bwd_kernel<4>, ga, b, 0, S_, q); break;
+            case 8: DEP_LAUNCH(head_mlp_bwd_kernel<8>, ga, b, 0, S_, q); break;
+            case 16: DEP_LAUNCH(head_mlp_bwd_kernel<16>, ga, b, 0, S_, q); break;
+            default: DEP_LAUNCH(head_mlp_bwd_kernel<32>, ga, b, 0, S_, q); break;
+        }
+        DEP_CHECK_LAUNCH();
+        return DEP_OK;
+    }
     switch (H1 / 8) {
         case 1: DEP_LAUNCH(head_mlp_bwd_rows_kernel<1>, g, b, 0, S_, q); break;
         case 2: DEP_LAUNCH(head_mlp_bwd_rows_kernel<2>, g, b, 0, S_, q); break;
diff --git a/icassp2022-depression_amd/csrc/rnn_cluster.hip b/icassp2022-depression_amd/csrc/rnn_cluster.hip
--- a/icassp2022-depression_amd/csrc/rnn_cluster.hip
+++ b/icassp2022-depression_amd/csrc/rnn_cluster.hip
@@ -66,6 +66,9 @@
     return DEP_OK;
 }
 
+size_t dep_cluster_header_bytes() { return PAYLOAD_OFF; }
+void dep_cluster_slot_words(int slot, size_t* off, size_t* bytes) { *off = (size_t)slot * HDR_SLOT + FLAG_OFF; *bytes = HDR_SLOT - FLAG_OFF; }
+
 int dep_pack_cluster_bwd(const float* w_hh, float* out, int G, int H, hipStream_t s) {
     const long n = (long)G * H * H;
     DEP_LAUNCH(pack_cluster_bwd_kernel, dim3(dep_cdiv(n, 256)), dim3(256), 0, s, w_hh, out, G, H);
diff --git a/icassp2022-depression_amd/csrc/rnn_cluster_bwd.hip b/icassp2022-depression_amd/csrc/rnn_cluster_bwd.hip
--- a/icassp2022-depression_amd/csrc/rnn_cluster_bwd.hip
+++ b/icassp2022-depression_amd/csrc/rnn_cluster_bwd.hip
@@ -784,19 +784,34 @@
     pack_fwd_split_piece<3>(W, out, H, idx);
 }
 
-struct PackJobs { const float* src[8]; u32x4* dst[8]; int bwd[8]; int n; };
+struct PackJobs {
+    const float* src[8]; u32x4* dst[8]; int bwd[8]; int n;
+    u32x4* zero[2]; long zero_n[2]; int nzero;
+    dep_ln_fold fold; int J, F;
+};
 __global__ void pack_cluster_split_multi_kernel(PackJobs j, int H) {
-    const int k = blockIdx.y;
-    if (k >= j.n) return;
+    int k = blockIdx.y;
     const long idx = (long)blockIdx.x * blockDim.x + threadIdx.x;
-    const float* W = j.src[k]; u32x4* out = j.dst[k];
-    if (j.bwd[k]) {
-        if (idx >= pack_bwd_split_pieces(3, H)) return;
-        pack_bwd_split_piece<3>(W, out, H, idx);
-    } else {
-        if (idx >= pack_fwd_split_pieces(3, H)) return;
-        pack_fwd_split_piece<3>(W, out, H, idx);
-    }
+    if (k < j.n) {
+        const float* W = j.src[k]; u32x4* out = j.dst[k];
+        if (j.bwd[k]) {
+            if (idx >= pack_bwd_split_pieces(3, H)) return;
+            pack_bwd_split_piece<3>(W, out, H, idx);
+        } else {
+            if (idx >= pack_fwd_split_pieces(3, H)) return;
+            pack_fwd_split_piece<3>(W, out, H, idx);
+        }
+        return;
+    }
+    k -= j.n;
+    if (k < j.nzero) {
+        const u32x4 z = {0u, 0u, 0u, 0u};
+        for (long i = idx; i < j.zero_n[k]; i += (long)gridDim.x * blockDim.x) j.zero[k][i] = z;
+        return;
+    }
+    if (k == j.nzero && j.fold.W)
+        for (int r = blockIdx.x * 4 + (threadIdx.x >> 6); r < j.J; r += gridDim.x * 4)
+            dep_ln_fold_fwd_row(j.fold.W, j.fold.b, j.fold.gamma, j.fold.beta, j.fold.Wf, j.fold.bf, r, j.F, threadIdx.x & 63);
 }
 
 Instance<F2>& fwd_instance(int H, bool split, bool rag) {
@@ -854,6 +869,27 @@
     for (int k = 0; k < n; ++k) { DEP_CHECK_ARG(src[k] && dst[k]); j.src[k] = src[k]; j.dst[k] = (u32x4*)dst[k]; j.bwd[k] = bwd[k]; }
     const long nf = pack_fwd_split_pieces(3, H), nb = pack_bwd_split_pieces(3, H);
     DEP_LAUNCH(pack_cluster_split_multi_kernel, dim3(dep_cdiv(nf > nb ? nf : nb, 256), n), dim3(256), 0, s, j, H);
+    DEP_CHECK_LAUNCH();
+    return DEP_OK;
+}
+
+int dep_step_jobs_launch(int n, const float* const* src, float* const* dst, const int* bwd, int nzero, void* const* zero,
+                         const size_t* zero_bytes, const dep_ln_fold* fold, int J, int F, int H, hipStream_t s) {
+    DEP_CHECK_ARG(n >= 0 && n <= 8 && nzero >= 0 && nzero <= 2 && (n == 0 || (src && dst && bwd)) && (nzero == 0 || (zero && zero_bytes)));
+    DEP_CHECK_ARG(n + nzero + (fold ? 1 : 0) > 0 && H >= 64 && H % 64 == 0);
+    PackJobs j{};
+    j.n = n; j.nzero = nzero;
+    for (int k = 0; k < n; ++k) { DEP_CHECK_ARG(src[k] && dst[k]); j.src[k] = src[k]; j.dst[k] = (u32x4*)dst[k]; j.bwd[k] = bwd[k]; }
+    for (int k = 0; k < nzero; ++k) {
+        DEP_CHECK_ARG(zero[k] && zero_bytes[k] > 0 && zero_bytes[k] % 16 == 0 && ((uintptr_t)zero[k] & 15) == 0);
+        j.zero[k] = (u32x4*)zero[k]; j.zero_n[k] = (long)(zero_bytes[k] / 16);
+    }
+    if (fold) {
+        DEP_CHECK_ARG(fold->W && fold->b && fold->gamma && fold->beta && fold->Wf && fold->bf && J > 0 && F > 0);
+        j.fold = *fold; j.J = J; j.F = F;
+    }
+    const long nf = pack_fwd_split_pieces(3, H), nb = pack_bwd_split_pieces(3, H);
+    DEP_LAUNCH(pack_cluster_split_multi_kernel, dim3(dep_cdiv(nf > nb ? nf : nb, 256), n + nzero + (fold ? 1 : 0)), dim3(256), 0, s, j, H);
     DEP_CHECK_LAUNCH();
     return DEP_OK;
 }
diff --git a/icassp2022-depression_amd/csrc/rnn_fused2_bwd.hip b/icassp2022-depression_amd/csrc/rnn_fused2_bwd.hip
--- a/icassp2022-depression_amd/csrc/rnn_fused2_bwd.hip
+++ b/icassp2022-depression_amd/csrc/rnn_fused2_bwd.hip
@@ -455,11 +455,12 @@
     DEP_CHECK_ARG(!bf || (sv16 && pk));
     DEP_CHECK_ARG(!pk || (sv16 && a.T % 2 == 0 && (size_t)a.B * a.T * 4 * BH * 4 < 0xfffffff0ull));
     DepProfScope prof(DEP_PROF_GRU_BWD, a.stream);
-    return launch_chunks(bwd_instance(drop, a.dy != nullptr, sv16, pk, bf, p.trace != nullptr), g, dim3(BTHREADS), p, a.stream, __PRETTY_FUNCTION__, [&](int) -> int {
+    return launch_chunks(bwd_instance(drop, a.dy != nullptr, sv16, pk, bf, p.trace != nullptr), g, dim3(BTHREADS), p, a.stream, __PRETTY_FUNCTION__, [&](int b0) -> int {
         const size_t pay = fused2_bwd_payload_bytes(p.nbtp);
         DEP_CHECK_ARG(xbuf && PAYLOAD_OFF + pay <= xbuf_bytes && g.resident() && pay < (1ull << 32));
         p.payload_bytes = (unsigned)pay; p.l0_off = (unsigned)((size_t)3 * p.nbtp * BNC * L1_MEMBER);
-        if (const int rc = hdr_prepare(xbuf, 0, false, a.stream)) return rc;
-        return hdr_prepare(xbuf, 1, false, a.stream);
+        const bool clean = a.hdr_clean && b0 == 0;
+        if (const int rc = hdr_prepare(xbuf, 0, clean, a.stream)) return rc;
+        return hdr_prepare(xbuf, 1, clean, a.stream);
     });
 }
diff --git a/icassp2022-depression_amd/csrc/rnn_sweep.hip b/icassp2022-depression_amd/csrc/rnn_sweep.hip
--- a/icassp2022-depression_amd/csrc/rnn_sweep.hip
+++ b/icassp2022-depression_amd/csrc/rnn_sweep.hip
@@ -661,8 +661,7 @@
     }
 }
 
-__global__ void finish_db_kernel(const float* __restrict__ part, int nrows, int H, int G, int cell,
-                                 float* db_ih, float* db_hh) {
+__device__ __forceinline__ void finish_db_column(const float* __restrict__ part, int nrows, int H, int cell, float* db_ih, float* db_hh) {
     const int i = blockIdx.x * blockDim.x + threadIdx.x;
     if (i >= 4 * H) return;
     float s = 0.f;
@@ -683,6 +682,14 @@
     } else {
         db_ih[i] = s; db_hh[i] = s;
     }
+}
+__global__ void finish_db_kernel(const float* __restrict__ part, int nrows, int H, int G, int cell,
+                                 float* db_ih, float* db_hh) {
+    finish_db_column(part, nrows, H, cell, db_ih, db_hh);
+}
+struct FinishDb2 { const float* part[2]; float* db_ih[2]; float* db_hh[2]; };
+__global__ void finish_db2_kernel(FinishDb2 j, int nrows, int H, int cell) {
+    finish_db_column(j.part[blockIdx.y], nrows, H, cell, j.db_ih[blockIdx.y], j.db_hh[blockIdx.y]);
 }
 
 int pick_jpw(int H, int* nw) {
@@ -845,3 +852,11 @@
     }
     return DEP_OK;
 }
+
+int dep_finish_db2(const dep_sweep_bwd_args& a, float* dbi_a, float* dbh_a, const dep_sweep_bwd_args& b, float* dbi_b, float* dbh_b) {
+    DEP_CHECK_ARG(a.dirs == 1 && b.dirs == 1 && a.dbpart_rows >= 1 && a.dbpart_rows == b.dbpart_rows && a.H == b.H && a.cell == b.cell);
+    const FinishDb2 j{{a.dbpart, b.dbpart}, {dbi_a, dbi_b}, {dbh_a, dbh_b}};
+    DEP_LAUNCH(finish_db2_kernel, dim3(dep_cdiv(4 * a.H, 128), 2), dim3(128), 0, a.stream, j, a.dbpart_rows, a.H, a.cell);
+    DEP_CHECK_LAUNCH();
+    return DEP_OK;
+}
diff --git a/icassp2022-depression_amd/models.py b/icassp2022-depression_amd/models.py
--- a/icassp2022-depression_amd/models.py
+++ b/icassp2022-depression_amd/models.py
@@ -206,13 +206,13 @@
         P = self._params
         if self.variant == 'clf':
             xn, _ = L.layernorm_fwd(x.view(B * T, F), None, None, save=False)
-            L.ln_fold_fwd(self._rnn_w[0], self._rnn_w[2], P['ln.weight'].data, P['ln.bias'].data, *self._fold[:2])
+            fold = (self._rnn_w[0], self._rnn_w[2], P['ln.weight'].data, P['ln.bias'].data, *self._fold[:2])
             weights = self._rnn_w_fold
         else:
-            xn, weights = x.view(B * T, F), self._rnn_w
+            xn, weights, fold = x.view(B * T, F), self._rnn_w, None
         rnn = self._rnns.get(B, T, training)
         pooled = torch.empty(B, self.hidden_dims, dtype=torch.float32, device=self.device)
-        rnn.forward(xn, weights, seed=seed, pooled=pooled, lengths=lengths)
+        rnn.forward(xn, weights, seed=seed, pooled=pooled, lengths=lengths, fold=fold)
         return pooled, (x, xn, rnn, lengths)
 
     def forward(self, x, lengths=None):
diff --git a/include/dep_rnn.h b/include/dep_rnn.h
--- a/include/dep_rnn.h
+++ b/include/dep_rnn.h
@@ -118,6 +118,17 @@
                     float* Wf, float* bf, int J, int F, void* stream);
 int dep_ln_fold_bwd(const float* W, const float* dWf, const float* dbf, const float* gamma, const float* beta,
                     float* dW, float* db, float* dgamma, float* dbeta, int J, int F, void* stream);
+typedef struct dep_ln_fold {
+    const float* W; const float* b; const float* gamma; const float* beta;
+    float* Wf; float* bf;
+} dep_ln_fold;
+int dep_rnn_forward_fold(const dep_rnn_desc* d, const float* x, const int32_t* lengths, const float* const* weights,
+                         const dep_ln_fold* fold, float* y, float* pooled, float* h_n,
+                         void* reserve, size_t reserve_bytes, void* workspace, size_t workspace_bytes, void* stream);
+enum { DEP_JOB_IMAGE_FWD = 0, DEP_JOB_IMAGE_BWD = 1, DEP_JOB_ZERO = 2, DEP_JOB_LN_FOLD = 3 };
+enum { DEP_REGION_WORKSPACE = 0, DEP_REGION_RESERVE = 1, DEP_REGION_CALLER = 2 };
+typedef struct dep_step_job { int kind; int region; size_t offset; size_t bytes; } dep_step_job;
+int dep_rnn_step_jobs(const dep_rnn_desc* d, int phase, int with_fold, dep_step_job* jobs, int cap);
 size_t dep_layernorm_bwd_workspace_bytes(int rows, int F);
 int dep_layernorm_bwd(const float* dy, const float* x, const float* gamma, const float* mean_rstd,
                       float* dx, float* dgamma, float* dbeta, int rows, int F,
```

After: 166,500 utterances/s (median of 6 runs). About the same (+0.6%).
